# haoheliu/AudioLDM2

Measured on AMD Instinct MI355X. Metric: audio_seconds_per_second, higher is better.
Workload: dtype f32 storage/accumulate; each product = 6 bf16 MFMA partial products of exact 3-part operand splits (fp32-grade); 1 GPU; audioldm2-full: batch 8 prompts/GPU x 1 GPU, 10.24 s @16 kHz, 200 DDIM steps, CFG 3.5, eta 1.0, n_candidates 1; one step = sample_log + VAE decode + HiFi-GAN + D2H of the waveform; synthetic conditioning, random-init weights, host-CPU RNG noise; global_batch=8, parallelism=prompt-sharded replicas x1, weight_broadcast_bytes=0

## Files before the change

audioldm2_amd/csrc/api.hip:

```cpp
#include "common.h"
#include <string.h>

namespace aldm {
static thread_local char g_err[512] = "";
void set_error(const char* fmt, ...) {
    va_list ap;
    va_start(ap, fmt);
    vsnprintf(g_err, sizeof(g_err), fmt, ap);
    va_end(ap);
}
}

extern "C" int aldm_version(void) { return 13; }
extern "C" const char* aldm_last_error(void) { return aldm::g_err; }
```

audioldm2_amd/csrc/igemm.hip:

```cpp
#include "igemm_kernel.h"
#include <algorithm>
#include <atomic>
#include <stdlib.h>

namespace aldm {

int igemm_launch_pre0(int BM, int BN, int kgroups, bool uni, bool w8, dim3 grid, hipStream_t st, const IgemmK& p);
int igemm_launch_pre1(int BM, int BN, int kgroups, bool uni, bool w8, dim3 grid, hipStream_t st, const IgemmK& p);
int igemm_launch_pre2(int BM, int BN, int kgroups, bool uni, bool w8, dim3 grid, hipStream_t st, const IgemmK& p);
int igemm_launch_pre3(int BM, int BN, int kgroups, bool uni, bool w8, dim3 grid, hipStream_t st, const IgemmK& p);
int igemm_launch_pre4(int BM, int BN, int kgroups, bool uni, bool w8, dim3 grid, hipStream_t st, const IgemmK& p);
int igemm_launch_bx_pre0(int BM, int BN, int kgroups, bool uni, bool w8, dim3 grid, hipStream_t st, const IgemmK& p);
int igemm_launch_bx_pre1(int BM, int BN, int kgroups, bool uni, bool w8, dim3 grid, hipStream_t st, const IgemmK& p);
int igemm_launch_bx_pre2(int BM, int BN, int kgroups, bool uni, bool w8, dim3 grid, hipStream_t st, const IgemmK& p);
int igemm_launch_bx_pre3(int BM, int BN, int kgroups, bool uni, bool w8, dim3 grid, hipStream_t st, const IgemmK& p);

int igemm_launch_dma(int BM, int BN, int nst, int parts, bool f16, dim3 grid, hipStream_t st, const IgemmK& p);
bool igemm_dma_config_ok(int BM, int BN, int nst, int parts);
#ifdef ALDM_TEST_HOOKS
extern std::atomic<int> g_debug_drop_product;
#endif
int igemm_launch_dma_ws(int BM, int BN, int nst, int parts, int blocks, hipStream_t st, const IgemmK& p);
bool igemm_dma_ws_config_ok(int BM, int BN, int nst, int parts);
int igemm_dma_ws_blocks_per_cu(int BM, int BN, int nst, int parts);
// ... 112 lines not shown
}

template <int NP>
__global__ void pack_split_kernel(const float* __restrict__ src, uint4* __restrict__ dst, int Kg, int Npad,
                                  int Ko) {
    const int64_t total = (int64_t)Ko * Npad;
    for (int64_t i = blockIdx.x * (int64_t)blockDim.x + threadIdx.x; i < total;
         i += (int64_t)gridDim.x * blockDim.x) {
        const int n = (int)(i % Npad);
        const int ko = (int)(i / Npad);
        u32x2 part[2][3];
#pragma unroll
        for (int h = 0; h < 2; ++h) {
            const int kg = 2 * ko + h;
            f32x4 f = {0.f, 0.f, 0.f, 0.f};
            if (kg < Kg) f = *reinterpret_cast<const f32x4*>(src + ((int64_t)kg * Npad + n) * 4);
            split4_parts(f, part[h], NP);
        }
#pragma unroll
        for (int q = 0; q < NP; ++q) {
            uint4 o;
            o.x = part[0][q][0];
            o.y = part[0][q][1];
            o.z = part[1][q][0];
            o.w = part[1][q][1];
            dst[((int64_t)ko * NP + q) * Npad + n] = o;
        }
    }
}

__global__ void pack_split_f16_kernel(const float* __restrict__ src, uint4* __restrict__ dst, int Kg, int Npad, int Ko, float scale) {
    const int64_t total = (int64_t)Ko * Npad;
    for (int64_t i = blockIdx.x * (int64_t)blockDim.x + threadIdx.x; i < total; i += (int64_t)gridDim.x * blockDim.x) {
        const int n = (int)(i % Npad);
        const int ko = (int)(i / Npad);
        u32x2 part[2][3];
#pragma unroll
        for (int h = 0; h < 2; ++h) {
            const int kg = 2 * ko + h;
            f32x4 f = {0.f, 0.f, 0.f, 0.f};
            if (kg < Kg) f = *reinterpret_cast<const f32x4*>(src + ((int64_t)kg * Npad + n) * 4);
            split4_f16(f, scale, part[h]);
        }
#pragma unroll
        for (int q = 0; q < 2; ++q) {
            uint4 o;
            o.x = part[0][q][0];
            o.y = part[0][q][1];
            o.z = part[1][q][0];
            o.w = part[1][q][1];
            dst[((int64_t)ko * 2 + q) * Npad + n] = o;
        }
    }
}

static int log2_exact(int v) {
    int s = 0;
    while ((1 << s) < v) ++s;
    return (1 << s) == v ? s : -1;
}

}

using namespace aldm;

static thread_local int g_force_bm = 0, g_force_bn = 0, g_force_splits = 0, g_force_kgroups = 0, g_force_stages = 0;

extern "C" void aldm_igemm_force(int bm, int bn, int splits, int kgroups) {
    g_force_bm = bm;
    g_force_bn = bn;
    g_force_splits = splits;
    g_force_kgroups = kgroups;
    g_force_stages = 0;
}
extern "C" void aldm_igemm_force_stages(int stages) { g_force_stages = stages; }

static int default_wave8_mask() {
    static const int m = [] {
        const char* e = getenv("ALDM_IGEMM_W8");
        return e ? atoi(e) : 1;
    }();
    return m;
}
static thread_local int g_wave8_mask = -1;

extern "C" int aldm_igemm_wave8_mask(int mask) {
    g_wave8_mask = mask;
    return mask < 0 ? default_wave8_mask() : mask;
}

static thread_local int g_force_mma = 0;
extern "C" int aldm_igemm_mma(int mode) {
    const int prev = g_force_mma;
    if (mode >= 0 && mode <= 2) g_force_mma = mode;
    return prev;
}

static int pre_mode_of(const aldm_igemm_desc& d) {
    if (d.pre_scale == nullptr && d.pre_act == ALDM_ACT_NONE) return PRE_NONE;
    if (d.pre_scale != nullptr && d.pre_act == ALDM_ACT_NONE) return PRE_AFFINE;
    if (d.pre_scale != nullptr && d.pre_act == ALDM_ACT_SILU) return PRE_AFFINE_SILU;
    if (d.pre_scale == nullptr && d.pre_act == ALDM_ACT_LRELU) return PRE_LRELU;
    return PRE_GENERIC;
}

static int device_cus() {
    static const int n = [] {
        int dev = 0, cus = 0;
        if (hipGetDevice(&dev) != hipSuccess ||
            hipDeviceGetAttribute(&cus, hipDeviceAttributeMultiprocessorCount, dev) != hipSuccess || cus <= 0)
            return 256;
        return cus;
    }();
    return n;
}

static bool dma_ws_eligible(const IgemmK& p, int BM, int BN) {
    const aldm_igemm_desc& d = p.d;
    const bool geglu = d.epi_mode == ALDM_EPI_GEGLU;
    auto al16 = [](const void* q) { return (reinterpret_cast<uintptr_t>(q) & 15) == 0; };
    if (d.out_mul > 0 || d.accumulate || d.batch != 1 || d.act != ALDM_ACT_NONE || d.out_split_act != ALDM_ACT_NONE ||
        d.epi_mode == ALDM_EPI_QKV)
        return false;
    if (p.M % BM != 0 || d.N % BN != 0 || (d.N & 3) != 0 || (d.ldo & 3) != 0) return false;
    if (!al16(d.out) || !al16(d.res) || !al16(d.bias) || !al16(d.rowbias) || !al16(d.out_split)) return false;
    if (d.rowbias && (p.OHW % BM != 0 || (p.rb_ld & 3) != 0)) return false;
    if (geglu && (BN != 128 || d.res || d.rowbias)) return false;
    return true;
}

static bool dma_os_eligible(const IgemmK& p) {
    const aldm_igemm_desc& d = p.d;
    if (d.KH != 1 || d.KW != 1 || d.SH != 1 || d.SW != 1 || d.PH != 0 || d.PW != 0 || d.up_h != 1 || d.up_w != 1) return false;
    if (d.OH != d.H || d.OW != d.W || d.K != p.Cin || d.K % 32 != 0 || d.out_mul > 0 || d.batch > 1) return false;
    if (d.epi_mode == ALDM_EPI_QKV && d.qkv_c % 128 != 0) return false;
    if (d.rowbias || d.accumulate || d.act != ALDM_ACT_NONE) return false;
    auto al16 = [](const void* q) { return (reinterpret_cast<uintptr_t>(q) & 15) == 0; };
    if ((d.N & 3) != 0 || (d.ldo & 3) != 0 || !al16(d.out) || !al16(d.res)) return false;
    return true;
}

static int dma_halo_chunks(const IgemmK& p, int BM) {
    const aldm_igemm_desc& d = p.d;
    if (d.KH != 3 || d.KW != 3 || d.SH != 1 || d.SW != 1 || d.PH != 1 || d.PW != 1 || d.DH != 1 || d.DW != 1) return 0;
    if (d.up_h != 1 || d.up_w != 1 || d.OH != d.H || d.OW != d.W || d.out_mul > 0 || d.batch > 1) return 0;
    if (d.W <= 0 || (d.W & (d.W - 1)) != 0 || BM % d.W != 0 || p.OHW % BM != 0) return 0;
    return ((BM / d.W + 2) * d.W + 15) / 16;
}

static bool tile_supported(int BM, int BN) {
    return (BM == 128 && (BN == 128 || BN == 64 || BN == 32)) || (BM == 64 && (BN == 128 || BN == 64));
}

static int igemm_prepare(const aldm_igemm_desc* dd, IgemmK& p, int& BM, int& BN) {
    ALDM_CHECK(dd != nullptr, "aldm_igemm: null descriptor");
    p.d = *dd;
    aldm_igemm_desc& d = p.d;
    ALDM_CHECK((d.x1 || d.a_split) && d.w && (d.out || d.out_split), "aldm_igemm: null x1/w/out");
    if (!d.x1) d.x1 = reinterpret_cast<const float*>(d.a_split);
    if (d.split_parts == 0) d.split_parts = 3;
    ALDM_CHECK(d.split_parts == 2 || d.split_parts == 3, "aldm_igemm: split_parts must be 0 / 3 or 2");
    if (d.out_split_parts == 0) d.out_split_parts = d.split_parts;
    ALDM_CHECK(d.out_split_parts == 2 || d.out_split_parts == 3, "aldm_igemm: out_split_parts must be 0, 2 or 3");
    ALDM_CHECK(d.a_fmt == ALDM_FMT_BF16 || (d.a_fmt == ALDM_FMT_F16 && d.a_split != nullptr && d.split_parts == 2 && d.acc_scale > 0.0f),
               "aldm_igemm: a_fmt = ALDM_FMT_F16 needs a pre-split operand (a_split), 2-part images and acc_scale > 0");
    if (d.a_fmt == ALDM_FMT_BF16) d.acc_scale = 1.0f;
    ALDM_CHECK(d.out_split_fmt == ALDM_FMT_BF16 ||
                   (d.out_split_fmt == ALDM_FMT_F16 && d.out_split_scale > 0.0f &&
                    (d.epi_mode == ALDM_EPI_QKV ? (d.k_split != nullptr && d.vt_split != nullptr && d.vt_scale > 0.0f) : d.out_split != nullptr)),
               "aldm_igemm: out_split_fmt = ALDM_FMT_F16 needs out_split (QKV: k_split, vt_split and vt_scale) and out_split_scale > 0");
    if (d.out_split_fmt == ALDM_FMT_F16) d.out_split_parts = 2;
    if (!d.x2) d.C2 = 0;
    if (d.pix1 == 0) d.pix1 = d.C1;
    if (d.pix2 == 0) d.pix2 = d.C2;
    if (d.up_h == 0) d.up_h = 1;
    if (d.up_w == 0) d.up_w = 1;
    if (d.batch == 0) d.batch = 1;
    p.Cin = d.C1 + d.C2;
    ALDM_CHECK(d.C1 > 0 && d.C1 % 4 == 0 && d.C2 % 4 == 0,
               "aldm_igemm: C1=%d/C2=%d must be multiples of 4", d.C1, d.C2);
    ALDM_CHECK(d.pix1 % 4 == 0 && d.pix2 % 4 == 0, "aldm_igemm: pixel pitch must be a multiple of 4");
    ALDM_CHECK(d.K == d.KH * d.KW * p.Cin, "aldm_igemm: K=%d != KH*KW*Cin=%d", d.K,
               d.KH * d.KW * p.Cin);
    ALDM_CHECK(d.N > 0 && (d.ldo >= d.N || d.epi_mode == ALDM_EPI_GEGLU || d.epi_mode == ALDM_EPI_QKV),
               "aldm_igemm: bad N=%d ldo=%d", d.N, d.ldo);
    ALDM_CHECK(d.B > 0 && d.H > 0 && d.W > 0 && d.OH > 0 && d.OW > 0, "aldm_igemm: bad extents");
    ALDM_CHECK(d.SH > 0 && d.SW > 0 && d.DH > 0 && d.DW > 0, "aldm_igemm: bad stride/dilation");
    p.shh = log2_exact(d.up_h);
    p.shw = log2_exact(d.up_w);
    ALDM_CHECK(p.shh >= 0 && p.shw >= 0, "aldm_igemm: upsample factors must be powers of two");
    ALDM_CHECK((reinterpret_cast<uintptr_t>(d.x1) & 15) == 0 &&
                   (reinterpret_cast<uintptr_t>(d.w) & 15) == 0 &&
                   (d.x2 == nullptr || (reinterpret_cast<uintptr_t>(d.x2) & 15) == 0),
               "aldm_igemm: operands must be 16-byte aligned");
    if (d.b_mode == ALDM_B_NT) {
        ALDM_CHECK(d.ldb % 4 == 0 && d.ldb >= d.K, "aldm_igemm: NT ldb=%d invalid", d.ldb);
        p.Npad = d.N;
    } else {
        p.Npad = (d.N + 31) / 32 * 32;
        ALDM_CHECK(d.ldb == 0 || d.ldb == p.Npad, "aldm_igemm: packed ldb must equal Npad");
    }
    if (d.out_mul > 0) ALDM_CHECK(d.OH == 1, "aldm_igemm: row remap requires OH == 1");
    ALDM_CHECK((d.pre_scale == nullptr) == (d.pre_shift == nullptr),
               "aldm_igemm: pre_scale/pre_shift must come together");
    ALDM_CHECK(d.pre_scale == nullptr ||
                   ((reinterpret_cast<uintptr_t>(d.pre_scale) | reinterpret_cast<uintptr_t>(d.pre_shift)) & 15) == 0,
               "aldm_igemm: pre_scale/pre_shift must be 16-byte aligned");
    const bool geglu = d.epi_mode == ALDM_EPI_GEGLU;
    const bool qkv = d.epi_mode == ALDM_EPI_QKV;
    ALDM_CHECK(d.epi_mode == ALDM_EPI_PLAIN || geglu || qkv, "aldm_igemm: unknown epi_mode %d", d.epi_mode);
    if (qkv) {
        auto al16 = [](const void* q) { return (reinterpret_cast<uintptr_t>(q) & 15) == 0; };
        ALDM_CHECK(d.a_split && d.qkv_c > 0 && d.qkv_c % 64 == 0 && d.N == 3 * d.qkv_c && d.qkv_rows > 0 && d.qkv_rows % 32 == 0 &&
                       (((int64_t)d.B * d.OH * d.OW) % d.qkv_rows == 0 ||
                        d.qkv_rows == (((int64_t)d.B * d.OH * d.OW + 31) & ~(int64_t)31)) && d.out && d.k_split && d.vt_split && al16(d.out) &&
                       al16(d.k_split) && al16(d.vt_split) && d.ldo >= d.qkv_c && (d.ldo & 3) == 0 && !d.bias && !d.rowbias &&
                       !d.res && !d.out_split && !d.accumulate && d.out_mul == 0 && d.act == ALDM_ACT_NONE && d.alpha == 1.0f &&
                       d.batch <= 1,
                   "aldm_igemm: ALDM_EPI_QKV needs a pre-split operand, N = 3*qkv_c (qkv_c %% 64 == 0), qkv_rows %% 32 == 0 dividing M "
                   "(or M rounded up to 32), "
                   "aligned out / k_split / vt_split and a plain epilogue");
    }
    if (geglu) {
        ALDM_CHECK(d.N % 64 == 0 && d.ldo >= d.N / 2 && d.ldo % 4 == 0 && d.b_mode == ALDM_B_PACKED &&
                       d.out_mul == 0 && !d.res && !d.rowbias && !d.accumulate &&
                       (d.act == ALDM_ACT_NONE || d.act == ALDM_ACT_GELU_TANH) &&
                       (reinterpret_cast<uintptr_t>(d.out) & 15) == 0 && d.stride_o % 4 == 0 &&
                       (d.bias == nullptr || (reinterpret_cast<uintptr_t>(d.bias) & 15) == 0),
                   "aldm_igemm: GEGLU epilogue needs N %% 64 == 0, ldo >= N/2, packed weights, a plain epilogue");
    }
    p.OHW = d.OH * d.OW;
    const int64_t M64 = (int64_t)d.B * p.OHW;
    ALDM_CHECK(M64 < (1ll << 31) - 256, "aldm_igemm: M too large");
    p.M = (int)M64;
    p.HV = d.H * d.up_h;
    p.WV = d.W * d.up_w;
    ALDM_CHECK((int64_t)d.B * d.H * d.W < (1ll << 31), "aldm_igemm: input has too many pixels");
    p.Kg = (d.K + 3) / 4;
    p.rb_ld = d.rowbias_ld > 0 ? d.rowbias_ld : d.N;

    const int nk = (d.K + BK - 1) / BK;
    const int64_t Mz = p.M;
    const int pre = pre_mode_of(d);
    p.dma = 0;
    p.nst = 0;
    p.ws = 0;
    p.ws_blocks = 0;
    p.os_rows = 0;
    ALDM_CHECK(d.out_split_act == ALDM_ACT_NONE || (d.out_split_act == ALDM_ACT_LRELU && d.out_split != nullptr &&
                                                   d.epi_mode == ALDM_EPI_PLAIN),
               "aldm_igemm: out_split_act must be ALDM_ACT_NONE or ALDM_ACT_LRELU with a split-image output of the plain epilogue");
    if (d.out_split) {
        ALDM_CHECK(d.out_split_c > 0 && d.out_split_c % 32 == 0 && d.out_split_c >= (geglu ? d.N / 2 : d.N) &&
                       d.N % 4 == 0 && d.batch == 1 && (reinterpret_cast<uintptr_t>(d.out_split) & 15) == 0 &&
                       ((reinterpret_cast<uintptr_t>(d.out) | reinterpret_cast<uintptr_t>(d.res)) & 15) == 0 &&
                       (d.out == nullptr || (d.ldo & 3) == 0),
                   "aldm_igemm: out_split needs out_split_c %% 32 == 0 and >= N, N %% 4 == 0, batch 1, aligned out/res");
        ALDM_CHECK(d.out != nullptr || !d.accumulate, "aldm_igemm: accumulate needs an fp32 output");
    }
    if (d.a_split) {
        ALDM_CHECK(d.w_split != nullptr && d.b_mode == ALDM_B_PACKED && d.stride_w == 0 && d.batch == 1,
                   "aldm_igemm: a_split needs packed, split weights and batch 1");
        ALDM_CHECK(d.C2 == 0 && d.C1 % 32 == 0 && pre == PRE_NONE,
                   "aldm_igemm: a_split needs one source with C1 %% 32 == 0 and no prologue (C1=%d C2=%d)", d.C1, d.C2);
        ALDM_CHECK(((reinterpret_cast<uintptr_t>(d.a_split) | reinterpret_cast<uintptr_t>(d.w_split)) & 15) == 0,
                   "aldm_igemm: split images must be 16-byte aligned");
        ALDM_CHECK((int64_t)d.B * d.H * d.W * p.Cin * 2 * d.split_parts < (1ll << 40), "aldm_igemm: split image too large");
        const bool can_split = d.N % 4 == 0 && nk >= 8 && !geglu && !qkv;
        const bool have_ws = d.ws != nullptr && (reinterpret_cast<uintptr_t>(d.ws) & 15) == 0;
        auto dma_cost = [&](int bm, int bn, int nst, int sp, int* sp_eff) -> double {
            const int kt = cdiv(nk, sp);
            sp = cdiv(nk, kt);
            *sp_eff = sp;
            const double blocks = (double)cdiv64(Mz, bm) * cdiv(d.N, bn) * sp;
            const int lds = nst * (bm + bn) * 64 * d.split_parts;
            const int o = std::min(2, (160 * 1024) / lds);
            const double tile_c = (bm / 64) * (bn / 64) * 64.0 * (d.split_parts == 3 ? 6 : 3);
            const double dma_c = (bm + bn) * 64.0 * d.split_parts / 56.0;
            const double L = kt * std::max(tile_c, dma_c);
            const double one = kt * std::max(tile_c + 200.0, dma_c) + 6000.0;
            const int64_t nb = (int64_t)((blocks + 255.0) / 256.0);
            const int64_t full = nb / o, last = nb - full * o;
            double T = full * std::max(one, o * L);
            if (last) T += std::max(one, last * L);
            if (sp > 1) T += 10000.0 + (double)(sp + 1) * Mz * d.N * 4.0 / 2000.0;
            return T;
        };
        int splits = 1, nst = 0;
        const bool hint_fits = d.hint_bm > 0 && (!qkv || (d.hint_bn > 0 && d.qkv_c % d.hint_bn == 0)) && (!geglu || d.hint_bn == 128);
        const int f_bm = g_force_bm ? g_force_bm : (hint_fits ? d.hint_bm : 0), f_bn = g_force_bm ? g_force_bn : d.hint_bn;
        const int f_sp = g_force_bm ? g_force_splits : d.hint_splits;
        int f_st = g_force_bm ? g_force_stages : (hint_fits ? d.hint_stages : 0);
        int ws_nst = 0;
        int lw_nst = 0;
        if (f_st >= 300 && f_st < 400) {
            const int KT = d.K / 32;
            int os_nst = f_st - 300;
            if (os_nst == 0) os_nst = igemm_dma_os_default_stages(KT, d.split_parts);
            if (dma_os_eligible(p) && igemm_dma_os_config_ok(KT, os_nst, d.split_parts)) {
                static const int env_rows = [] {
                    const char* e = getenv("ALDM_OS_ROWS");
                    return e ? atoi(e) : 0;
                }();
                const int tn = cdiv(d.N, 128);
                const int stages = cdiv(p.M, 32);
                const int chunks = std::max(1, device_cus() / tn);
                int rows = cdiv(stages, chunks) * 32;
// ... 77 lines not shown
                if (geglu ? bn != 128 : (bn > 64 && d.N <= 64)) continue;
                if (qkv && d.qkv_c % bn != 0) continue;
                if (bm == 256 && Mz < 4096) continue;
                for (int si = 0; si < 8; ++si) {
                    const int sp = sps[si];
                    if (sp > 1 && (!can_split || !have_ws || nk / sp < 3)) break;
                    int spe;
                    const double t = dma_cost(bm, bn, cand[c][2], sp, &spe);
                    if (spe > 1 && (int64_t)spe * Mz * d.N > d.ws_floats) continue;
                    if (t < best) {
                        best = t;
                        BM = bm;
                        BN = bn;
                        nst = cand[c][2];
                        splits = spe;
                    }
                }
            }
        }
        ALDM_CHECK(!geglu || BN == 128, "aldm_igemm: the GEGLU epilogue needs a 128-column tile");
        ALDM_CHECK(!qkv || d.qkv_c % BN == 0, "aldm_igemm: the QKV epilogue needs a tile width dividing qkv_c");
        if (qkv) splits = 1;
        p.tiles_m = cdiv(p.M, BM);
        p.tiles_n = cdiv(d.N, BN);
        p.kt_per_split = cdiv(nk, splits);
        splits = cdiv(nk, p.kt_per_split);
        if (splits > 1 && (!have_ws || d.ws_floats < (int64_t)splits * p.M * d.N)) {
            splits = 1;
            p.kt_per_split = nk;
        }
        p.splits = splits;
        p.kgroups = 1;
        p.bx = 1;
        p.pre = pre;
        p.dma = 1;
        p.nst = nst;
        p.ws = 0;
        p.ws_blocks = 0;
        if (lw_nst > 0) {
            ALDM_CHECK(igemm_dma_lw_config_ok(BM, BN, lw_nst, d.split_parts), "aldm_igemm: no loader-wave DMA kernel for tile %dx%d, %d stages", BM, BN, lw_nst);
            p.ws = 2;
            p.nst = lw_nst;
        }
        if (ws_nst > 0) {
            if (splits == 1 && d.a_fmt == ALDM_FMT_BF16 && d.out_split_parts == d.split_parts && d.out_split_fmt == ALDM_FMT_BF16 &&
                igemm_dma_ws_config_ok(BM, BN, ws_nst, d.split_parts) && dma_ws_eligible(p, BM, BN)) {
                const int ntiles = p.tiles_m * p.tiles_n;
                const int per = cdiv(ntiles, device_cus() * igemm_dma_ws_blocks_per_cu(BM, BN, ws_nst, d.split_parts));
                p.ws = 1;
                p.nst = ws_nst;
                p.ws_blocks = cdiv(ntiles, per);
            } else {
                ALDM_CHECK(!g_force_bm, "aldm_igemm: the persistent DMA kernel cannot run this launch (tile %dx%d, %d stages)", BM,
                           BN, ws_nst);
            }
        }
        return 0;
    }
    const bool bx_ok = d.w_split != nullptr && d.split_parts == 3 && d.b_mode == ALDM_B_PACKED && d.stride_w == 0 && d.batch == 1 &&
                       pre != PRE_GENERIC && (reinterpret_cast<uintptr_t>(d.w_split) & 15) == 0 &&
                       (g_force_mma == 2 || (g_force_mma == 0 && d.hint_mma != 1));
    auto occ_of = [&](int bm, int bn) {
        if (bx_ok && bn != 32) return bm * bn >= 128 * 128 ? 1 : (bm * bn >= 64 * 128 ? 2 : 3);
        return bm * bn >= 128 * 128 ? 2 : ((bm * bn >= 64 * 128 || bn == 32) ? 3 : 4);
    };
    const double pre_w = (d.pre_scale != nullptr || d.pre_act != ALDM_ACT_NONE) ? 1.5 : 1.0;
    auto cost_of = [&](int bm, int bn, int sp, int kg, int* sp_eff) -> double {
        const bool bx = bx_ok && bn != 32;
        const double mf = bx ? 0.375 : 1.0;
        const int kt = cdiv(nk, sp);
        sp = cdiv(nk, kt);
        *sp_eff = sp;
        const double blocks = (double)cdiv64(Mz, bm) * cdiv(d.N, bn) * d.batch * sp;
        const double L = (double)kt * bm * bn / 4.0 * mf;
        const int o = kg == 2 ? (bx ? 1 : 2) : occ_of(bm, bn);
        const double S = (300.0 * (bm / 32) * pre_w + 200.0 * (bn / 32)) *
                         (bx ? (bm * bn >= 128 * 128 && !geglu ? 0.45 : 1.3) : 1.0);
        const double F = 4000.0 + (kg == 2 ? 600.0 : 0.0);
        const int64_t nb = (int64_t)((blocks + 255.0) / 256.0);
        const int64_t full = nb / o, last = nb - full * o;
        const double one = (double)cdiv(kt, kg) * ((double)bm * bn / 4.0 * mf + S) + F;
        double T = full * std::max(one, o * L);
        if (last) T += std::max(one, last * L);
        if (sp > 1) T += 10000.0 + (double)(sp + 1) * Mz * d.N * d.batch * 4.0 / 2000.0;
        return T;
    };
    const bool can_split = d.N % 4 == 0 && nk >= 8 && !geglu;
    const bool have_ws = d.ws != nullptr && (reinterpret_cast<uintptr_t>(d.ws) & 15) == 0;
    int splits = 1, kgroups = 1;
    const int f_bm = g_force_bm ? g_force_bm : d.hint_bm, f_bn = g_force_bm ? g_force_bn : d.hint_bn;
    const int f_sp = g_force_bm ? g_force_splits : d.hint_splits;
    const int f_kg = g_force_bm ? g_force_kgroups : d.hint_kgroups;
    if (f_bm) {
        BM = f_bm;
        BN = f_bn;
        ALDM_CHECK(tile_supported(BM, BN), "aldm_igemm: unsupported forced/hinted tile %dx%d", BM, BN);
        ALDM_CHECK(!geglu || BN == 128, "aldm_igemm: the GEGLU epilogue needs a 128-column tile");
        if (f_sp > 0 && can_split && nk / f_sp >= 1) splits = f_sp;
        if (f_kg == 2) {
            ALDM_CHECK(BM == 64 && BN == 64, "aldm_igemm: two wave groups exist for the 64x64 tile only");
            kgroups = 2;
        }
    } else if (d.N <= 32 && !geglu) {
        BM = 128;
        BN = 32;
    } else {
        static const int cand[4][2] = {{128, 128}, {64, 128}, {128, 64}, {64, 64}};
        static const int sps[8] = {1, 2, 3, 4, 6, 8, 12, 16};
        double best = 1e300;
        BM = 64;
        BN = 64;
        for (int c = 0; c < 4; ++c) {
            const int bm = cand[c][0], bn = cand[c][1];
            if (geglu ? bn != 128 : (bn > 64 && d.N <= 64)) continue;
            for (int si = 0; si < 8; ++si) {
                const int sp = sps[si];
                if (sp > 1 && (!can_split || !have_ws || nk / sp < 3)) break;
                for (int kg = 1; kg <= ((bm == 64 && bn == 64) ? 2 : 1); ++kg) {
                    int spe;
                    const double t = cost_of(bm, bn, sp, kg, &spe);
                    if (spe > 1 && (int64_t)d.batch * spe * Mz * d.N > d.ws_floats) continue;
                    if (kg == 2 && cdiv(nk, spe) < 4) continue;
                    if (t < best) {
                        best = t;
                        BM = bm;
                        BN = bn;
                        splits = spe;
                        kgroups = kg;
                    }
                }
            }
        }
    }
    ALDM_CHECK(!geglu || BN == 128, "aldm_igemm: internal: GEGLU epilogue without a 128-column tile");
    p.tiles_m = cdiv(p.M, BM);
    p.tiles_n = cdiv(d.N, BN);
    if (splits < 1) splits = 1;
    p.kt_per_split = cdiv(nk, splits);
    splits = cdiv(nk, p.kt_per_split);
    if (splits > 1) {
        const int64_t need = (int64_t)d.batch * splits * p.M * d.N;
        if (!have_ws || d.ws_floats < need) {
            splits = 1;
            p.kt_per_split = nk;
        }
    }
    p.splits = splits;
    p.kgroups = kgroups;
    p.bx = bx_ok && BN != 32 ? 1 : 0;
    p.pre = pre;
    return 0;
}

extern "C" int aldm_igemm_plan(const aldm_igemm_desc* dd, int* bm, int* bn, int64_t* flops, int* splits,
                               int* kgroups, int* mma) {
    IgemmK p;
    int BM, BN;
    const int rc = igemm_prepare(dd, p, BM, BN);
    if (rc) return rc;
    if (bm) *bm = BM;
    if (bn) *bn = BN;
    if (flops) *flops = 2ll * p.M * p.d.N * p.d.K * p.d.batch;
    if (splits) *splits = p.splits;
    if (kgroups) *kgroups = p.kgroups;
    if (mma) *mma = p.bx ? ALDM_MMA_BF16X6 : ALDM_MMA_F32;
    return 0;
}

extern "C" int aldm_igemm_plan_stages(const aldm_igemm_desc* dd) {
    IgemmK p;
    int BM, BN;
    if (igemm_prepare(dd, p, BM, BN)) return -1;
    if (p.dma && p.ws == 4) return 400 + (BM == 128 && p.ws_blocks == 4 ? 10 : 0) + p.nst;
    return p.dma ? p.nst + 100 * p.ws : 0;
}

extern "C" int64_t aldm_igemm_ws_floats(const aldm_igemm_desc* dd) {
    if (!dd) return 0;
    aldm_igemm_desc t = *dd;
    t.ws = reinterpret_cast<float*>(uintptr_t(16));
    t.ws_floats = INT64_MAX;
    IgemmK p;
    int BM, BN;
    if (igemm_prepare(&t, p, BM, BN)) return 0;
    return p.splits > 1 ? (int64_t)p.d.batch * p.splits * p.M * p.d.N : 0;
}

extern "C" int aldm_igemm(const aldm_igemm_desc* dd, void* stream) {
    IgemmK p;
    int BM, BN;
    int rc = igemm_prepare(dd, p, BM, BN);
    if (rc) return rc;
    const aldm_igemm_desc& d = p.d;
    dim3 grid((unsigned)(p.tiles_m * p.tiles_n), (unsigned)p.splits, (unsigned)d.batch);
    hipStream_t st = (hipStream_t)stream;
    const int pre = p.pre;
    const bool uni = p.OHW % BM == 0;
    const int env_w8 = g_wave8_mask < 0 ? default_wave8_mask() : g_wave8_mask;
    const bool gn_pre = pre == PRE_AFFINE || pre == PRE_AFFINE_SILU;
    const int tile_bit = (BM == 128 && BN == 128) ? 1 : (BM == 64 && BN == 128) ? 2 : (BM == 128 && BN == 64) ? 4 : 0;
    const bool w8 = p.kgroups == 1 && d.epi_mode != ALDM_EPI_GEGLU && (env_w8 & tile_bit) != 0 &&
                    (p.bx ? tile_bit == 1 : (gn_pre || (tile_bit == 1 && (env_w8 & 8) != 0)));
#ifdef ALDM_TEST_HOOKS
    if (g_debug_drop_product.load(std::memory_order_relaxed))
        ALDM_CHECK(p.dma && p.ws == 0 && BM == 64 && BN == 128 && p.nst == 2 && d.split_parts == 3,
                   "aldm_igemm: aldm_debug_drop_product is set: force the classic DMA-fed 64x128 tile with 2 stages and 3-part images "
                   "(got dma=%d form=%d tile %dx%d, %d stages, %d parts) or clear the switch", p.dma, p.ws, BM, BN, p.nst, d.split_parts);
#endif
    if (p.dma && p.ws == 4) {
        rc = igemm_launch_dma_halo(BM, BN, p.nst, p.ws_blocks, d.split_parts, d.a_fmt == ALDM_FMT_F16, p.os_rows, grid, st, p);
    } else if (p.dma && p.ws == 3) {
        rc = igemm_launch_dma_os(d.K / 32, p.nst, d.split_parts, d.a_fmt == ALDM_FMT_F16, grid, st, p);
    } else if (p.dma && p.ws == 2) {
        rc = igemm_launch_dma_lw(BM, BN, p.nst, d.split_parts, d.a_fmt == ALDM_FMT_F16, grid, st, p);
    } else if (p.dma && p.ws) {
        rc = igemm_launch_dma_ws(BM, BN, p.nst, d.split_parts, p.ws_blocks, st, p);
    } else if (p.dma) {
        rc = igemm_launch_dma(BM, BN, p.nst, d.split_parts, d.a_fmt == ALDM_FMT_F16, grid, st, p);
    } else if (p.bx) {
        switch (pre) {
            case PRE_NONE: rc = igemm_launch_bx_pre0(BM, BN, p.kgroups, uni, w8, grid, st, p); break;
            case PRE_AFFINE: rc = igemm_launch_bx_pre1(BM, BN, p.kgroups, uni, w8, grid, st, p); break;
            case PRE_AFFINE_SILU: rc = igemm_launch_bx_pre2(BM, BN, p.kgroups, uni, w8, grid, st, p); break;
            default: rc = igemm_launch_bx_pre3(BM, BN, p.kgroups, uni, w8, grid, st, p); break;
        }
    } else
    switch (pre) {
        case PRE_NONE: rc = igemm_launch_pre0(BM, BN, p.kgroups, uni, w8, grid, st, p); break;
        case PRE_AFFINE: rc = igemm_launch_pre1(BM, BN, p.kgroups, uni, w8, grid, st, p); break;
        case PRE_AFFINE_SILU: rc = igemm_launch_pre2(BM, BN, p.kgroups, uni, w8, grid, st, p); break;
        case PRE_LRELU: rc = igemm_launch_pre3(BM, BN, p.kgroups, uni, w8, grid, st, p); break;
        default: rc = igemm_launch_pre4(BM, BN, p.kgroups, uni, w8, grid, st, p); break;
    }
    if (rc) {
        set_error("aldm_igemm: no kernel for tile %dx%d", BM, BN);
        return -1;
    }
    if (p.splits > 1) {
        const int64_t total = (int64_t)p.M * (d.N >> 2);
        hipLaunchKernelGGL(igemm_reduce_kernel, dim3((unsigned)cdiv64(total, 256), 1, (unsigned)d.batch),
                           dim3(256), 0, st, p);
    }
    ALDM_LAUNCH_CHECK("aldm_igemm");
    return 0;
}

extern "C" int64_t aldm_split_bytes_parts(int K, int N, int parts) {
    if (K <= 0 || N <= 0 || (parts != 2 && parts != 3)) return 0;
    const int Npad = (N + 31) / 32 * 32;
    const int64_t Ko = 4ll * ((K + 31) / 32);
    return Ko * parts * Npad * 16;
}
extern "C" int64_t aldm_split_bytes(int K, int N) { return aldm_split_bytes_parts(K, N, 3); }

extern "C" int aldm_pack_split_f16(const float* packed, void* dst, int K, int N, float scale, void* stream) {
    ALDM_CHECK(packed && dst && K > 0 && N > 0 && scale > 0.0f, "aldm_pack_split_f16: bad args");
    ALDM_CHECK(((reinterpret_cast<uintptr_t>(packed) | reinterpret_cast<uintptr_t>(dst)) & 15) == 0,
               "aldm_pack_split_f16: operands must be 16-byte aligned");
    const int Npad = (N + 31) / 32 * 32;
    const int Kg = (K + 3) / 4;
    const int Ko = 4 * ((K + 31) / 32);
    const int64_t total = (int64_t)Ko * Npad;
    hipLaunchKernelGGL(pack_split_f16_kernel, dim3((unsigned)std::min<int64_t>(cdiv64(total, 256), 4096)), dim3(256), 0,
                       (hipStream_t)stream, packed, reinterpret_cast<uint4*>(dst), Kg, Npad, Ko, scale);
    ALDM_LAUNCH_CHECK("aldm_pack_split_f16");
    return 0;
}

extern "C" int aldm_pack_split_bf16_parts(const float* packed, void* dst, int K, int N, int parts, void* stream) {
    ALDM_CHECK(packed && dst && K > 0 && N > 0 && (parts == 2 || parts == 3), "aldm_pack_split_bf16: bad args");
    ALDM_CHECK(((reinterpret_cast<uintptr_t>(packed) | reinterpret_cast<uintptr_t>(dst)) & 15) == 0,
               "aldm_pack_split_bf16: operands must be 16-byte aligned");
    const int Npad = (N + 31) / 32 * 32;
    const int Kg = (K + 3) / 4;
    const int Ko = 4 * ((K + 31) / 32);
    const int64_t total = (int64_t)Ko * Npad;
    const int blocks = (int)std::min<int64_t>((total + 255) / 256, 65535);
    if (parts == 3)
        hipLaunchKernelGGL(pack_split_kernel<3>, dim3(blocks), dim3(256), 0, (hipStream_t)stream, packed,
                           reinterpret_cast<uint4*>(dst), Kg, Npad, Ko);
    else
        hipLaunchKernelGGL(pack_split_kernel<2>, dim3(blocks), dim3(256), 0, (hipStream_t)stream, packed,
                           reinterpret_cast<uint4*>(dst), Kg, Npad, Ko);
    ALDM_LAUNCH_CHECK("aldm_pack_split_bf16");
    return 0;
}
extern "C" int aldm_pack_split_bf16(const float* packed, void* dst, int K, int N, void* stream) {
    return aldm_pack_split_bf16_parts(packed, dst, K, N, 3, stream);
}

extern "C" int aldm_pack_weight(const float* src, float* dst, int N, int Cin, int KH, int KW,
                                int transposed, int phase, int stride, void* stream) {
    ALDM_CHECK(src && dst && N > 0 && Cin > 0 && KH > 0 && KW > 0, "aldm_pack_weight: bad args");
    const int Npad = (N + 31) / 32 * 32;
    hipStream_t st = (hipStream_t)stream;
    if (!transposed) {
        const int K = KH * KW * Cin;
        const int Kg = (K + 3) / 4;
        const int64_t total = (int64_t)Kg * Npad * 4;
        const int blocks = (int)std::min<int64_t>(cdiv64(total, 256), 4096);
        hipLaunchKernelGGL(pack_weight_kernel, dim3(blocks), dim3(256), 0, st, src, dst, N, Cin, KH,
                           KW, Kg, Npad);
    } else {
        ALDM_CHECK(KH == 1 && stride > 0 && phase >= 0 && phase < stride,
                   "aldm_pack_weight: bad transposed args");
        const int T = (KW + stride - 1) / stride;
// ... 24 lines not shown
```

audioldm2_amd/csrc/igemm_epilogue.h:

```cpp
#pragma once
#include "common.h"

#ifndef ALDM_DMA_ABLATE
#define ALDM_DMA_ABLATE 0
#endif

namespace aldm {

struct IgemmK {
    aldm_igemm_desc d;
    int Cin, M, OHW, HV, WV, shh, shw, Kg, Npad, tiles_m, tiles_n;
    int splits, kt_per_split;
    int kgroups;
    int rb_ld;
    int bx;
    int pre;
    int dma;
    int nst;
    int ws;
    int ws_blocks;
    int os_rows;
};

enum { PRE_NONE = 0, PRE_AFFINE = 1, PRE_AFFINE_SILU = 2, PRE_LRELU = 3, PRE_GENERIC = 4 };
// ... 24 lines not shown
__device__ __forceinline__ void acc_total(f32x16 (&acc)[MT][NT], const f32x16 (&sum)[MT][NT]) {
#pragma unroll
    for (int i = 0; i < MT; ++i)
#pragma unroll
        for (int j = 0; j < NT; ++j)
#pragma unroll
            for (int e = 0; e < 16; ++e) acc[i][j][e] += sum[i][j][e];
}

using bf16x8 = __bf16 __attribute__((ext_vector_type(8)));
using u32x2 = unsigned __attribute__((ext_vector_type(2)));
using u32x4 = unsigned __attribute__((ext_vector_type(4)));
__device__ __forceinline__ unsigned hi16_pair(unsigned a, unsigned b) { return __builtin_amdgcn_perm(b, a, 0x07060302u); }

constexpr int SPLIT_BLOCK_BYTES = 192;

__device__ __forceinline__ unsigned bf16_rn_bits(float x) {
    const unsigned u = __builtin_bit_cast(unsigned, x);
    return (u + 0x7FFFu + ((u >> 16) & 1u)) & 0xFFFF0000u;
}

__device__ __forceinline__ void split4(const f32x4 v, u32x2 (&part)[3]) {
    unsigned u0[4], u1[4], u2[4];
#pragma unroll
    for (int c = 0; c < 4; ++c) {
        const float x = v[c];
        u0[c] = __builtin_bit_cast(unsigned, x);
        const float r1 = x - __builtin_bit_cast(float, u0[c] & 0xFFFF0000u);
        u1[c] = __builtin_bit_cast(unsigned, r1);
        const float r2 = r1 - __builtin_bit_cast(float, u1[c] & 0xFFFF0000u);
        u2[c] = __builtin_bit_cast(unsigned, r2);
    }
    part[0] = u32x2{hi16_pair(u0[0], u0[1]), hi16_pair(u0[2], u0[3])};
    part[1] = u32x2{hi16_pair(u1[0], u1[1]), hi16_pair(u1[2], u1[3])};
    part[2] = u32x2{hi16_pair(u2[0], u2[1]), hi16_pair(u2[2], u2[3])};
}

using bf16x4 = __bf16 __attribute__((ext_vector_type(4)));
__device__ __forceinline__ void split4_rn2(const f32x4 v, u32x2 (&part)[3]) {
    const bf16x4 h = __builtin_convertvector(v, bf16x4);
    const bf16x4 m = __builtin_convertvector(v - __builtin_convertvector(h, f32x4), bf16x4);
    part[0] = __builtin_bit_cast(u32x2, h);
    part[1] = __builtin_bit_cast(u32x2, m);
    part[2] = u32x2{0u, 0u};
}

__device__ __forceinline__ void split4_parts(const f32x4 v, u32x2 (&part)[3], int parts) {
    if (parts == 2) split4_rn2(v, part);
    else split4(v, part);
}

using f16x4 = _Float16 __attribute__((ext_vector_type(4)));
using f16x8 = _Float16 __attribute__((ext_vector_type(8)));
__device__ __forceinline__ void split4_f16(const f32x4 v, float s, u32x2 (&part)[3]) {
    f32x4 x;
#pragma unroll
    for (int e = 0; e < 4; ++e) {
        const float t = v[e] * s;
        x[e] = t != t ? t : __builtin_fminf(__builtin_fmaxf(t, -65504.0f), 65504.0f);
    }
    const f16x4 h = __builtin_convertvector(x, f16x4);
    const f16x4 l = __builtin_convertvector(x - __builtin_convertvector(h, f32x4), f16x4);
    part[0] = __builtin_bit_cast(u32x2, h);
    part[1] = __builtin_bit_cast(u32x2, l);
    part[2] = u32x2{0u, 0u};
}
__device__ __forceinline__ void split4_fmt(const f32x4 v, u32x2 (&part)[3], int parts, float f16_scale) {
    if (f16_scale != 0.f) split4_f16(v, f16_scale, part);
    else split4_parts(v, part, parts);
}

__device__ __forceinline__ void split_store4(void* img, int64_t row, int Cs, int c, const f32x4 v, int parts = 3) {
    u32x2 part[3];
    split4_parts(v, part, parts);
    char* base = reinterpret_cast<char*>(img) + (row * (Cs >> 5) + (c >> 5)) * (64 * parts) + (c & 31) * 2;
#pragma unroll
    for (int q = 0; q < 3; ++q)
        if (q < parts) *reinterpret_cast<u32x2*>(base + q * 64) = part[q];
}

__device__ __forceinline__ void split_store4_f16(void* img, int64_t row, int Cs, int c, const f32x4 v, float scale) {
    u32x2 part[3];
    split4_f16(v, scale, part);
    char* base = reinterpret_cast<char*>(img) + (row * (Cs >> 5) + (c >> 5)) * 128 + (c & 31) * 2;
    *reinterpret_cast<u32x2*>(base) = part[0];
    *reinterpret_cast<u32x2*>(base + 64) = part[1];
}
__device__ __forceinline__ void split_store4_out(const aldm_igemm_desc& d, void* img, int64_t row, int Cs, int c, const f32x4 v) {
    if (d.out_split_fmt == ALDM_FMT_F16) split_store4_f16(img, row, Cs, c, v, d.out_split_scale);
    else split_store4(img, row, Cs, c, v, d.out_split_parts);
}

template <int P>
__device__ __forceinline__ void split_store4_t(void* img, int64_t row, int Cs, int c, const f32x4 v) {
    static_assert(P == 2 || P == 3, "2 or 3 parts");
    u32x2 part[3];
    if constexpr (P == 2) split4_rn2(v, part);
    else split4(v, part);
    char* base = reinterpret_cast<char*>(img) + (row * (Cs >> 5) + (c >> 5)) * (64 * P) + (c & 31) * 2;
#pragma unroll
    for (int q = 0; q < P; ++q) *reinterpret_cast<u32x2*>(base + q * 64) = part[q];
}

__device__ __forceinline__ float epi_value(const aldm_igemm_desc& d, int rb_ld, const float* __restrict__ outp,
                                           const float* __restrict__ resp, int b, int64_t o, int n, float v) {
    if (d.bias) v += d.bias[n];
    if (d.rowbias) v += d.rowbias[(int64_t)b * rb_ld + n];
    v = act_apply(v, d.act, d.act_slope);
    if (resp) v += resp[o];
    v *= d.alpha;
    if (d.accumulate) v += outp[o];
    return v;
}

__device__ __forceinline__ float silu_fast(float v) {
    return v * __frcp_rn(1.0f + __expf(-v));
}

__device__ __forceinline__ void split8_to_parts(const float (&x)[8], u32x4 (&part)[3], int parts) {
    f32x4 a = {x[0], x[1], x[2], x[3]}, b = {x[4], x[5], x[6], x[7]};
    u32x2 pa[3], pb[3];
    split4_parts(a, pa, parts);
    split4_parts(b, pb, parts);
#pragma unroll
    for (int q = 0; q < 3; ++q) part[q] = u32x4{pa[q][0], pa[q][1], pb[q][0], pb[q][1]};
}

template <int MT, int NT, int PAD = 4>
__device__ __forceinline__ void igemm_epilogue(const IgemmK& p, f32x16 (&acc)[MT][NT], float* lds, int m0, int n0,
                                               int wave, int wm, int wn, int lane, int z, int split) {
    const aldm_igemm_desc& d = p.d;
    const bool epi_st = (ALDM_DMA_ABLATE & 64) ? p.M == -12345 : true;
    constexpr int SP = NT * 32 + PAD;
    constexpr int C4 = NT * 8;
    constexpr int RPI = 64 / C4;
    constexpr int IT = 32 / RPI;
    constexpr int ITC = IT < 4 ? IT : 4;
    const int l31 = lane & 31;
    const int lh = lane >> 5;
    float* stg = lds + wave * (32 * SP);
    const int sr = lane / C4;
    const int sc = (lane % C4) * 4;
    const int ncol = n0 + wn * NT * 32 + sc;
    const bool split_out = p.splits > 1;
    const bool vec = split_out || ((d.ldo & 3) == 0 && (d.N & 3) == 0 &&
                                   ((reinterpret_cast<uintptr_t>(d.out) | reinterpret_cast<uintptr_t>(d.res)) & 15) == 0 &&
                                   ((d.stride_o & 3) == 0));
    float* outp = split_out ? d.ws + ((int64_t)z * p.splits + split) * (int64_t)p.M * d.N
                            : (d.out ? d.out + (int64_t)z * d.stride_o : nullptr);
    const float* resp = (!split_out && d.res) ? d.res + (int64_t)z * d.stride_o : nullptr;
    const bool need_b = !split_out && (d.rowbias != nullptr || d.out_mul > 0);
    const int ld_out = split_out ? d.N : d.ldo;
    void* simg = split_out ? nullptr : d.out_split;
    int col_shift = 0;
    int simg_c = d.out_split_c;
    if (d.epi_mode == ALDM_EPI_QKV) {
        const int seg = n0 / d.qkv_c;
        if (seg == 2) {
            char* vt = reinterpret_cast<char*>(d.vt_split);
            const int heads = d.qkv_c >> 5, parts = d.out_split_parts;
            const int tiles = d.qkv_rows >> 5;
#pragma unroll
            for (int i = 0; i < MT; ++i) {
                const int mb = m0 + (wm * MT + i) * 32;
                if (mb >= p.M) continue;
                const int b = mb / d.qkv_rows, t = (mb - b * d.qkv_rows) >> 5;
#pragma unroll
                for (int j = 0; j < NT; ++j) {
                    const int h = (n0 - 2 * d.qkv_c + (wn * NT + j) * 32) >> 5;
                    char* base = vt + ((((int64_t)b * heads + h) * tiles + t) * parts) * 2048 + l31 * 64 + lh * 16;
#pragma unroll
                    for (int s = 0; s < 2; ++s) {
                        float x8[8];
#pragma unroll
                        for (int e = 0; e < 8; ++e) x8[e] = acc[i][j][8 * s + e];
                        u32x4 part[3];
                        if (d.out_split_fmt == ALDM_FMT_F16) {
                            f32x4 a = {x8[0], x8[1], x8[2], x8[3]}, bq = {x8[4], x8[5], x8[6], x8[7]};
                            u32x2 pa[3], pb[3];
                            split4_f16(a, d.vt_scale, pa);
                            split4_f16(bq, d.vt_scale, pb);
#pragma unroll
                            for (int q = 0; q < 3; ++q) part[q] = u32x4{pa[q][0], pa[q][1], pb[q][0], pb[q][1]};
                        } else {
                            split8_to_parts(x8, part, parts);
                        }
#pragma unroll
                        for (int q = 0; q < 3; ++q)
                            if (q < parts && epi_st) *reinterpret_cast<u32x4*>(base + q * 2048 + s * 32) = part[q];
                    }
                }
            }
            return;
        }
        if (seg == 1) {
            outp = nullptr;
            simg = d.k_split;
            simg_c = d.qkv_c;
            col_shift = d.qkv_c;
        } else {
            simg = nullptr;
        }
    }
    if constexpr (NT == 2) {
        if (d.epi_mode == ALDM_EPI_GEGLU) {
            const int gr = lane >> 3, gc = (lane & 7) * 4;
            const int ncol_p = n0 + wn * 64 + gc;
            const int ncol_o = ((n0 + wn * 64) >> 1) + gc;
            const bool cok = ncol_p < d.N;
            f32x4 bv = {0.f, 0.f, 0.f, 0.f}, bg = {0.f, 0.f, 0.f, 0.f};
            if (d.bias && cok) {
                bv = *reinterpret_cast<const f32x4*>(d.bias + ncol_p);
                bg = *reinterpret_cast<const f32x4*>(d.bias + ncol_p + 32);
            }
            float* go = d.out ? d.out + (int64_t)z * d.stride_o : nullptr;
            const int gate_act = d.act == ALDM_ACT_GELU_TANH ? ALDM_ACT_GELU_TANH : ALDM_ACT_GELU;
#pragma unroll
            for (int i = 0; i < MT; ++i) {
#pragma unroll
                for (int j = 0; j < NT; ++j)
#pragma unroll
                    for (int e = 0; e < 16; ++e)
                        stg[((e & 3) + 8 * (e >> 2) + 4 * lh) * SP + j * 32 + l31] = acc[i][j][e];
#pragma unroll
                for (int it = 0; it < 4; ++it) {
                    const int r = it * 8 + gr;
                    f32x4 xv = *reinterpret_cast<const f32x4*>(&stg[r * SP + gc]) + bv;
                    const f32x4 xg = *reinterpret_cast<const f32x4*>(&stg[r * SP + 32 + gc]) + bg;
#pragma unroll
                    for (int c = 0; c < 4; ++c) xv[c] *= act_apply(xg[c], gate_act, 0.f);
                    const int m = m0 + (wm * MT + i) * 32 + r;
                    if (m < p.M && cok && epi_st) {
                        if (go) *reinterpret_cast<f32x4*>(go + (int64_t)m * d.ldo + ncol_o) = xv;
                        if (simg) split_store4_out(d, simg, m, d.out_split_c, ncol_o, xv);
                    }
                }
            }
            return;
        }
    }
    f32x4 bias4 = {0.f, 0.f, 0.f, 0.f};
    if (!split_out && d.bias) {
#pragma unroll
        for (int c = 0; c < 4; ++c) bias4[c] = d.bias[min(ncol + c, d.N - 1)];
    }
#pragma unroll
    for (int i = 0; i < MT; ++i) {
#pragma unroll
        for (int j = 0; j < NT; ++j)
#pragma unroll
            for (int e = 0; e < 16; ++e)
                stg[((e & 3) + 8 * (e >> 2) + 4 * lh) * SP + j * 32 + l31] = acc[i][j][e];
#pragma unroll
        for (int itc = 0; itc < IT; itc += ITC) {
        f32x4 v[ITC];
        int64_t rowoff[ITC];
        int64_t srow[ITC];
        int rboff[ITC];
        unsigned okmask = 0;
#pragma unroll
        for (int it = 0; it < ITC; ++it) {
            const int r = (itc + it) * RPI + sr;
            v[it] = *reinterpret_cast<const f32x4*>(&stg[r * SP + sc]);
            const int m = m0 + (wm * MT + i) * 32 + r;
            bool ok = m < p.M && ncol < d.N;
            int b = 0;
            int64_t orow = m;
            if (need_b) {
                b = m / p.OHW;
                if (d.out_mul > 0) {
                    const int qq = m - b * p.OHW;
                    const int t = qq * d.out_mul + d.out_off;
                    ok = ok && (unsigned)t < (unsigned)d.out_len;
                    orow = (int64_t)b * d.out_len + t;
                }
            }
            rowoff[it] = ok ? orow * ld_out + (ncol - col_shift) : 0;
            srow[it] = orow;
            rboff[it] = ok ? b * p.rb_ld + ncol : 0;
            okmask |= ((ok && epi_st) ? 1u : 0u) << it;
        }
        if (split_out) {
#pragma unroll
            for (int it = 0; it < ITC; ++it)
                if ((okmask >> it) & 1u) *reinterpret_cast<f32x4*>(outp + rowoff[it]) = v[it];
            continue;
        }
#pragma unroll
        for (int it = 0; it < ITC; ++it) v[it] += bias4;
        if (d.rowbias) {
#pragma unroll
            for (int it = 0; it < ITC; ++it)
#pragma unroll
                for (int c = 0; c < 4; ++c) v[it][c] += d.rowbias[rboff[it] + (ncol + c < d.N ? c : 0)];
        }
        switch (d.act) {
            case ALDM_ACT_NONE: break;
            case ALDM_ACT_SILU:
#pragma unroll
                for (int it = 0; it < ITC; ++it)
#pragma unroll
                    for (int c = 0; c < 4; ++c) v[it][c] = act_apply(v[it][c], ALDM_ACT_SILU, 0.f);
                break;
            case ALDM_ACT_GELU:
#pragma unroll
                for (int it = 0; it < ITC; ++it)
#pragma unroll
                    for (int c = 0; c < 4; ++c) v[it][c] = act_apply(v[it][c], ALDM_ACT_GELU, 0.f);
                break;
            default:
#pragma unroll
                for (int it = 0; it < ITC; ++it)
#pragma unroll
                    for (int c = 0; c < 4; ++c) v[it][c] = act_apply(v[it][c], d.act, d.act_slope);
                break;
        }
        if (vec) {
            if (resp) {
#pragma unroll
                for (int it = 0; it < ITC; ++it) v[it] += *reinterpret_cast<const f32x4*>(resp + rowoff[it]);
            }
#pragma unroll
            for (int it = 0; it < ITC; ++it) v[it] *= d.alpha;
            if (d.accumulate) {
#pragma unroll
                for (int it = 0; it < ITC; ++it) v[it] += *reinterpret_cast<const f32x4*>(outp + rowoff[it]);
            }
            if (outp) {
#pragma unroll
                for (int it = 0; it < ITC; ++it)
                    if ((okmask >> it) & 1u) *reinterpret_cast<f32x4*>(outp + rowoff[it]) = v[it];
            }
            if (simg) {
                if (d.out_split_act == ALDM_ACT_LRELU) {
#pragma unroll
                    for (int it = 0; it < ITC; ++it)
#pragma unroll
                        for (int c = 0; c < 4; ++c) v[it][c] = v[it][c] > 0.0f ? v[it][c] : v[it][c] * d.out_split_slope;
                }
#pragma unroll
                for (int it = 0; it < ITC; ++it)
                    if ((okmask >> it) & 1u) {
                        split_store4_out(d, simg, srow[it], simg_c, ncol - col_shift, v[it]);
                    }
            }
        } else {
#pragma unroll
            for (int it = 0; it < ITC; ++it)
#pragma unroll
                for (int c = 0; c < 4; ++c) {
                    if (!((okmask >> it) & 1u) || ncol + c >= d.N) continue;
                    float x = v[it][c];
                    if (resp) x += resp[rowoff[it] + c];
                    x *= d.alpha;
                    if (d.accumulate) x += outp[rowoff[it] + c];
                    outp[rowoff[it] + c] = x;
                }
        }
        }
    }
}

}
```

audioldm2_amd/csrc/norm.hip:

```cpp
#include <stdlib.h>
#include "igemm_epilogue.h"

namespace aldm {

constexpr int GN_ITERS = 16;
constexpr int GN_UNROLL = 8;

struct GnPart {
    float n, mean, m2;
};

__device__ __forceinline__ void gn_merge(double& n, double& mean, double& m2, double nb, double mb, double m2b) {
    if (nb <= 0.0) return;
    const double nt = n + nb;
    const double dlt = mb - mean;
    mean += dlt * (nb / nt);
    m2 += m2b + dlt * dlt * (n * nb / nt);
    n = nt;
}

template <bool FUSED>
__global__ __launch_bounds__(256) void gn_partial_kernel(const float* __restrict__ x1,
                                                         const float* __restrict__ x2, int P,
                                                         int C1, int C2, int G, int cols, int rows,
// ... 79 lines not shown
                    wred[tid >> 6][1] = mean;
                    wred[tid >> 6][2] = m2;
                }
                __syncthreads();
                if (tid == 0) {
                    double an = gacc[gl][0], am = gacc[gl][1], a2 = gacc[gl][2];
                    for (int w = 0; w < 4; ++w) gn_merge(an, am, a2, wred[w][0], wred[w][1], wred[w][2]);
                    gacc[gl][0] = an;
                    gacc[gl][1] = am;
                    gacc[gl][2] = a2;
                }
                __syncthreads();
            }
            continue;
        }
        ps[tid] = part;
        __syncthreads();
        if (tid < gpb) {
            const int g = g_lo + tid;
            const int base = c4_lo + cp * cols;
            const int lo = max(g * Cg4, base), hi = min((g + 1) * Cg4, min(C4, base + cols));
            if (lo < hi) {
                double n = gacc[tid][0], mean = gacc[tid][1], m2 = gacc[tid][2];
                for (int yy = 0; yy < rows; ++yy)
                    for (int cc = lo; cc < hi; ++cc) {
                        const GnPart& t = ps[yy * cols + (cc - base)];
                        gn_merge(n, mean, m2, (double)t.n, (double)t.mean, (double)t.m2);
                    }
                gacc[tid][0] = n;
                gacc[tid][1] = mean;
                gacc[tid][2] = m2;
            }
        }
        __syncthreads();
    }
    if (FUSED) {
        const int Cg = C / G;
        __shared__ float fin[64][2];
        if (tid < gpb) {
            const double n = gacc[tid][0];
            double var = n > 0.0 ? gacc[tid][2] / n : 0.0;
            if (var < 0.0) var = 0.0;
            fin[tid][0] = (float)gacc[tid][1];
            fin[tid][1] = (float)(1.0 / sqrt(var + (double)eps));
        }
        __syncthreads();
        __shared__ float lsc[256], lsh[256];
        for (int c = g_lo * Cg + tid; c < (g_lo + gpb) * Cg; c += 256) {
            const int g = c / Cg - g_lo;
            const float sc = fin[g][1] * (gamma ? gamma[c] : 1.f);
            const float sh = (beta ? beta[c] : 0.f) - fin[g][0] * sc;
            scale[(int64_t)b * C + c] = sc;
            shift[(int64_t)b * C + c] = sh;
            if (dst) {
                lsc[c - g_lo * Cg] = sc;
                lsh[c - g_lo * Cg] = sh;
            }
        }
        if (dst) {
            __syncthreads();
            const int c_lo = g_lo * Cg, sw = (gpb * Cg) >> 3;
            for (int i = tid; i < P * sw; i += 256) {
                const int p = i / sw;
                const int cl = (i - p * sw) << 3;
                const int c = c_lo + cl;
                const int64_t row = (int64_t)b * P + p;
                const float* src = c < C1 ? x1 + row * C1 + c : x2 + row * C2 + (c - C1);
                f32x4 v0 = *reinterpret_cast<const f32x4*>(src);
                f32x4 v1 = *reinterpret_cast<const f32x4*>(src + 4);
                const int64_t off = (row * (C >> 5) + (c >> 5)) * (64 * parts) + (c & 31) * 2;
                u32x2 p0[3], p1[3];
                if (dst_raw) {
                    const int64_t roff = (row * (C >> 5) + (c >> 5)) * (64 * raw_parts) + (c & 31) * 2;
                    split4_parts(v0, p0, raw_parts);
                    split4_parts(v1, p1, raw_parts);
#pragma unroll
                    for (int q = 0; q < 3; ++q)
                        if (q < raw_parts)
                            *reinterpret_cast<u32x4*>(dst_raw + roff + q * 64) = u32x4{p0[q][0], p0[q][1], p1[q][0], p1[q][1]};
                }
#pragma unroll
                for (int e = 0; e < 4; ++e) {
                    v0[e] = __builtin_fmaf(v0[e], lsc[cl + e], lsh[cl + e]);
                    v1[e] = __builtin_fmaf(v1[e], lsc[cl + 4 + e], lsh[cl + 4 + e]);
                }
                if (act == ALDM_ACT_SILU) {
#pragma unroll
                    for (int e = 0; e < 4; ++e) {
                        v0[e] = silu_fast(v0[e]);
                        v1[e] = silu_fast(v1[e]);
                    }
                }
                split4_fmt(v0, p0, parts, f16_scale);
                split4_fmt(v1, p1, parts, f16_scale);
#pragma unroll
                for (int q = 0; q < 3; ++q)
                    if (q < parts) *reinterpret_cast<u32x4*>(dst + off + q * 64) = u32x4{p0[q][0], p0[q][1], p1[q][0], p1[q][1]};
            }
        }
    } else if (tid < G) {
        double* w = reinterpret_cast<double*>(ws) + ((int64_t)(b * gridDim.x + chunk) * G + tid) * 3;
        w[0] = gacc[tid][0];
        w[1] = gacc[tid][1];
        w[2] = gacc[tid][2];
    }
}

__global__ __launch_bounds__(256) void gn_finalize_kernel(const float* __restrict__ ws, int chunks,
                                                          int P, int C, int G, float eps,
                                                          const float* __restrict__ gamma,
                                                          const float* __restrict__ beta,
                                                          float* __restrict__ scale,
                                                          float* __restrict__ shift) {
    const int b = blockIdx.x;
    __shared__ float s_mean[64], s_rstd[64];
    __shared__ double s_part[256][3];
    const int Cg = C / G;
    const double* wsd = reinterpret_cast<const double*>(ws);
    const int LPG = 256 / G >= 1 ? 256 / G : 1;
    {
        const int g = threadIdx.x / LPG, l = threadIdx.x % LPG;
        double n = 0.0, mean = 0.0, m2 = 0.0;
        if (g < G) {
            for (int ch = l; ch < chunks; ch += LPG) {
                const double* w = wsd + ((int64_t)(b * chunks + ch) * G + g) * 3;
                gn_merge(n, mean, m2, w[0], w[1], w[2]);
            }
        }
        s_part[threadIdx.x][0] = n;
        s_part[threadIdx.x][1] = mean;
        s_part[threadIdx.x][2] = m2;
    }
    __syncthreads();
    if (threadIdx.x < G) {
        const int g = threadIdx.x;
        double n = 0.0, mean = 0.0, m2 = 0.0;
        for (int l = 0; l < LPG; ++l) gn_merge(n, mean, m2, s_part[g * LPG + l][0], s_part[g * LPG + l][1], s_part[g * LPG + l][2]);
        double var = n > 0.0 ? m2 / n : 0.0;
        if (var < 0.0) var = 0.0;
        s_mean[g] = (float)mean;
        s_rstd[g] = (float)(1.0 / sqrt(var + (double)eps));
    }
    __syncthreads();
    for (int c = threadIdx.x; c < C; c += blockDim.x) {
        const int g = c / Cg;
        const float ga = gamma ? gamma[c] : 1.f;
        const float be = beta ? beta[c] : 0.f;
        const float sc = s_rstd[g] * ga;
        scale[(int64_t)b * C + c] = sc;
        shift[(int64_t)b * C + c] = be - s_mean[g] * sc;
    }
}

constexpr int LN_MAXV = 8;

template <int MAXV, int R, bool RMS = false>
__global__ __launch_bounds__(256) void layernorm_kernel(const float* __restrict__ x,
                                                        float* __restrict__ y, int M, int C,
                                                        const float* __restrict__ gamma,
                                                        const float* __restrict__ beta, float eps,
                                                        void* __restrict__ y_split, int parts, float f16_scale) {
    const int lane = threadIdx.x & 63;
    const int row0 = (blockIdx.x * 4 + (threadIdx.x >> 6)) * R;
    if (row0 >= M) return;
    const int C4 = C >> 2;
    f32x4 v[R][MAXV];
#pragma unroll
    for (int r = 0; r < R; ++r) {
        const float* xr = x + (int64_t)min(row0 + r, M - 1) * C;
#pragma unroll
        for (int i = 0; i < MAXV; ++i) {
            const int c4 = lane + 64 * i;
            v[r][i] = c4 < C4 ? *reinterpret_cast<const f32x4*>(xr + 4 * c4) : f32x4{0.f, 0.f, 0.f, 0.f};
        }
    }
    f32x4 ga[MAXV], be[MAXV];
#pragma unroll
    for (int i = 0; i < MAXV; ++i) {
        const int c4 = min(lane + 64 * i, C4 - 1);
        ga[i] = *reinterpret_cast<const f32x4*>(gamma + 4 * c4);
        be[i] = RMS ? f32x4{0.f, 0.f, 0.f, 0.f} : *reinterpret_cast<const f32x4*>(beta + 4 * c4);
    }
    float mean[R], rstd[R];
#pragma unroll
    for (int r = 0; r < R; ++r) {
        float s = 0.f;
#pragma unroll
        for (int i = 0; i < MAXV; ++i) s += (v[r][i][0] + v[r][i][1]) + (v[r][i][2] + v[r][i][3]);
#pragma unroll
        for (int o = 32; o > 0; o >>= 1) s += __shfl_xor(s, o);
        mean[r] = RMS ? 0.f : s / (float)C;
    }
#pragma unroll
    for (int r = 0; r < R; ++r) {
        float q = 0.f;
#pragma unroll
        for (int i = 0; i < MAXV; ++i) {
            if (lane + 64 * i < C4) {
                const f32x4 dlt = v[r][i] - mean[r];
                q += (dlt[0] * dlt[0] + dlt[1] * dlt[1]) + (dlt[2] * dlt[2] + dlt[3] * dlt[3]);
            }
        }
#pragma unroll
        for (int o = 32; o > 0; o >>= 1) q += __shfl_xor(q, o);
        rstd[r] = 1.0f / sqrtf(q / (float)C + eps);
    }
#pragma unroll
    for (int r = 0; r < R; ++r) {
        if (row0 + r >= M) break;
        float* yr = y ? y + (int64_t)(row0 + r) * C : nullptr;
#pragma unroll
        for (int i = 0; i < MAXV; ++i) {
            const int c4 = lane + 64 * i;
            if (c4 < C4) {
                const f32x4 o = (v[r][i] - mean[r]) * rstd[r] * ga[i] + be[i];
                if (yr) *reinterpret_cast<f32x4*>(yr + 4 * c4) = o;
                if (y_split) {
                    if (f16_scale != 0.f) {
                        u32x2 part[3];
                        split4_f16(o, f16_scale, part);
                        char* base = reinterpret_cast<char*>(y_split) + ((int64_t)(row0 + r) * (C >> 5) + (c4 >> 3)) * 128 + (c4 & 7) * 8;
                        *reinterpret_cast<u32x2*>(base) = part[0];
                        *reinterpret_cast<u32x2*>(base + 64) = part[1];
                    } else {
                        split_store4(y_split, row0 + r, C, 4 * c4, o, parts);
                    }
                }
            }
        }
    }
}

template <bool MASKED, bool BIASED = false>
__global__ __launch_bounds__(256) void softmax_rows_kernel(const float* __restrict__ x,
                                                           float* __restrict__ y, int N,
                                                           float scale, const float* __restrict__ keymask,
                                                           int rows_per_batch, int q_rows, int q_pos0,
                                                           const float* __restrict__ bias = nullptr) {
    extern __shared__ __attribute__((aligned(16))) float srow[];
    __shared__ float red[4];
    const int64_t row = blockIdx.x;
    const float* xr = x + row * N;
    float* yr = y + row * N;
    const int tid = threadIdx.x;
    float mx = -INFINITY;
    const float* km = nullptr;
    int jmax = N;
    const float* br = nullptr;
    if (MASKED) {
        km = keymask + (row / rows_per_batch) * N;
        jmax = BIASED ? N : q_pos0 + (int)(row % q_rows) + 1;
    }
    if (BIASED) br = bias + (row % rows_per_batch) * N;
    for (int i = tid; i < N; i += 256) {
        float v = xr[i] * scale;
        if (BIASED) v += br[i];
        if (MASKED && (i >= jmax || km[i] == 0.0f)) v = -INFINITY;
        srow[i] = v;
        mx = fmaxf(mx, v);
    }
#pragma unroll
    for (int o = 32; o > 0; o >>= 1) mx = fmaxf(mx, __shfl_xor(mx, o));
    if ((tid & 63) == 0) red[tid >> 6] = mx;
    __syncthreads();
    mx = fmaxf(fmaxf(red[0], red[1]), fmaxf(red[2], red[3]));
    __syncthreads();
    float s = 0.f;
    for (int i = tid; i < N; i += 256) {
        const float e = (MASKED && srow[i] == -INFINITY) ? 0.0f : expf(srow[i] - mx);
        srow[i] = e;
        s += e;
    }
#pragma unroll
    for (int o = 32; o > 0; o >>= 1) s += __shfl_xor(s, o);
    if ((tid & 63) == 0) red[tid >> 6] = s;
    __syncthreads();
    s = (red[0] + red[1]) + (red[2] + red[3]);
    const float inv = 1.0f / s;
    for (int i = tid; i < N; i += 256) yr[i] = srow[i] * inv;
}

static void gn_geometry(int P, int C, int* cols, int* rows, int* chunk_px, int* chunks) {
    const int C4 = C / 4;
    *cols = C4 < 256 ? C4 : 256;
    *rows = 256 / *cols;
    if (*rows < 1) *rows = 1;
    *chunk_px = *rows * GN_ITERS;
    *chunks = (P + *chunk_px - 1) / *chunk_px;
}

}

using namespace aldm;

extern "C" int64_t aldm_gn_ws_floats(int B, int P, int C, int G) {
    int cols, rows, chunk_px, chunks;
    gn_geometry(P, C, &cols, &rows, &chunk_px, &chunks);
    return (int64_t)B * chunks * G * 6 + 2;
}

extern "C" int aldm_split_rows(const float* x1, const float* x2, int C1, int C2, int64_t rows, int P, const float* scale,
                               const float* shift, int act, void* dst, void* dst_raw, int parts, void* stream);
extern "C" int aldm_split_rows_f16(const float* x1, const float* x2, int C1, int C2, int64_t rows, int P, const float* scale,
                                   const float* shift, int act, float slope, void* dst, void* dst_raw, int raw_parts, float f16_scale,
                                   void* stream);

static int groupnorm_launch(const float* x1, const float* x2, int B, int P, int C1, int C2, int G, float eps,
                            const float* gamma, const float* beta, float* scale, float* shift, float* ws, void* dst,
                            void* dst_raw, int parts, int act, void* stream, int raw_parts = 0, float f16_scale = 0.f) {
    if (raw_parts == 0) raw_parts = parts;
    if (!x2) C2 = 0;
    const int C = C1 + C2;
    ALDM_CHECK(x1 && scale && shift && ws, "aldm_groupnorm_stats: null pointer");
    ws = reinterpret_cast<float*>((reinterpret_cast<uintptr_t>(ws) + 7) & ~uintptr_t(7));
    ALDM_CHECK(G > 0 && G <= 64 && C % G == 0 && (C / G) % 4 == 0 && C1 % 4 == 0,
               "aldm_groupnorm_stats: need C%%G==0, (C/G)%%4==0, C1%%4==0 (C1=%d C2=%d G=%d)", C1, C2, G);
    int cols, rows, chunk_px, chunks;
    gn_geometry(P, C, &cols, &rows, &chunk_px, &chunks);
    hipStream_t st = (hipStream_t)stream;
    static const int64_t fused_max = [] {
        const char* e = getenv("ALDM_GN_FUSED_MAX");
        return e ? (int64_t)atoll(e) : (int64_t)1 << 17;
    }();
    int gs = 1;
    while (gs < G && gs * B < 256 && G % (gs * 2) == 0) gs *= 2;
    const int gpb = G / gs;
    if ((int64_t)P * C <= fused_max && P <= 1024 && gpb <= 4) {
        const int c4b = gpb * (C / G) / 4;
        const int fcols = c4b < 256 ? c4b : 256, frows = 256 / fcols;
        const int slab = gpb * (C / G);
        static const bool fuse_split = [] {
            const char* e = getenv("ALDM_GN_SPLIT_FUSED");
            return e == nullptr || e[0] != '0';
        }();
        if (dst && fuse_split && slab % 8 == 0 && slab <= 256 && C1 % 8 == 0) {
            hipLaunchKernelGGL(gn_partial_kernel<true>, dim3(gs, B), dim3(256), 0, st, x1, x2, P, C1, C2, G, fcols, frows, P, ws,
                               eps, gamma, beta, scale, shift, gpb, reinterpret_cast<char*>(dst),
                               reinterpret_cast<char*>(dst_raw), parts, act, raw_parts, f16_scale);
            ALDM_LAUNCH_CHECK("aldm_groupnorm_split");
            return 0;
        }
        hipLaunchKernelGGL(gn_partial_kernel<true>, dim3(gs, B), dim3(256), 0, st, x1, x2, P, C1, C2, G, fcols,
                           frows, P, ws, eps, gamma, beta, scale, shift, gpb, nullptr, nullptr, 3, ALDM_ACT_NONE);
    } else {
        hipLaunchKernelGGL(gn_partial_kernel<false>, dim3(chunks, B), dim3(256), 0, st, x1, x2, P, C1, C2, G,
                           cols, rows, chunk_px, ws, eps, gamma, beta, scale, shift, G);
        hipLaunchKernelGGL(gn_finalize_kernel, dim3(B), dim3(256), 0, st, ws, chunks, P, C, G, eps, gamma,
                           beta, scale, shift);
    }
    ALDM_LAUNCH_CHECK("aldm_groupnorm_stats");
    if (dst) {
        if (f16_scale != 0.f)
            return aldm_split_rows_f16(x1, x2, C1, C2, (int64_t)B * P, P, scale, shift, act, 0.f, dst, dst_raw, raw_parts, f16_scale, stream);
        return aldm_split_rows(x1, x2, C1, C2, (int64_t)B * P, P, scale, shift, act, dst, dst_raw, parts, stream);
    }
    return 0;
}

extern "C" int aldm_groupnorm_stats(const float* x1, const float* x2, int B, int P, int C1, int C2,
                                    int G, float eps, const float* gamma, const float* beta,
                                    float* scale, float* shift, float* ws, void* stream) {
    return groupnorm_launch(x1, x2, B, P, C1, C2, G, eps, gamma, beta, scale, shift, ws, nullptr, nullptr, 3, ALDM_ACT_NONE,
                            stream);
}

extern "C" int aldm_groupnorm_split(const float* x1, const float* x2, int B, int P, int C1, int C2, int G, float eps,
                                    const float* gamma, const float* beta, int act, float* scale, float* shift, float* ws,
                                    void* dst, void* dst_raw, int parts, void* stream) {
    if (!x2) C2 = 0;
    ALDM_CHECK(dst != nullptr && (parts == 2 || parts == 3) && (C1 + C2) % 32 == 0 && C1 % 8 == 0 && C2 % 8 == 0,
               "aldm_groupnorm_split: need dst, parts 2|3, (C1+C2) %% 32 == 0, C1 %% 8 == 0 (C1=%d C2=%d)", C1, C2);
    ALDM_CHECK(act == ALDM_ACT_NONE || act == ALDM_ACT_SILU, "aldm_groupnorm_split: activation %d not supported", act);
    ALDM_CHECK(((reinterpret_cast<uintptr_t>(dst) | reinterpret_cast<uintptr_t>(dst_raw)) & 15) == 0,
               "aldm_groupnorm_split: split images must be 16-byte aligned");
    return groupnorm_launch(x1, x2, B, P, C1, C2, G, eps, gamma, beta, scale, shift, ws, dst, dst_raw, parts, act, stream);
}

extern "C" int aldm_groupnorm_split_f16(const float* x1, const float* x2, int B, int P, int C1, int C2, int G, float eps,
                                        const float* gamma, const float* beta, int act, float* scale, float* shift, float* ws,
                                        void* dst, void* dst_raw, int raw_parts, float f16_scale, void* stream) {
    if (!x2) C2 = 0;
    ALDM_CHECK(dst != nullptr && f16_scale > 0.0f && (raw_parts == 2 || raw_parts == 3) && (C1 + C2) % 32 == 0 && C1 % 8 == 0 && C2 % 8 == 0,
               "aldm_groupnorm_split_f16: need dst, f16_scale > 0, raw_parts 2|3, (C1+C2) %% 32 == 0, C1 %% 8 == 0 (C1=%d C2=%d)", C1, C2);
    ALDM_CHECK(act == ALDM_ACT_NONE || act == ALDM_ACT_SILU, "aldm_groupnorm_split_f16: activation %d not supported", act);
    ALDM_CHECK(((reinterpret_cast<uintptr_t>(dst) | reinterpret_cast<uintptr_t>(dst_raw)) & 15) == 0,
               "aldm_groupnorm_split_f16: split images must be 16-byte aligned");
    return groupnorm_launch(x1, x2, B, P, C1, C2, G, eps, gamma, beta, scale, shift, ws, dst, dst_raw, 2, act, stream, raw_parts, f16_scale);
}

static int layernorm_launch(const float* x, float* y, void* y_split, int parts, int M, int C, const float* gamma,
                            const float* beta, float eps, void* stream, const char* name, bool rms = false, float f16_scale = 0.f) {
    ALDM_CHECK(parts == 2 || parts == 3, "%s: parts must be 2 or 3", name);
    ALDM_CHECK(x && (y || y_split) && gamma && (beta || rms), "%s: null pointer", name);
    ALDM_CHECK(C % 4 == 0 && C <= 256 * LN_MAXV, "%s: C=%d must be a multiple of 4 and <= %d", name, C, 256 * LN_MAXV);
    ALDM_CHECK(y_split == nullptr || (C % 32 == 0 && (reinterpret_cast<uintptr_t>(y_split) & 15) == 0),
               "%s: a split-image output needs C %% 32 == 0 and 16-byte alignment", name);
    hipStream_t st = (hipStream_t)stream;
#define ALDM_LN(V_, R_)                                                                                             \
    do {                                                                                                            \
        if (rms)                                                                                                    \
            hipLaunchKernelGGL((layernorm_kernel<V_, R_, true>), dim3(cdiv(M, 4 * R_)), dim3(256), 0, st, x, y, M, C, \
                               gamma, beta, eps, y_split, parts, f16_scale);                                        \
        else                                                                                                        \
            hipLaunchKernelGGL((layernorm_kernel<V_, R_, false>), dim3(cdiv(M, 4 * R_)), dim3(256), 0, st, x, y, M, \
                               C, gamma, beta, eps, y_split, parts, f16_scale);                                     \
    } while (0)
    const int nv = cdiv(C / 4, 64);
    static const int env_r = [] {
        const char* e = getenv("ALDM_LN_R");
        return e ? atoi(e) : 0;
    }();
    if (nv <= 1) {
        if (env_r == 4) ALDM_LN(1, 4);
        else if (env_r == 2) ALDM_LN(1, 2);
        else ALDM_LN(1, 1);
    } else if (nv <= 2) {
        if (env_r == 4) ALDM_LN(2, 4);
        else if (env_r == 2) ALDM_LN(2, 2);
        else ALDM_LN(2, 1);
    } else if (nv <= 4) ALDM_LN(4, 2);
    else ALDM_LN(8, 1);
#undef ALDM_LN
    ALDM_LAUNCH_CHECK(name);
    return 0;
}

extern "C" int aldm_layernorm(const float* x, float* y, int M, int C, const float* gamma,
                              const float* beta, float eps, void* stream) {
    return layernorm_launch(x, y, nullptr, 3, M, C, gamma, beta, eps, stream, "aldm_layernorm");
}

extern "C" int aldm_layernorm_split(const float* x, float* y, void* y_split, int M, int C, const float* gamma,
                                    const float* beta, float eps, int parts, void* stream) {
    return layernorm_launch(x, y, y_split, parts, M, C, gamma, beta, eps, stream, "aldm_layernorm_split");
}

extern "C" int aldm_layernorm_split_f16(const float* x, float* y, void* y_split, int M, int C, const float* gamma,
                                        const float* beta, float eps, float f16_scale, void* stream) {
    ALDM_CHECK(y_split != nullptr && f16_scale > 0.0f, "aldm_layernorm_split_f16: need y_split and f16_scale > 0");
    return layernorm_launch(x, y, y_split, 2, M, C, gamma, beta, eps, stream, "aldm_layernorm_split_f16", false, f16_scale);
}

extern "C" int aldm_rmsnorm(const float* x, float* y, int M, int C, const float* weight, float eps, void* stream) {
    return layernorm_launch(x, y, nullptr, 3, M, C, weight, nullptr, eps, stream, "aldm_rmsnorm", true);
}

extern "C" int aldm_softmax_rows(const float* x, float* y, int64_t M, int N, float scale,
                                 void* stream) {
    ALDM_CHECK(x && y && M > 0 && N > 0, "aldm_softmax_rows: bad args");
    ALDM_CHECK((int64_t)N * 4 <= 60 * 1024, "aldm_softmax_rows: row of %d floats exceeds the 60 KiB LDS stage", N);
    ALDM_CHECK(M < (1ll << 31), "aldm_softmax_rows: too many rows");
    hipLaunchKernelGGL(softmax_rows_kernel<false>, dim3((unsigned)M), dim3(256), (size_t)N * 4,
                       (hipStream_t)stream, x, y, N, scale, nullptr, 1, 1, 0);
    ALDM_LAUNCH_CHECK("aldm_softmax_rows");
    return 0;
}

extern "C" int aldm_softmax_rows_masked(const float* x, float* y, int B, int heads, int q_rows, int N, float scale,
                                        const float* keymask, int q_pos0, void* stream) {
    ALDM_CHECK(x && y && keymask && B > 0 && heads > 0 && q_rows > 0 && N > 0 && q_pos0 >= 0,
               "aldm_softmax_rows_masked: bad args");
    ALDM_CHECK((int64_t)N * 4 <= 60 * 1024, "aldm_softmax_rows_masked: row of %d floats exceeds the 60 KiB LDS stage", N);
    const int64_t M = (int64_t)B * heads * q_rows;
    ALDM_CHECK(M < (1ll << 31), "aldm_softmax_rows_masked: too many rows");
    hipLaunchKernelGGL(softmax_rows_kernel<true>, dim3((unsigned)M), dim3(256), (size_t)N * 4, (hipStream_t)stream, x, y,
                       N, scale, keymask, heads * q_rows, q_rows, q_pos0);
    ALDM_LAUNCH_CHECK("aldm_softmax_rows_masked");
    return 0;
}

extern "C" int aldm_softmax_rows_bias(const float* x, float* y, int B, int heads, int q_rows, int N, float scale,
                                      const float* bias, const float* keymask, void* stream) {
    ALDM_CHECK(x && y && bias && keymask && B > 0 && heads > 0 && q_rows > 0 && N > 0, "aldm_softmax_rows_bias: bad args");
    ALDM_CHECK((int64_t)N * 4 <= 60 * 1024, "aldm_softmax_rows_bias: row of %d floats exceeds the 60 KiB LDS stage", N);
    const int64_t M = (int64_t)B * heads * q_rows;
    ALDM_CHECK(M < (1ll << 31), "aldm_softmax_rows_bias: too many rows");
    hipLaunchKernelGGL((softmax_rows_kernel<true, true>), dim3((unsigned)M), dim3(256), (size_t)N * 4, (hipStream_t)stream, x,
                       y, N, scale, keymask, heads * q_rows, q_rows, 0, bias);
    ALDM_LAUNCH_CHECK("aldm_softmax_rows_bias");
    return 0;
}
```

audioldm2_amd/lib.py:

```python
from __future__ import annotations

import ctypes as C
import os

_HERE = os.path.dirname(os.path.abspath(__file__))
LIB_PATH = os.environ.get("ALDM_LIB_PATH") or os.path.join(_HERE, "libaldm_hip.so")
ABI_VERSION = 13

ACT_NONE, ACT_SILU, ACT_LRELU, ACT_TANH, ACT_LOGCLAMP, ACT_GELU, ACT_GELU_TANH = range(7)
B_PACKED, B_NT = 0, 1
EPI_PLAIN, EPI_GEGLU, EPI_QKV = 0, 1, 2
FMT_BF16, FMT_F16 = 0, 1


class IgemmDesc(C.Structure):

    _fields_ = [
        ("x1", C.c_void_p), ("x2", C.c_void_p),
        ("C1", C.c_int32), ("C2", C.c_int32),
        ("pix1", C.c_int32), ("pix2", C.c_int32),
        ("B", C.c_int32), ("H", C.c_int32), ("W", C.c_int32),
        ("up_h", C.c_int32), ("up_w", C.c_int32),
        ("KH", C.c_int32), ("KW", C.c_int32), ("SH", C.c_int32), ("SW", C.c_int32),
        ("PH", C.c_int32), ("PW", C.c_int32), ("DH", C.c_int32), ("DW", C.c_int32),
        ("OH", C.c_int32), ("OW", C.c_int32),
        ("pre_scale", C.c_void_p), ("pre_shift", C.c_void_p),
        ("pre_act", C.c_int32), ("pre_slope", C.c_float),
        ("w", C.c_void_p),
        ("b_mode", C.c_int32), ("ldb", C.c_int32),
        ("K", C.c_int32), ("N", C.c_int32),
        ("bias", C.c_void_p), ("rowbias", C.c_void_p), ("res", C.c_void_p), ("out", C.c_void_p),
        ("ldo", C.c_int32), ("act", C.c_int32), ("act_slope", C.c_float), ("alpha", C.c_float),
        ("accumulate", C.c_int32),
        ("out_mul", C.c_int32), ("out_off", C.c_int32), ("out_len", C.c_int32),
        ("batch", C.c_int32),
        ("stride_x", C.c_int64), ("stride_w", C.c_int64), ("stride_o", C.c_int64),
        ("rowbias_ld", C.c_int32), ("epi_mode", C.c_int32),
        ("ws", C.c_void_p), ("ws_floats", C.c_int64),
        ("hint_bm", C.c_int32), ("hint_bn", C.c_int32), ("hint_splits", C.c_int32), ("hint_kgroups", C.c_int32),
        ("w_split", C.c_void_p), ("hint_mma", C.c_int32), ("hint_stages", C.c_int32),
        ("a_split", C.c_void_p), ("out_split", C.c_void_p), ("out_split_c", C.c_int32), ("split_parts", C.c_int32),
        ("out_split_act", C.c_int32), ("out_split_slope", C.c_float),
        ("k_split", C.c_void_p), ("vt_split", C.c_void_p), ("qkv_c", C.c_int32), ("qkv_rows", C.c_int32),
        ("a_fmt", C.c_int32), ("acc_scale", C.c_float), ("out_split_parts", C.c_int32),
        ("out_split_fmt", C.c_int32), ("out_split_scale", C.c_float), ("vt_scale", C.c_float),
    ]


_SIGS = {
    "aldm_version": (C.c_int, []),
    "aldm_last_error": (C.c_char_p, []),
    "aldm_igemm": (C.c_int, [C.POINTER(IgemmDesc), C.c_void_p]),
    "aldm_igemm_plan": (C.c_int, [C.POINTER(IgemmDesc), C.POINTER(C.c_int), C.POINTER(C.c_int),
                                  C.POINTER(C.c_int64), C.POINTER(C.c_int), C.POINTER(C.c_int),
                                  C.POINTER(C.c_int)]),
    "aldm_igemm_ws_floats": (C.c_int64, [C.POINTER(IgemmDesc)]),
    "aldm_igemm_plan_stages": (C.c_int, [C.POINTER(IgemmDesc)]),
    "aldm_igemm_force": (None, [C.c_int, C.c_int, C.c_int, C.c_int]),
    "aldm_igemm_force_stages": (None, [C.c_int]),
    "aldm_igemm_wave8_mask": (C.c_int, [C.c_int]),
    "aldm_split_image_bytes": (C.c_int64, [C.c_int64, C.c_int, C.c_int]),
    "aldm_split_rows": (C.c_int, [C.c_void_p, C.c_void_p, C.c_int, C.c_int, C.c_int64, C.c_int, C.c_void_p, C.c_void_p,
                                  C.c_int, C.c_void_p, C.c_void_p, C.c_int, C.c_void_p]),
    "aldm_split_rows_act": (C.c_int, [C.c_void_p, C.c_void_p, C.c_int, C.c_int, C.c_int64, C.c_int, C.c_void_p, C.c_void_p,
                                      C.c_int, C.c_float, C.c_void_p, C.c_void_p, C.c_int, C.c_void_p]),
    "aldm_layernorm_split": (C.c_int, [C.c_void_p, C.c_void_p, C.c_void_p, C.c_int, C.c_int, C.c_void_p, C.c_void_p,
                                       C.c_float, C.c_int, C.c_void_p]),
    "aldm_attention_d32_split": (C.c_int, [C.c_void_p, C.c_void_p, C.c_void_p, C.c_void_p, C.c_void_p, C.c_int, C.c_int,
                                           C.c_int, C.c_int, C.c_int, C.c_int, C.c_int, C.c_int, C.c_int,
                                           C.c_void_p, C.c_float, C.c_void_p]),
    "aldm_split_bytes_parts": (C.c_int64, [C.c_int, C.c_int, C.c_int]),
    "aldm_pack_split_bf16_parts": (C.c_int, [C.c_void_p, C.c_void_p, C.c_int, C.c_int, C.c_int, C.c_void_p]),
    "aldm_pack_split_f16": (C.c_int, [C.c_void_p, C.c_void_p, C.c_int, C.c_int, C.c_float, C.c_void_p]),
    "aldm_split_rows_f16": (C.c_int, [C.c_void_p, C.c_void_p, C.c_int, C.c_int, C.c_int64, C.c_int, C.c_void_p, C.c_void_p,
                                      C.c_int, C.c_float, C.c_void_p, C.c_void_p, C.c_int, C.c_float, C.c_void_p]),
    "aldm_groupnorm_split_f16": (C.c_int, [C.c_void_p, C.c_void_p, C.c_int, C.c_int, C.c_int, C.c_int, C.c_int, C.c_float,
                                           C.c_void_p, C.c_void_p, C.c_int, C.c_void_p, C.c_void_p, C.c_void_p, C.c_void_p,
                                           C.c_void_p, C.c_int, C.c_float, C.c_void_p]),
    "aldm_layernorm_split_f16": (C.c_int, [C.c_void_p, C.c_void_p, C.c_void_p, C.c_int, C.c_int, C.c_void_p, C.c_void_p,
                                           C.c_float, C.c_float, C.c_void_p]),
    "aldm_igemm_mma": (C.c_int, [C.c_int]),
    "aldm_split_bytes": (C.c_int64, [C.c_int, C.c_int]),
    "aldm_pack_split_bf16": (C.c_int, [C.c_void_p, C.c_void_p, C.c_int, C.c_int, C.c_void_p]),
    "aldm_pack_weight": (C.c_int, [C.c_void_p, C.c_void_p, C.c_int, C.c_int, C.c_int, C.c_int,
                                   C.c_int, C.c_int, C.c_int, C.c_void_p]),
    "aldm_pack_kn": (C.c_int, [C.c_void_p, C.c_void_p, C.c_int, C.c_int, C.c_int, C.c_int,
                               C.c_int64, C.c_int64, C.c_void_p]),
    "aldm_groupnorm_stats": (C.c_int, [C.c_void_p, C.c_void_p, C.c_int, C.c_int, C.c_int, C.c_int,
                                       C.c_int, C.c_float, C.c_void_p, C.c_void_p, C.c_void_p,
                                       C.c_void_p, C.c_void_p, C.c_void_p]),
    "aldm_gn_ws_floats": (C.c_int64, [C.c_int, C.c_int, C.c_int, C.c_int]),
    "aldm_groupnorm_split": (C.c_int, [C.c_void_p, C.c_void_p, C.c_int, C.c_int, C.c_int, C.c_int, C.c_int, C.c_float,
                                       C.c_void_p, C.c_void_p, C.c_int, C.c_void_p, C.c_void_p, C.c_void_p, C.c_void_p,
                                       C.c_void_p, C.c_int, C.c_void_p]),
    "aldm_layernorm": (C.c_int, [C.c_void_p, C.c_void_p, C.c_int, C.c_int, C.c_void_p, C.c_void_p,
                                 C.c_float, C.c_void_p]),
    "aldm_attention_mma": (C.c_int, [C.c_int]),
    "aldm_attention_sched": (C.c_int, [C.c_int]),
    "aldm_attention_query_tiles": (C.c_int, [C.c_int, C.c_int, C.c_int]),
    "aldm_attention_d32_presplit_f16": (C.c_int, [C.c_void_p, C.c_void_p, C.c_void_p, C.c_void_p, C.c_void_p, C.c_int, C.c_float,
                                                  C.c_int, C.c_int, C.c_int, C.c_int, C.c_int, C.c_int, C.c_float, C.c_float,
                                                  C.c_float, C.c_float, C.c_void_p]),
    "aldm_attention_d32_presplit": (C.c_int, [C.c_void_p, C.c_void_p, C.c_void_p, C.c_void_p, C.c_void_p, C.c_int, C.c_int,
                                              C.c_int, C.c_int, C.c_int, C.c_int, C.c_int, C.c_float, C.c_void_p]),
    "aldm_vt_regroup": (C.c_int, [C.c_void_p, C.c_void_p, C.c_int, C.c_int, C.c_int, C.c_int, C.c_void_p]),
    "aldm_attention_d32": (C.c_int, [C.c_void_p, C.c_void_p, C.c_void_p, C.c_void_p, C.c_int,
                                     C.c_int, C.c_int, C.c_int, C.c_int, C.c_int, C.c_int, C.c_int,
                                     C.c_void_p, C.c_float, C.c_void_p]),
    "aldm_rel_attention": (C.c_int, [C.c_void_p, C.c_void_p, C.c_void_p, C.c_void_p, C.c_int, C.c_int, C.c_int, C.c_int,
                                     C.c_int, C.c_int, C.c_int, C.c_int, C.c_void_p, C.c_void_p, C.c_int, C.c_void_p,
                                     C.c_void_p]),
    "aldm_rowscale_add": (C.c_int, [C.c_void_p, C.c_void_p, C.c_void_p, C.c_void_p, C.c_int64, C.c_int, C.c_int, C.c_void_p]),
    "aldm_rmsnorm": (C.c_int, [C.c_void_p, C.c_void_p, C.c_int, C.c_int, C.c_void_p, C.c_float, C.c_void_p]),
    "aldm_softmax_rows_bias": (C.c_int, [C.c_void_p, C.c_void_p, C.c_int, C.c_int, C.c_int, C.c_int, C.c_float, C.c_void_p,
                                         C.c_void_p, C.c_void_p]),
    "aldm_resample_sinc": (C.c_int, [C.c_void_p, C.c_void_p, C.c_void_p, C.c_int, C.c_int, C.c_int, C.c_int, C.c_int, C.c_int,
                                     C.c_int, C.c_void_p]),
    "aldm_power_spec": (C.c_int, [C.c_void_p, C.c_void_p, C.c_int64, C.c_int, C.c_int, C.c_int, C.c_void_p]),
    "aldm_col_affine": (C.c_int, [C.c_void_p, C.c_void_p, C.c_void_p, C.c_void_p, C.c_int64, C.c_int, C.c_void_p]),
    "aldm_bicubic_patchify": (C.c_int, [C.c_void_p, C.c_void_p, C.c_int, C.c_int, C.c_int, C.c_int, C.c_int, C.c_void_p]),
    "aldm_token_mean": (C.c_int, [C.c_void_p, C.c_void_p, C.c_int, C.c_int, C.c_int, C.c_void_p]),
    "aldm_row_cosine": (C.c_int, [C.c_void_p, C.c_void_p, C.c_void_p, C.c_int, C.c_int, C.c_float, C.c_void_p]),
    "aldm_decode_linear": (C.c_int, [C.c_void_p, C.c_int, C.c_int, C.c_int, C.c_void_p, C.c_int, C.c_void_p, C.c_void_p,
                                     C.c_void_p, C.c_float, C.c_int, C.c_void_p, C.c_int, C.c_void_p, C.c_int, C.c_void_p]),
    "aldm_decode_attention": (C.c_int, [C.c_void_p, C.c_int, C.c_void_p, C.c_void_p, C.c_void_p, C.c_void_p, C.c_int, C.c_int,
                                        C.c_int, C.c_float, C.c_void_p, C.c_int, C.c_void_p]),
    "aldm_decode_gemv_slices": (C.c_int, [C.c_int, C.c_int]),
    "aldm_decode_gemv": (C.c_int, [C.c_void_p, C.c_int, C.c_int, C.c_int64, C.c_void_p, C.c_int, C.c_int, C.c_int, C.c_void_p,
                                   C.c_int, C.c_void_p, C.c_void_p]),
    "aldm_decode_reduce_ln": (C.c_int, [C.c_void_p, C.c_int, C.c_int64, C.c_int, C.c_void_p, C.c_void_p, C.c_void_p, C.c_int,
                                        C.c_int, C.c_int, C.c_void_p, C.c_int, C.c_void_p, C.c_void_p, C.c_float, C.c_void_p,
                                        C.c_int, C.c_void_p, C.c_int, C.c_void_p]),
    "aldm_decode_attention_parts": (C.c_int, [C.c_void_p, C.c_int, C.c_int, C.c_int64, C.c_void_p, C.c_void_p, C.c_void_p,
                                              C.c_void_p, C.c_void_p, C.c_int, C.c_int, C.c_int, C.c_float, C.c_void_p, C.c_int,
                                              C.c_void_p]),
    "aldm_softmax_rows_masked": (C.c_int, [C.c_void_p, C.c_void_p, C.c_int, C.c_int, C.c_int, C.c_int, C.c_float,
                                           C.c_void_p, C.c_int, C.c_void_p]),
    "aldm_softmax_rows": (C.c_int, [C.c_void_p, C.c_void_p, C.c_int64, C.c_int, C.c_float,
                                    C.c_void_p]),
    "aldm_geglu": (C.c_int, [C.c_void_p, C.c_void_p, C.c_int64, C.c_int, C.c_void_p]),
    "aldm_timestep_embedding": (C.c_int, [C.c_void_p, C.c_void_p, C.c_int, C.c_int, C.c_float,
                                          C.c_void_p]),
    "aldm_nchw_to_nhwc": (C.c_int, [C.c_void_p, C.c_void_p, C.c_int, C.c_int, C.c_int, C.c_int,
                                    C.c_void_p]),
    "aldm_nhwc_to_nchw": (C.c_int, [C.c_void_p, C.c_void_p, C.c_int, C.c_int, C.c_int, C.c_void_p]),
    "aldm_ddim_step": (C.c_int, [C.c_void_p, C.c_void_p, C.c_void_p, C.c_void_p, C.c_void_p,
                                 C.c_void_p, C.c_int64, C.c_void_p]),
    "aldm_ddim_step_indexed": (C.c_int, [C.c_void_p, C.c_void_p, C.c_void_p, C.c_void_p, C.c_void_p, C.c_void_p, C.c_int64,
                                         C.c_int, C.c_void_p]),
    "aldm_plms_first_step": (C.c_int, [C.c_void_p, C.c_void_p, C.c_void_p, C.c_void_p, C.c_void_p, C.c_void_p, C.c_void_p,
                                       C.c_int64, C.c_void_p]),
    "aldm_plms_step_indexed": (C.c_int, [C.c_void_p, C.c_void_p, C.c_void_p, C.c_void_p, C.c_void_p, C.c_void_p, C.c_int64,
                                         C.c_int, C.c_void_p]),
    "aldm_dpmpp_step_indexed": (C.c_int, [C.c_void_p, C.c_void_p, C.c_void_p, C.c_void_p, C.c_void_p, C.c_int64, C.c_int,
                                          C.c_void_p]),
    "aldm_step_advance": (C.c_int, [C.c_void_p, C.c_void_p, C.c_void_p, C.c_int, C.c_int, C.c_void_p]),
    "aldm_ddpm_step": (C.c_int, [C.c_void_p, C.c_void_p, C.c_void_p, C.c_void_p, C.c_void_p, C.c_int64,
                                 C.c_void_p]),
    "aldm_inpaint_blend": (C.c_int, [C.c_void_p, C.c_void_p, C.c_void_p, C.c_void_p, C.c_void_p,
                                     C.c_int64, C.c_void_p]),
    "aldm_axpby": (C.c_int, [C.c_void_p, C.c_void_p, C.c_void_p, C.c_float, C.c_float, C.c_int64,
                             C.c_void_p]),
    "aldm_reflect_pad_1d": (C.c_int, [C.c_void_p, C.c_void_p, C.c_int, C.c_int, C.c_int, C.c_int,
                                      C.c_void_p]),
    "aldm_mag_phase": (C.c_int, [C.c_void_p, C.c_void_p, C.c_void_p, C.c_int64, C.c_int, C.c_int,
                                 C.c_int, C.c_void_p]),
    "aldm_row_l2norm": (C.c_int, [C.c_void_p, C.c_void_p, C.c_int64, C.c_int, C.c_int, C.c_void_p]),
}

EXPORTED_SYMBOLS = tuple(_SIGS.keys())
TEST_HOOK_SIGS = {"aldm_debug_drop_product": (C.c_int, [C.c_int])}
TESTHOOKS_LIB_PATH = os.path.join(_HERE, "libaldm_hip_testhooks.so")

_lib = None


def source_hash(family: str = "all") -> str:
    import glob
    import hashlib
    h = hashlib.sha256()
    files = sorted(glob.glob(os.path.join(_HERE, "csrc", "*.hip")) + glob.glob(os.path.join(_HERE, "csrc", "*.h")) +
                   glob.glob(os.path.join(os.path.dirname(_HERE), "include", "*.h")))
    if family == "igemm":
        files = [f for f in files if os.path.basename(f).startswith("igemm") or os.path.basename(f) in ("common.h", "aldm_hip.h")]
    elif family != "all":
        raise ValueError(f"source_hash: unknown family {family!r}")
    for f in files:
        h.update(os.path.basename(f).encode())
        with open(f, "rb") as fh:
            h.update(fh.read())
    return h.hexdigest()[:16]


def tuning_hash() -> str:
    import glob
    import hashlib
    h = hashlib.sha256()
    for f in sorted(glob.glob(os.path.join(_HERE, "tuning", "*.json"))):
        h.update(os.path.basename(f).encode())
        with open(f, "rb") as fh:
            h.update(fh.read())
    return h.hexdigest()[:16]


def load():
    global _lib
    if _lib is not None:
        return _lib
    if not os.path.exists(LIB_PATH):
        raise RuntimeError(
            f"{LIB_PATH} is missing: the HIP kernel library has not been built. Run "
            "`python -c 'import __graft_entry__ as g; g.build()'` (or `make -C audioldm2_amd/csrc`). "
            "There is no CPU fallback for the sampling hot path."
        )
    lib = C.CDLL(LIB_PATH)
    for name, (res, args) in _SIGS.items():
        fn = getattr(lib, name)
        fn.restype = res
        fn.argtypes = args
    for name, (res, args) in TEST_HOOK_SIGS.items():
        fn = getattr(lib, name, None)
        if fn is not None:
            fn.restype = res
            fn.argtypes = args
    ver = lib.aldm_version()
    if ver != ABI_VERSION:
        raise RuntimeError(f"libaldm_hip.so ABI version {ver} != expected {ABI_VERSION}; rebuild")
    _lib = lib
    return lib


def check(rc: int, what: str = ""):
    if rc != 0:
        msg = load().aldm_last_error().decode("utf-8", "replace")
        raise RuntimeError(f"libaldm_hip {what} failed ({rc}): {msg}")
```

audioldm2_amd/ops.py:

```python
from __future__ import annotations

import ctypes as C
import json
import os
from dataclasses import dataclass
from typing import List, Optional, Sequence, Tuple

import torch

from . import lib as _l
from .lib import (ACT_GELU, ACT_GELU_TANH, ACT_LOGCLAMP, ACT_LRELU, ACT_NONE, ACT_SILU, ACT_TANH, B_NT, B_PACKED,
                  IgemmDesc)


def _stream() -> int:
    return torch.cuda.current_stream().cuda_stream


def _p(t: Optional[torch.Tensor]):
    return None if t is None else t.data_ptr()


def _chk(t: torch.Tensor, name: str):
    if not (t.is_cuda and t.dtype == torch.float32 and t.is_contiguous()):
# ... 211 lines not shown

    @property
    def device(self):
        return self.data.device

    def data_ptr(self) -> int:
        return self.data.data_ptr()

    def view(self, *shape) -> "SplitT":
        shape = tuple(shape[0]) if len(shape) == 1 and isinstance(shape[0], (tuple, list)) else tuple(shape)
        n = 1
        for s_ in shape:
            n *= abs(s_)
        tot = self.rows * self.C
        shape = tuple(tot // n if s_ == -1 else s_ for s_ in shape)
        assert shape[-1] == self.C, "a split image can only be re-viewed over its row dimensions"
        return SplitT(self.data, shape, self.fmt, self.scale, self.rn, self.rt)

    def float(self) -> torch.Tensor:
        if self.fmt == "f16":
            h = self.data.view(torch.float16).float()
            return ((h[:, :, 0] + h[:, :, 1]) / self.scale).reshape(self.shape)
        parts = (self.data.to(torch.int32) << 16).view(torch.float32)
        acc = parts[:, :, 0] + parts[:, :, 1]
        if self.parts == 3:
            acc = acc + parts[:, :, 2]
        return acc.reshape(self.shape)


DMA_MODE = os.environ.get("ALDM_DMA", "1") != "0"


def set_dma(on: bool) -> bool:
    global DMA_MODE
    prev, DMA_MODE = DMA_MODE, bool(on)
    return prev


def use_dma() -> bool:
    return DMA_MODE and MMA_MODE in ("bf16x6", "bf16x3", "f16x3")


def split_rows(x: torch.Tensor, x2: Optional[torch.Tensor] = None, pre=None, act: int = ACT_NONE,
               want_raw: bool = False, slope: float = 0.0):
    _chk(x, "split_rows.x")
    C1 = x.shape[-1]
    C2 = 0
    if x2 is not None:
        _chk(x2, "split_rows.x2")
        assert x2.shape[:-1] == x.shape[:-1]
        C2 = x2.shape[-1]
    shape = (*x.shape[:-1], C1 + C2)
    rows = x.numel() // C1
    P = rows // x.shape[0]
    dst = SplitT.empty(shape, x.device)
    raw = SplitT.empty(shape, x.device) if want_raw else None
    sc = sh = None
    if pre is not None:
        sc, sh = pre
        assert sc.shape == (x.shape[0], C1 + C2) and sc.is_contiguous() and sh.is_contiguous()
    _l.check(_l.load().aldm_split_rows_act(x.data_ptr(), _p(x2), C1, C2, rows, P, _p(sc), _p(sh), act, slope, dst.data_ptr(),
                                           None if raw is None else raw.data_ptr(), dst.parts, _stream()), "split_rows")
    return (dst, raw) if want_raw else dst


PROFILE = None
ATTN_PROFILE = None


_ws = {}
_ws_retired = []
WS_SLOT = 0


def _workspace(lib, d: IgemmDesc, device) -> None:
    need = lib.aldm_igemm_ws_floats(C.byref(d))
    if need <= 0:
        return
    key = (device.index if device.index is not None else torch.cuda.current_device(), WS_SLOT)
    buf = _ws.get(key)
    if buf is None or buf.numel() < need:
        if torch.cuda.is_current_stream_capturing():
            return
        if buf is not None:
            _ws_retired.append(buf)
        buf = torch.empty(max(need, 8 << 20), device=device, dtype=torch.float32)
        _ws[key] = buf
    d.ws = buf.data_ptr()
    d.ws_floats = buf.numel()


_TUNE_FIELDS = ("B", "H", "W", "C1", "C2", "pix1", "up_h", "up_w", "KH", "KW", "SH", "SW", "PH", "PW", "DH", "DW",
                "OH", "OW", "N", "b_mode", "batch", "epi_mode", "out_mul")
_TUNED = None
TUNE_LOG = None


def tune_key(d: IgemmDesc) -> str:
    return ",".join(str(getattr(d, f)) for f in _TUNE_FIELDS) + f",{_pre_mode(d)}" + \
        (("," + ("dma2" if d.split_parts == 2 else "dma")) if d.a_split else "")


def _tuned_table(bx=False):
    global _TUNED
    if _TUNED is None:
        _TUNED = {False: {}, True: {}, "dma": {}, "dma2": {}}
        if os.environ.get("ALDM_NO_TUNING", "0") != "1":
            for mode, name in ((False, "mi355x_igemm.json"), (True, "mi355x_igemm_bf16x6.json"),
                               ("dma", "mi355x_igemm_dma.json"), ("dma2", "mi355x_igemm_dma_bf16x3.json")):
                path = os.path.join(os.environ.get("ALDM_TUNING_DIR", ""), name)
                if not (os.environ.get("ALDM_TUNING_DIR") and os.path.exists(path)):
                    path = os.path.join(os.path.dirname(os.path.abspath(__file__)), "tuning", name)
                if os.path.exists(path):
                    with open(path) as f:
                        _TUNED[mode] = {k: v[:5] if mode is True else v[:4] for k, v in json.load(f)["entries"].items()}
    return _TUNED[bx]


def _set_split_operand(d: IgemmDesc, x: "SplitT", pw: "Packed", so: Optional["SplitT"] = None) -> None:
    d.a_split = x.data_ptr()
    d.split_parts = x.parts
    if x.fmt == "f16":
        d.a_fmt = _l.FMT_F16
        d.w_split = pw.split16_ptr()
        d.acc_scale = 1.0 / (x.scale * pw.w_scale)
        d.out_split_parts = so.parts if so is not None else 3
    else:
        d.w_split = pw.split_ptr(x.parts)
        if so is not None:
            assert so.parts == x.parts and so.fmt == "bf16"


def _igemm(d: IgemmDesc, what: str, device=None):
    lib = _l.load()
    if d.a_split and d.epi_mode == _l.EPI_QKV:
        d.epi_mode = _l.EPI_PLAIN
        key = tune_key(d)
        d.epi_mode = _l.EPI_QKV
    else:
        key = tune_key(d)
    key_t = key
    if TUNE_LOG is not None:
        TUNE_LOG.append(key)
    if d.a_split:
        hint = _tuned_table("dma2" if d.split_parts == 2 else "dma").get(key_t)
        if hint is not None:
            d.hint_bm, d.hint_bn, d.hint_splits, d.hint_stages = hint[:4]
    else:
        hint = _tuned_table(bool(d.w_split)).get(key)
        if hint is not None:
            d.hint_bm, d.hint_bn, d.hint_splits, d.hint_kgroups = hint[:4]
            d.hint_mma = hint[4] if len(hint) > 4 else 0
    _workspace(lib, d, device if device is not None else torch.device("cuda", torch.cuda.current_device()))
    if PROFILE is None:
        _l.check(lib.aldm_igemm(C.byref(d), _stream()), what)
        return
    bm, bn, fl, sp, kg, mma = C.c_int(), C.c_int(), C.c_int64(), C.c_int(), C.c_int(), C.c_int()
    _l.check(lib.aldm_igemm_plan(C.byref(d), C.byref(bm), C.byref(bn), C.byref(fl), C.byref(sp), C.byref(kg),
                                 C.byref(mma)), what)
    e0 = torch.cuda.Event(enable_timing=True)
    e1 = torch.cuda.Event(enable_timing=True)
    e0.record()
    _l.check(lib.aldm_igemm(C.byref(d), _stream()), what)
    e1.record()
    shape = (d.B * d.OH * d.OW, d.N, d.K, d.KH * d.KW, d.C2, int(bool(d.pre_scale)), d.pre_act, d.batch,
             sp.value * 10 + kg.value, int(bool(d.a_split)), int(bool(d.out)), int(bool(d.out_split)), d.split_parts or 3,
             int(d.epi_mode == _l.EPI_GEGLU), int(bool(d.res)))
    PROFILE.append((what, bm.value, bn.value, fl.value, e0, e1, shape,
                    _kernel_name(d, bm.value, bn.value, kg.value, bool(mma.value))))


def _pre_mode(d: IgemmDesc) -> int:
    if not d.pre_scale and d.pre_act == ACT_NONE:
        return 0
    if d.pre_scale and d.pre_act == ACT_NONE:
        return 1
    if d.pre_scale and d.pre_act == ACT_SILU:
        return 2
    if not d.pre_scale and d.pre_act == ACT_LRELU:
        return 3
    return 4


def _kernel_name(d: IgemmDesc, bm: int, bn: int, kg: int = 1, bx: bool = False) -> str:
    if d.a_split:
        nst = _l.load().aldm_igemm_plan_stages(C.byref(d))
        if nst >= 400:
            w8 = (nst - 400) // 10
            return f"igemm_dma_halo_kernel<{bm}, {bn}, {(nst - 400) % 10}, {4 if (bm == 256 or w8) else 2}, {d.split_parts or 3}>"
        if nst >= 300:
            epi = 1 if d.epi_mode == _l.EPI_GEGLU else (2 if d.epi_mode == _l.EPI_QKV else 0)
            return f"igemm_dma_os_kernel<{d.K // 32}, {nst - 300}, {d.split_parts or 3}, {epi}>"
        if nst >= 200:
            return f"igemm_dma_lw_kernel<{bm}, {bn}, {nst - 200}, {4 if bm == 256 else 2}, {d.split_parts or 3}>"
        if nst >= 100:
            return f"igemm_dma_ws_kernel<{bm}, {bn}, {nst - 100}, {d.split_parts or 3}>"
        return f"igemm_dma_kernel<{bm}, {bn}, {nst}, {4 if bm == 256 else 2}, {d.split_parts or 3}>"
    pre = _pre_mode(d)
    wm, wn = (4, 1) if bn == 32 else (2, 2)
    w8 = _wave8_mask if _wave8_mask >= 0 else int(os.environ.get("ALDM_IGEMM_W8", "1"))
    bit = {(128, 128): 1, (64, 128): 2, (128, 64): 4}.get((bm, bn), 0)
    if kg == 1 and d.epi_mode != _l.EPI_GEGLU and (w8 & bit) and (
            bit == 1 if bx else (pre in (1, 2) or (bit == 1 and (w8 & 8)))):
        wm, wn = (4, 2) if bit == 4 else (2, 4)
    if bx and (bm, bn) == (128, 128) and d.epi_mode == _l.EPI_GEGLU and pre == 0:
        wm, wn = 4, 2
    uni = "true" if pre in (1, 2) and (d.OH * d.OW) % bm == 0 else "false"
    return f"igemm_kernel<{bm}, {bn}, {wm}, {wn}, {pre}, {kg}, {uni}, {'true' if bx else 'false'}>"


def igemm_force(bm: int = 0, bn: int = 0, splits: int = 0, kgroups: int = 0, stages: int = 0) -> None:
    _l.load().aldm_igemm_force(bm, bn, splits, kgroups)
    _l.load().aldm_igemm_force_stages(stages)


def attention_mma(mode: int) -> int:
    return _l.load().aldm_attention_mma(mode)


def attention_sched(sched: int) -> int:
    return _l.load().aldm_attention_sched(sched)


def attention_query_tiles(B: int, heads: int, Lq: int) -> int:
    return _l.load().aldm_attention_query_tiles(B, heads, Lq)


def debug_drop_product(on: bool) -> bool:
    fn = getattr(_l.load(), "aldm_debug_drop_product", None)
    if fn is None:
        raise RuntimeError("aldm_debug_drop_product is a test hook of libaldm_hip_testhooks.so; the release library does not "
                           f"export it (run with ALDM_LIB_PATH={_l.TESTHOOKS_LIB_PATH})")
    return bool(fn(1 if on else 0))


def igemm_mma(mode: int) -> int:
    return _l.load().aldm_igemm_mma(mode)


_wave8_mask = -1


def igemm_wave8(mask: int = -1) -> int:
    global _wave8_mask
    _wave8_mask = mask
    return _l.load().aldm_igemm_wave8_mask(mask)


def _npad(n: int) -> int:
    return (n + 31) // 32 * 32


def pack_conv(weight: torch.Tensor, bias: Optional[torch.Tensor] = None) -> Packed:
    w = weight.detach().to(device="cuda", dtype=torch.float32).contiguous()
    if w.dim() == 2:
        N, Cin, KH, KW = w.shape[0], w.shape[1], 1, 1
    elif w.dim() == 3:
        N, Cin, KH, KW = w.shape[0], w.shape[1], 1, w.shape[2]
    else:
        N, Cin, KH, KW = w.shape
    K = KH * KW * Cin
    dst = torch.empty(((K + 3) // 4) * _npad(N) * 4, device="cuda", dtype=torch.float32)
    lib = _l.load()
    _l.check(lib.aldm_pack_weight(w.data_ptr(), dst.data_ptr(), N, Cin, KH, KW, 0, 0, 1, _stream()),
             "pack_weight")
    b = None if bias is None else bias.detach().to(device="cuda", dtype=torch.float32).contiguous()
    return Packed(dst, N, Cin, KH, KW, b)


def pack_geglu(weight: torch.Tensor, bias: Optional[torch.Tensor]) -> Packed:
    two_inner = weight.shape[0]
    inner = two_inner // 2
    assert weight.dim() == 2 and two_inner % 64 == 0
    g = torch.arange(inner // 32).view(-1, 1, 1)
    j = torch.arange(2).view(1, -1, 1)
    l = torch.arange(32).view(1, 1, -1)
    perm = (j * inner + g * 32 + l).reshape(-1).to(weight.device)
    pw = pack_conv(weight.detach()[perm], None if bias is None else bias.detach()[perm])
    pw.geglu = True
    return pw


def linear_geglu(x, pw: Packed, split_out: Optional[str] = None, gate_act: int = ACT_NONE,
                 out: Optional[torch.Tensor] = None):
    is_split = isinstance(x, SplitT)
    if not is_split:
        _chk(x, "linear_geglu.x")
    shp = x.shape
    M = (x.rows if is_split else x.numel() // shp[-1])
    assert shp[-1] == pw.Cin and pw.KH == 1 and pw.KW == 1 and pw.N % 64 == 0
    oshape = (*shp[:-1], pw.N // 2)
    if split_out == "only":
        assert out is None
    elif out is None:
        out = torch.empty(oshape, device=x.device, dtype=torch.float32)
    else:
        _chk(out, "linear_geglu.out")
        assert out.numel() == M * (pw.N // 2), (out.shape, oshape)
        out = out.view(oshape)
    so = None
    if split_out:
        if is_split and x.fmt == "f16" and x.rn > 0.0 and f16_mode() and F16_FF_OUT:
            if pw.geglu:
                bound, typ = pw.geglu_bound(x.rn, x.rt)
            else:
                bound, typ = pw.out_bound(x.rn) ** 2, 0.0
            if typ <= 0.0 or bound <= typ * 2.0 ** F16_GEGLU_MAX_SLACK_LOG2:
                so = SplitT.empty(oshape, x.device, f16_scale=_pow2_scale(bound))
        if so is None:
            so = SplitT.empty(oshape, x.device)
    d = IgemmDesc()
    if is_split:
        _set_split_operand(d, x, pw, so if (so is None or so.fmt == "bf16") else None)
        if so is not None and so.fmt == "f16":
            d.out_split_fmt = _l.FMT_F16; d.out_split_scale = so.scale
    else:
        d.x1 = x.data_ptr(); d.split_parts = 3
        d.w_split = pw.split_ptr(3)
    if so is not None and not is_split:
        d.split_parts = so.parts
    d.C1 = pw.Cin; d.B = 1; d.H = 1; d.W = M; d.up_h = d.up_w = 1
    d.KH = d.KW = d.SH = d.SW = d.DH = d.DW = 1
    d.OH = 1; d.OW = M
    d.w = pw.data.data_ptr(); d.b_mode = B_PACKED; d.K = pw.K; d.N = pw.N
    d.bias = _p(pw.bias); d.out = _p(out); d.ldo = pw.N // 2; d.alpha = 1.0
    if so is not None:
        d.out_split = so.data_ptr(); d.out_split_c = pw.N // 2
    d.epi_mode = _l.EPI_GEGLU; d.batch = 1
    d.act = gate_act
    _igemm(d, "igemm(geglu)")
    return so if split_out == "only" else ((out, so) if split_out else out)


def linear_qkv(x: "SplitT", pw: Packed, heads: int, rows_per_sample: int):
    assert isinstance(x, SplitT) and pw.KH == 1 and pw.KW == 1 and pw.bias is None
    Cq = heads * 32
    assert pw.N == 3 * Cq and x.shape[-1] == pw.Cin
    M = x.rows
    assert M % rows_per_sample == 0
    Bn = M // rows_per_sample
    ragged = rows_per_sample % 32 != 0
    f16_kv = x.fmt == "f16" and x.rn > 0.0 and f16_mode() and F16_ATTN
    P = 2 if f16_kv else (3 if x.fmt == "f16" else x.parts)
    dev = x.device
    q = torch.empty((*x.shape[:-1], Cq), device=dev, dtype=torch.float32)
    if ragged:
        k_img = torch.empty((M + 31, heads, P, 32), device=dev, dtype=torch.int16)[:M]
        vt_img = torch.empty((Bn, heads, -(-rows_per_sample // 32), P, 32, 32), device=dev, dtype=torch.int16)
        vt_raw = torch.empty((heads, -(-M // 32), P, 32, 32), device=dev, dtype=torch.int16)
    else:
        k_img = torch.empty((M, heads, P, 32), device=dev, dtype=torch.int16)
        vt_img = torch.empty((Bn, heads, rows_per_sample // 32, P, 32, 32), device=dev, dtype=torch.int16)
    d = IgemmDesc()
    _set_split_operand(d, x, pw)
    d.out_split_parts = P
    if f16_kv:
        bound = pw.out_bound(x.rn)
        kv_scale = _pow2_scale(bound)
        q_scale = _pow2_scale(bound * (32 ** -0.5) * 1.4426950408889634)
        d.out_split_fmt = _l.FMT_F16; d.out_split_scale = kv_scale; d.vt_scale = kv_scale
        k_img._aldm_f16 = vt_img._aldm_f16 = (q_scale, kv_scale, kv_scale)
    d.C1 = pw.Cin; d.B = 1; d.H = 1; d.W = M; d.up_h = d.up_w = 1
    d.KH = d.KW = d.SH = d.SW = d.DH = d.DW = 1
    d.OH = 1; d.OW = M
    d.w = pw.data.data_ptr(); d.b_mode = B_PACKED; d.K = pw.K; d.N = pw.N
    d.out = q.data_ptr(); d.ldo = Cq; d.alpha = 1.0
    d.k_split = k_img.data_ptr(); d.vt_split = vt_img.data_ptr(); d.qkv_c = Cq; d.qkv_rows = rows_per_sample
    if ragged:
        d.vt_split = vt_raw.data_ptr(); d.qkv_rows = vt_raw.shape[1] * 32
    d.epi_mode = _l.EPI_QKV; d.batch = 1
    _igemm(d, "igemm(qkv)")
    if ragged:
        _l.check(_l.load().aldm_vt_regroup(vt_raw.data_ptr(), vt_img.data_ptr(), Bn, rows_per_sample, heads, P, _stream()),
                 "vt_regroup")
    return q, k_img, vt_img


def attention_presplit(q: torch.Tensor, k_img: torch.Tensor, vt_img: torch.Tensor, heads: int, *,
                       scale: Optional[float] = None, split_out: Optional[str] = None):
    qp, Lq, ldq = _rowview(q, "attn_pre.q")
    B = q.shape[0]
    Lk = k_img.shape[0] // B
    parts = k_img.shape[2]
    assert q.shape[2] == heads * 32 and k_img.shape[1] == heads and vt_img.shape[0] == B and vt_img.shape[2] == -(-Lk // 32)
    if scale is None:
        scale = 32 ** -0.5
    out = None if split_out == "only" else torch.empty((B, Lq, heads * 32), device=q.device, dtype=torch.float32)
    f16s = getattr(k_img, "_aldm_f16", None) or getattr(vt_img, "_aldm_f16", None)
    if f16s is None and parts == 2 and f16_mode():
        raise RuntimeError("attention_presplit: a 2-part K / V^T image without its fp16 scales in f16x3 mode (the scales are an "
                           "attribute of the tensors linear_qkv returned: pass those, not a view or a clone of them)")
    f16_out = f16s is not None and F16_ATTN_OUT
    so = None
    if split_out:
        so = SplitT.empty((B, Lq, heads * 32), q.device, f16_scale=f16s[2]) if f16_out else \
            SplitT.empty((B, Lq, heads * 32), q.device, 3 if f16s is not None else parts)
    ev = None
    if ATTN_PROFILE is not None:
        ev = (torch.cuda.Event(enable_timing=True), torch.cuda.Event(enable_timing=True))
        ev[0].record()
    if f16s is not None:
        assert abs(scale - 32 ** -0.5) < 1e-12, "the fp16 images' q scale was chosen for the default softmax scale"
        _l.check(_l.load().aldm_attention_d32_presplit_f16(qp, k_img.data_ptr(), vt_img.data_ptr(), _p(out),
                                                           None if so is None else so.data_ptr(),
                                                           3 if so is None else (0 if so.fmt == "f16" else so.parts),
                                                           0.0 if so is None or so.fmt != "f16" else so.scale, B, heads,
                                                           Lq, Lk, ldq, heads * 32, scale, f16s[0], f16s[1], f16s[2], _stream()),
                 "attention_d32_presplit_f16")
    else:
        _l.check(_l.load().aldm_attention_d32_presplit(qp, k_img.data_ptr(), vt_img.data_ptr(), _p(out),
                                                       None if so is None else so.data_ptr(), parts, B, heads, Lq, Lk, ldq,
                                                       heads * 32, scale, _stream()), "attention_d32_presplit")
    if ev is not None:
        ev[1].record()
        ATTN_PROFILE.append((B, heads, Lq, Lk, False, 4.0 * B * heads * Lq * Lk * 32, ev[0], ev[1]))
    if not split_out:
        return out
    return so if split_out == "only" else (out, so)


def pack_convtr1d(weight: torch.Tensor, bias: Optional[torch.Tensor], stride: int) -> List[Packed]:
    w = weight.detach().to(device="cuda", dtype=torch.float32).contiguous()
    Cin, N, KW = w.shape
    T = (KW + stride - 1) // stride
    lib = _l.load()
    b = None if bias is None else bias.detach().to(device="cuda", dtype=torch.float32).contiguous()
    out = []
    for ph in range(stride):
        dst = torch.empty(((T * Cin + 3) // 4) * _npad(N) * 4, device="cuda", dtype=torch.float32)
        _l.check(lib.aldm_pack_weight(w.data_ptr(), dst.data_ptr(), N, Cin, 1, KW, 1, ph, stride,
                                      _stream()), "pack_weight(tr)")
        out.append(Packed(dst, N, Cin, 1, T, b))
    return out


def conv(x: torch.Tensor, pw: Packed, *, stride=(1, 1), pad=(0, 0), dil=(1, 1), up=(1, 1),
         x2: Optional[torch.Tensor] = None, out_hw: Optional[Tuple[int, int]] = None,
         pre: Optional[Tuple[torch.Tensor, torch.Tensor]] = None, pre_act: int = ACT_NONE,
         pre_slope: float = 0.0, bias: Optional[torch.Tensor] = None,
         rowbias: Optional[torch.Tensor] = None, res: Optional[torch.Tensor] = None,
         act: int = ACT_NONE, act_slope: float = 0.0, alpha: float = 1.0,
         out: Optional[torch.Tensor] = None, accumulate: bool = False,
         remap: Optional[Tuple[int, int, int]] = None,
         use_pw_bias: bool = True, split_out: Optional[str] = None, split_act: int = ACT_NONE, split_slope: float = 0.0):
    is_split = isinstance(x, SplitT)
    if is_split:
        assert x2 is None and pre is None and pre_act == ACT_NONE, "a pre-split operand takes no prologue"
    else:
        _chk(x, "conv.x")
    B, H, W, C1 = x.shape
    C2 = 0
    if x2 is not None:
        _chk(x2, "conv.x2")
        assert x2.shape[:3] == x.shape[:3]
        C2 = x2.shape[3]
    assert C1 + C2 == pw.Cin, f"channels {C1}+{C2} != packed Cin {pw.Cin}"
    VH, VW = H * up[0], W * up[1]
    if out_hw is None:
        OH = (VH + 2 * pad[0] - dil[0] * (pw.KH - 1) - 1) // stride[0] + 1
        OW = (VW + 2 * pad[1] - dil[1] * (pw.KW - 1) - 1) // stride[1] + 1
    else:
        OH, OW = out_hw
    N = pw.N
    if remap is not None:
        out_mul, out_off, out_len = remap
        oshape = (B, 1, out_len, N)
    else:
        out_mul = out_off = out_len = 0
        oshape = (B, OH, OW, N)
    if split_out == "only":
        assert out is None and not accumulate
    elif out is None:
        assert not accumulate
        out = torch.empty(oshape, device=x.device, dtype=torch.float32)
    else:
        _chk(out, "conv.out")
        assert out.numel() == oshape[0] * oshape[1] * oshape[2] * oshape[3], (out.shape, oshape)
    so = SplitT.empty(oshape, x.device) if split_out else None
    if bias is None and use_pw_bias:
        bias = pw.bias
    d = IgemmDesc()
    if is_split:
        _set_split_operand(d, x, pw, so)
    else:
        d.x1 = x.data_ptr(); d.split_parts = so.parts if so is not None else 3
    d.x2 = _p(x2)
    d.C1 = C1; d.C2 = C2; d.pix1 = 0; d.pix2 = 0
    d.B = B; d.H = H; d.W = W; d.up_h = up[0]; d.up_w = up[1]
    d.KH = pw.KH; d.KW = pw.KW; d.SH = stride[0]; d.SW = stride[1]
    d.PH = pad[0]; d.PW = pad[1]; d.DH = dil[0]; d.DW = dil[1]
    d.OH = OH; d.OW = OW
    if pre is not None:
        d.pre_scale = pre[0].data_ptr(); d.pre_shift = pre[1].data_ptr()
    d.pre_act = pre_act; d.pre_slope = pre_slope
    d.w = pw.data.data_ptr(); d.b_mode = B_PACKED; d.ldb = 0
    if not is_split:
        d.w_split = pw.split_ptr(3)
    d.K = pw.K; d.N = N
    d.bias = _p(bias); d.rowbias = _p(rowbias); d.res = _p(res); d.out = _p(out)
    if so is not None:
        d.out_split = so.data_ptr(); d.out_split_c = N
        d.out_split_act = split_act; d.out_split_slope = split_slope
    if rowbias is not None:
        if not (rowbias.dim() == 2 and rowbias.stride(1) == 1 and rowbias.shape == (B, N)):
            raise RuntimeError("conv.rowbias: need a [B, N] fp32 view with unit inner stride")
        d.rowbias_ld = rowbias.stride(0)
    d.ldo = N; d.act = act; d.act_slope = act_slope; d.alpha = alpha
    d.accumulate = 1 if accumulate else 0
    d.out_mul = out_mul; d.out_off = out_off; d.out_len = out_len
    d.batch = 1
    _igemm(d, "igemm(conv)")
    if split_out == "only":
        return so
    return (out.view(oshape), so) if split_out else out.view(oshape)


def linear(x, pw: Packed, **kw):
    shp = x.shape
    if isinstance(x, SplitT):
        M = x.rows
        y = conv(x.view(1, 1, M, shp[-1]), pw, **kw)
    else:
        M = x.numel() // shp[-1]
        y = conv(x.reshape(1, 1, M, shp[-1]), pw, **kw)
    oshape = (*shp[:-1], pw.N)
    if isinstance(y, tuple):
        return y[0].view(oshape), y[1].view(oshape)
    return y.view(oshape)


def _view3(t: torch.Tensor, name: str):
    if not (t.is_cuda and t.dtype == torch.float32 and t.dim() == 3 and t.stride(2) == 1):
        raise RuntimeError(f"{name}: need a [Z, R, D] fp32 CUDA view with unit inner stride")
    return t.data_ptr(), t.stride(0), t.stride(1)


def gemm_nt(a: torch.Tensor, bmat: torch.Tensor, *, alpha: float = 1.0,
            out: Optional[torch.Tensor] = None) -> torch.Tensor:
    ap, sa, lda = _view3(a, "gemm_nt.a")
    bp, sb, ldb = _view3(bmat, "gemm_nt.b")
    Z, M, K = a.shape
    Zb, N, Kb = bmat.shape
    assert Z == Zb and K == Kb and K % 4 == 0
    if out is None:
        out = torch.empty((Z, M, N), device=a.device, dtype=torch.float32)
    d = IgemmDesc()
    d.x1 = ap; d.C1 = K; d.pix1 = lda; d.B = 1; d.H = 1; d.W = M; d.up_h = d.up_w = 1
    d.KH = d.KW = d.SH = d.SW = d.DH = d.DW = 1
    d.OH = 1; d.OW = M
    d.w = bp; d.b_mode = B_NT; d.ldb = ldb; d.K = K; d.N = N
    d.out = out.data_ptr(); d.ldo = N; d.alpha = alpha
    d.batch = Z; d.stride_x = sa; d.stride_w = sb; d.stride_o = M * N
    _igemm(d, "igemm(nt)")
    return out


def pack_kn(src: torch.Tensor) -> torch.Tensor:
    sp, ss, lds = _view3(src, "pack_kn.src")
    Z, K, N = src.shape
    per = ((K + 3) // 4) * _npad(N) * 4
    dst = torch.empty((Z, per), device=src.device, dtype=torch.float32)
    _l.check(_l.load().aldm_pack_kn(sp, dst.data_ptr(), K, N, lds, Z, ss, per, _stream()), "pack_kn")
    return dst


def gemm_packed_batched(a: torch.Tensor, bp: torch.Tensor, K: int, N: int, *,
                        out: Optional[torch.Tensor] = None) -> torch.Tensor:
    _chk(a, "gemm_packed.a")
    Z, M, Ka = a.shape
    assert Ka == K and K % 4 == 0
    if out is None:
        out = torch.empty((Z, M, N), device=a.device, dtype=torch.float32)
    d = IgemmDesc()
    d.x1 = a.data_ptr(); d.C1 = K; d.B = 1; d.H = 1; d.W = M; d.up_h = d.up_w = 1
    d.KH = d.KW = d.SH = d.SW = d.DH = d.DW = 1
    d.OH = 1; d.OW = M
    d.w = bp.data_ptr(); d.b_mode = B_PACKED; d.ldb = 0; d.K = K; d.N = N
    d.out = out.data_ptr(); d.ldo = N; d.alpha = 1.0
    d.batch = Z; d.stride_x = M * K; d.stride_w = bp.shape[1]; d.stride_o = M * N
    _igemm(d, "igemm(packed batched)")
    return out


_gn_ws = {}


def gn_stats(x: torch.Tensor, gamma: torch.Tensor, beta: torch.Tensor, *, groups: int = 32,
             eps: float = 1e-5, x2: Optional[torch.Tensor] = None):
    _chk(x, "gn.x")
    B = x.shape[0]
    C1 = x.shape[-1]
    P = x.numel() // (B * C1)
    C2 = 0
    if x2 is not None:
        _chk(x2, "gn.x2")
        C2 = x2.shape[-1]
    Cc = C1 + C2
    lib = _l.load()
    nws = lib.aldm_gn_ws_floats(B, P, Cc, groups)
    ws = torch.empty(nws, device=x.device, dtype=torch.float32)
    ss = torch.empty((2, B, Cc), device=x.device, dtype=torch.float32)
    _l.check(lib.aldm_groupnorm_stats(x.data_ptr(), _p(x2), B, P, C1, C2, groups, eps,
                                      gamma.data_ptr(), beta.data_ptr(), ss[0].data_ptr(),
                                      ss[1].data_ptr(), ws.data_ptr(), _stream()), "groupnorm_stats")
    return ss[0], ss[1]


def gn_split(x: torch.Tensor, gamma: torch.Tensor, beta: torch.Tensor, *, groups: int = 32, eps: float = 1e-5,
             x2: Optional[torch.Tensor] = None, act: int = ACT_NONE, want_raw: bool = False):
    _chk(x, "gn_split.x")
    B = x.shape[0]
    C1 = x.shape[-1]
    P = x.numel() // (B * C1)
    C2 = 0
    if x2 is not None:
        _chk(x2, "gn_split.x2")
        assert x2.shape[:-1] == x.shape[:-1]
        C2 = x2.shape[-1]
    Cc = C1 + C2
    lib = _l.load()
    ws = torch.empty(lib.aldm_gn_ws_floats(B, P, Cc, groups), device=x.device, dtype=torch.float32)
    ss = torch.empty((2, B, Cc), device=x.device, dtype=torch.float32)
    shape = (*x.shape[:-1], Cc)
    raw = SplitT.empty(shape, x.device) if want_raw else None
    if f16_mode():
        dst = SplitT.empty(shape, x.device, f16_scale=_norm_f16_scale(gamma, beta, (Cc // groups) * P))
        _l.check(lib.aldm_groupnorm_split_f16(x.data_ptr(), _p(x2), B, P, C1, C2, groups, eps, gamma.data_ptr(), beta.data_ptr(), act,
                                              ss[0].data_ptr(), ss[1].data_ptr(), ws.data_ptr(), dst.data_ptr(),
                                              None if raw is None else raw.data_ptr(), 3, dst.scale, _stream()), "groupnorm_split_f16")
        return (dst, raw) if want_raw else dst
    dst = SplitT.empty(shape, x.device)
    _l.check(lib.aldm_groupnorm_split(x.data_ptr(), _p(x2), B, P, C1, C2, groups, eps, gamma.data_ptr(), beta.data_ptr(), act,
                                      ss[0].data_ptr(), ss[1].data_ptr(), ws.data_ptr(), dst.data_ptr(),
                                      None if raw is None else raw.data_ptr(), dst.parts, _stream()), "groupnorm_split")
    return (dst, raw) if want_raw else dst


def layernorm(x: torch.Tensor, gamma: torch.Tensor, beta: torch.Tensor, eps: float = 1e-5,
              split_out: Optional[str] = None):
    _chk(x, "ln.x")
    Cc = x.shape[-1]
    M = x.numel() // Cc
    y = None if split_out == "only" else torch.empty_like(x)
    if not split_out:
        _l.check(_l.load().aldm_layernorm(x.data_ptr(), y.data_ptr(), M, Cc, gamma.data_ptr(),
                                          beta.data_ptr(), eps, _stream()), "layernorm")
        return y
    if f16_mode():
        so = SplitT.empty(x.shape, x.device, f16_scale=_norm_f16_scale(gamma, beta, Cc))
        so.rn = _row_norm_bound(gamma, beta, Cc)
        so.rt = _row_norm_typical(gamma, beta)
        _l.check(_l.load().aldm_layernorm_split_f16(x.data_ptr(), _p(y), so.data_ptr(), M, Cc, gamma.data_ptr(), beta.data_ptr(), eps,
                                                    so.scale, _stream()), "layernorm_split_f16")
        return so if split_out == "only" else (y, so)
    so = SplitT.empty(x.shape, x.device)
    _l.check(_l.load().aldm_layernorm_split(x.data_ptr(), _p(y), so.data_ptr(), M, Cc, gamma.data_ptr(),
                                            beta.data_ptr(), eps, so.parts, _stream()), "layernorm_split")
    return so if split_out == "only" else (y, so)


def _rowview(t: torch.Tensor, name: str):
    if not (t.is_cuda and t.dtype == torch.float32 and t.dim() == 3 and t.stride(2) == 1
            and t.stride(0) == t.shape[1] * t.stride(1)):
        raise RuntimeError(f"{name}: need [B, L, D] fp32 CUDA view with unit inner stride")
    return t.data_ptr(), t.shape[1], t.stride(1)


def attention(q: torch.Tensor, k: torch.Tensor, v: torch.Tensor, heads: int, *,
              mask: Optional[torch.Tensor] = None, scale: Optional[float] = None,
              split_out: Optional[str] = None):
    qp, Lq, ldq = _rowview(q, "attn.q")
    kp, Lk, ldk = _rowview(k, "attn.k")
    vp, Lv, ldv = _rowview(v, "attn.v")
    assert Lk == Lv and q.shape[2] == heads * 32
    B = q.shape[0]
    if scale is None:
        scale = 32 ** -0.5
    out = None if split_out == "only" else torch.empty((B, Lq, heads * 32), device=q.device, dtype=torch.float32)
    if mask is not None:
        mask = mask.to(torch.float32).reshape(B, Lk).contiguous()
    ev = None
    if ATTN_PROFILE is not None:
        ev = (torch.cuda.Event(enable_timing=True), torch.cuda.Event(enable_timing=True))
        ev[0].record()
    if not split_out:
        _l.check(_l.load().aldm_attention_d32(qp, kp, vp, out.data_ptr(), B, heads, Lq, Lk, ldq, ldk, ldv,
                                              heads * 32, _p(mask), scale, _stream()), "attention_d32")
        res = out
    else:
        so = SplitT.empty((B, Lq, heads * 32), q.device)
        _l.check(_l.load().aldm_attention_d32_split(qp, kp, vp, _p(out), so.data_ptr(), so.parts, B, heads, Lq, Lk, ldq,
                                                    ldk, ldv, heads * 32, _p(mask), scale, _stream()), "attention_d32_split")
        res = so if split_out == "only" else (out, so)
    if ev is not None:
        ev[1].record()
        ATTN_PROFILE.append((B, heads, Lq, Lk, mask is not None, 4.0 * B * heads * Lq * Lk * 32, ev[0], ev[1]))
    return res


def rmsnorm(x: torch.Tensor, weight: torch.Tensor, eps: float = 1e-6) -> torch.Tensor:
    _chk(x, "rmsnorm.x")
    Cc = x.shape[-1]
    y = torch.empty_like(x)
    _l.check(_l.load().aldm_rmsnorm(x.data_ptr(), y.data_ptr(), x.numel() // Cc, Cc, weight.data_ptr(), eps, _stream()),
             "rmsnorm")
    return y


def softmax_rows_bias(x: torch.Tensor, bias: torch.Tensor, keymask: torch.Tensor, scale: float = 1.0) -> torch.Tensor:
    _chk(x, "softmax_bias.x"); _chk(bias, "softmax_bias.bias"); _chk(keymask, "softmax_bias.keymask")
    B, heads, q_rows, N = x.shape
    assert bias.shape == (heads, q_rows, N) and keymask.shape == (B, N)
    y = torch.empty_like(x)
    _l.check(_l.load().aldm_softmax_rows_bias(x.data_ptr(), y.data_ptr(), B, heads, q_rows, N, scale, bias.data_ptr(),
                                              keymask.data_ptr(), _stream()), "softmax_rows_bias")
    return y


def rel_attention(q: torch.Tensor, k: torch.Tensor, v: torch.Tensor, heads: int, emb_k: torch.Tensor, emb_v: torch.Tensor,
                  mask: torch.Tensor) -> torch.Tensor:
    qp, T, ldq = _rowview(q, "rel_attn.q")
    kp, Tk, ldk = _rowview(k, "rel_attn.k")
    vp, Tv, ldv = _rowview(v, "rel_attn.v")
    B = q.shape[0]
    d = q.shape[2] // heads
    assert T == Tk == Tv and emb_k.shape == emb_v.shape and emb_k.shape[1] == d and emb_k.shape[0] % 2 == 1
    _chk(emb_k, "rel_attn.emb_k"); _chk(emb_v, "rel_attn.emb_v"); _chk(mask, "rel_attn.mask")
    assert mask.shape == (B, T)
    out = torch.empty((B, T, heads * d), device=q.device, dtype=torch.float32)
    _l.check(_l.load().aldm_rel_attention(qp, kp, vp, out.data_ptr(), B, heads, T, d, ldq, ldk, ldv, heads * d,
                                          emb_k.data_ptr(), emb_v.data_ptr(), emb_k.shape[0] // 2, mask.data_ptr(),
                                          _stream()), "rel_attention")
    return out


def rowscale_add(x: torch.Tensor, s: torch.Tensor, res: Optional[torch.Tensor] = None, divide: bool = False) -> torch.Tensor:
    _chk(x, "rowscale.x"); _chk(s, "rowscale.s")
    Cc = x.shape[-1]
    rows = x.numel() // Cc
    assert s.numel() == rows
    if res is not None:
        _chk(res, "rowscale.res")
        assert res.shape == x.shape
    y = torch.empty_like(x)
    _l.check(_l.load().aldm_rowscale_add(x.data_ptr(), s.data_ptr(), _p(res), y.data_ptr(), rows, Cc, 1 if divide else 0,
                                         _stream()), "rowscale_add")
    return y


def resample_sinc(x: torch.Tensor, kernel: torch.Tensor, down: int, up: int, width: int, out_len: int) -> torch.Tensor:
    _chk(x, "resample.x"); _chk(kernel, "resample.kernel")
    B, T = x.shape
    assert kernel.shape[0] == up
    y = torch.empty((B, out_len), device=x.device, dtype=torch.float32)
    _l.check(_l.load().aldm_resample_sinc(x.data_ptr(), kernel.data_ptr(), y.data_ptr(), B, T, out_len, down, up,
                                          kernel.shape[1], width, _stream()), "resample_sinc")
    return y


def power_spec(spec: torch.Tensor, F: int, ld_out: int) -> torch.Tensor:
    _chk(spec, "power_spec.spec")
    M = spec.numel() // spec.shape[-1]
    out = torch.empty((M, ld_out), device=spec.device, dtype=torch.float32)
    _l.check(_l.load().aldm_power_spec(spec.data_ptr(), out.data_ptr(), M, F, spec.shape[-1], ld_out, _stream()),
             "power_spec")
    return out


def col_affine(x: torch.Tensor, scale: torch.Tensor, shift: torch.Tensor) -> torch.Tensor:
    _chk(x, "col_affine.x"); _chk(scale, "col_affine.scale"); _chk(shift, "col_affine.shift")
    Cc = x.shape[-1]
    assert scale.numel() == Cc and shift.numel() == Cc
    y = torch.empty_like(x)
    _l.check(_l.load().aldm_col_affine(x.data_ptr(), scale.data_ptr(), shift.data_ptr(), y.data_ptr(), x.numel() // Cc, Cc,
                                       _stream()), "col_affine")
    return y


def bicubic_patchify(x: torch.Tensor, S: int, p: int) -> torch.Tensor:
    _chk(x, "bicubic_patchify.x")
    B, T, Fm = x.shape
    out = torch.empty((B, (S // p) ** 2, p * p), device=x.device, dtype=torch.float32)
    _l.check(_l.load().aldm_bicubic_patchify(x.data_ptr(), out.data_ptr(), B, T, Fm, S, p, _stream()), "bicubic_patchify")
    return out
# ... 348 lines not shown
```

audioldm2_amd/unet.py:

```python
from __future__ import annotations

from typing import List, Optional

import torch
import torch.nn as nn

import os

from . import ops
from .ops import ACT_NONE, ACT_SILU

PRESPLIT_ATTENTION = os.environ.get("ALDM_ATTN_PRESPLIT", "1") != "0" and "ALDM_ATTN_MMA" not in os.environ


class ResBlock(nn.Module):

    def __init__(self, channels, emb_channels, dropout, out_channels=None):
        super().__init__()
        self.channels = channels
        self.out_channels = out_channels or channels
        self.in_layers = nn.Sequential(nn.GroupNorm(32, channels), nn.SiLU(),
                                       nn.Conv2d(channels, self.out_channels, 3, padding=1))
        self.emb_layers = nn.Sequential(nn.SiLU(), nn.Linear(emb_channels, self.out_channels))
        self.out_layers = nn.Sequential(nn.GroupNorm(32, self.out_channels), nn.SiLU(), nn.Dropout(p=dropout),
                                        nn.Conv2d(self.out_channels, self.out_channels, 3, padding=1))
        if self.out_channels == channels:
            self.skip_connection = nn.Identity()
        else:
            self.skip_connection = nn.Conv2d(channels, self.out_channels, 1)
        self._pk = None

    def _prepare(self):
        if self._pk is None:
            c1, c2 = self.in_layers[2], self.out_layers[3]
            self._pk = dict(
                gn1=(self.in_layers[0].weight.detach().float().cuda().contiguous(),
                     self.in_layers[0].bias.detach().float().cuda().contiguous()),
                gn2=(self.out_layers[0].weight.detach().float().cuda().contiguous(),
                     self.out_layers[0].bias.detach().float().cuda().contiguous()),
                conv1=ops.pack_conv(c1.weight, c1.bias),
                conv2=ops.pack_conv(c2.weight, c2.bias),
                skip=None if isinstance(self.skip_connection, nn.Identity)
                else ops.pack_conv(self.skip_connection.weight, self.skip_connection.bias),
            )
        return self._pk

    def run(self, x, e, x2=None):
        pk = self._prepare()
        c2 = 0 if x2 is None else x2.shape[-1]
        if ops.use_dma() and self.channels % 32 == 0 and x.shape[-1] % 8 == 0 and c2 % 8 == 0:
            if pk["skip"] is None:
                assert x2 is None
                a1, skip = ops.gn_split(x, *pk["gn1"], groups=32, eps=1e-5, act=ACT_SILU), x
            else:
                a1, araw = ops.gn_split(x, *pk["gn1"], groups=32, eps=1e-5, x2=x2, act=ACT_SILU, want_raw=True)
                skip = ops.conv(araw, pk["skip"])
            h = ops.conv(a1, pk["conv1"], pad=(1, 1), rowbias=e)
            a2 = ops.gn_split(h, *pk["gn2"], groups=32, eps=1e-5, act=ACT_SILU)
            return ops.conv(a2, pk["conv2"], pad=(1, 1), res=skip)
        sc, sh = ops.gn_stats(x, *pk["gn1"], groups=32, eps=1e-5, x2=x2)
        h = ops.conv(x, pk["conv1"], x2=x2, pad=(1, 1), pre=(sc, sh), pre_act=ACT_SILU, rowbias=e)
        sc2, sh2 = ops.gn_stats(h, *pk["gn2"], groups=32, eps=1e-5)
        if pk["skip"] is None:
            assert x2 is None
            skip = x
        else:
            skip = ops.conv(x, pk["skip"], x2=x2)
        return ops.conv(h, pk["conv2"], pad=(1, 1), pre=(sc2, sh2), pre_act=ACT_SILU, res=skip)


class Downsample(nn.Module):

    def __init__(self, channels, use_conv=True, dims=2, out_channels=None, padding=1):
        super().__init__()
        assert use_conv and dims == 2
        self.channels = channels
        self.out_channels = out_channels or channels
        self.op = nn.Conv2d(channels, self.out_channels, 3, stride=2, padding=padding)
        self._pk = None

    def run(self, x):
        if self._pk is None:
            self._pk = ops.pack_conv(self.op.weight, self.op.bias)
        if ops.use_dma() and self.channels % 32 == 0:
            x = ops.split_rows(x)
        return ops.conv(x, self._pk, stride=(2, 2), pad=(1, 1))


class Upsample(nn.Module):

    def __init__(self, channels, use_conv=True, dims=2, out_channels=None, padding=1):
        super().__init__()
        assert use_conv and dims == 2
        self.channels = channels
        self.out_channels = out_channels or channels
        self.conv = nn.Conv2d(channels, self.out_channels, 3, padding=padding)
        self._pk = None

    def run(self, x):
        if self._pk is None:
            self._pk = ops.pack_conv(self.conv.weight, self.conv.bias)
        if ops.use_dma() and self.channels % 32 == 0:
            x = ops.split_rows(x)
        return ops.conv(x, self._pk, pad=(1, 1), up=(2, 2))


class GEGLU(nn.Module):
    def __init__(self, dim_in, dim_out):
        super().__init__()
        self.proj = nn.Linear(dim_in, dim_out * 2)


class FeedForward(nn.Module):

    def __init__(self, dim, mult=4, dropout=0.0):
        super().__init__()
        self.net = nn.Sequential(GEGLU(dim, dim * mult), nn.Dropout(dropout), nn.Linear(dim * mult, dim))


class CrossAttention(nn.Module):

    def __init__(self, query_dim, context_dim=None, heads=8, dim_head=64, dropout=0.0):
        super().__init__()
        inner = dim_head * heads
        self.heads = heads
        self.dim_head = dim_head
        self.scale = dim_head ** -0.5
        context_dim = query_dim if context_dim is None else context_dim
        self.to_q = nn.Linear(query_dim, inner, bias=False)
        self.to_k = nn.Linear(context_dim, inner, bias=False)
        self.to_v = nn.Linear(context_dim, inner, bias=False)
        self.to_out = nn.Sequential(nn.Linear(inner, query_dim), nn.Dropout(dropout))


class BasicTransformerBlock(nn.Module):

    def __init__(self, dim, n_heads, d_head, dropout=0.0, context_dim=None):
        super().__init__()
        assert d_head == 32, "the HIP attention kernel is specialised for head dim 32 (all AudioLDM2 configs)"
        self.attn1 = CrossAttention(dim, heads=n_heads, dim_head=d_head, dropout=dropout)
        self.ff = FeedForward(dim, dropout=dropout)
        self.attn2 = CrossAttention(dim, context_dim=context_dim, heads=n_heads, dim_head=d_head, dropout=dropout)
        self.norm1 = nn.LayerNorm(dim)
        self.norm2 = nn.LayerNorm(dim)
        self.norm3 = nn.LayerNorm(dim)
        self.heads = n_heads
        self.dim = dim
        self._pk = None
        self._kv = None

    def _context_kv(self, context, pk):
        for c in (self._kv or ()):
            if c[0] is context and c[1] == context._version:
                return c[2]
        kv = ops.linear(context, pk["kv2"])
        if not torch.cuda.is_current_stream_capturing():
            self._kv = [(context, context._version, kv)] + list(self._kv or ())[:1]
        return kv

    def _prepare(self):
        if self._pk is None:
            f = lambda t: t.detach().float().cuda().contiguous()
            a1, a2 = self.attn1, self.attn2
            self._pk = dict(
                ln=[(f(n.weight), f(n.bias)) for n in (self.norm1, self.norm2, self.norm3)],
                qkv1=ops.pack_conv(torch.cat([a1.to_q.weight, a1.to_k.weight, a1.to_v.weight], 0)),
                out1=ops.pack_conv(a1.to_out[0].weight, a1.to_out[0].bias),
                qkv2=ops.pack_conv(torch.cat([a2.to_q.weight, a2.to_k.weight, a2.to_v.weight], 0))
                if a2.to_k.weight.shape[1] == self.dim else None,
                q2=ops.pack_conv(a2.to_q.weight),
                kv2=ops.pack_conv(torch.cat([a2.to_k.weight, a2.to_v.weight], 0)),
                out2=ops.pack_conv(a2.to_out[0].weight, a2.to_out[0].bias),
                ff1=ops.pack_geglu(self.ff.net[0].proj.weight, self.ff.net[0].proj.bias),
                ff2=ops.pack_conv(self.ff.net[2].weight, self.ff.net[2].bias),
            )
        return self._pk

    def run(self, h, context=None, mask=None, want_split=False):
        pk = self._prepare()
        C = self.dim
        so = "only" if (ops.use_dma() and C % 32 == 0) else None
        n = ops.layernorm(h, *pk["ln"][0], split_out=so)
        pre = so is not None and PRESPLIT_ATTENTION and C % 64 == 0 and pk["qkv1"].bias is None
        if pre:
            q, kimg, vtimg = ops.linear_qkv(n, pk["qkv1"], self.heads, h.shape[1])
            a = ops.attention_presplit(q, kimg, vtimg, self.heads, split_out=so)
        else:
            qkv = ops.linear(n, pk["qkv1"])
            a = ops.attention(qkv[:, :, :C], qkv[:, :, C:2 * C], qkv[:, :, 2 * C:], self.heads, split_out=so)
        h = ops.linear(a, pk["out1"], res=h)
        n = ops.layernorm(h, *pk["ln"][1], split_out=so)
        if context is None:
            if pk["qkv2"] is None:
                raise RuntimeError("attn2 was built with a context_dim but no context was provided")
            if pre and pk["qkv2"].bias is None:
                q, kimg, vtimg = ops.linear_qkv(n, pk["qkv2"], self.heads, h.shape[1])
                a = ops.attention_presplit(q, kimg, vtimg, self.heads, split_out=so)
            else:
                qkv = ops.linear(n, pk["qkv2"])
                a = ops.attention(qkv[:, :, :C], qkv[:, :, C:2 * C], qkv[:, :, 2 * C:], self.heads, split_out=so)
        else:
            q = ops.linear(n, pk["q2"])
            kv = self._context_kv(context, pk)
            a = ops.attention(q, kv[:, :, :C], kv[:, :, C:], self.heads, mask=mask, split_out=so)
        h = ops.linear(a, pk["out2"], res=h)
        n = ops.layernorm(h, *pk["ln"][2], split_out=so)
        g = ops.linear_geglu(n, pk["ff1"], split_out=so)
        if want_split and so:
            return ops.linear(g, pk["ff2"], res=h, split_out="also")
        return ops.linear(g, pk["ff2"], res=h)


class SpatialTransformer(nn.Module):

    def __init__(self, in_channels, n_heads, d_head, depth=1, dropout=0.0, context_dim=None):
        super().__init__()
        self.in_channels = in_channels
        inner = n_heads * d_head
        self.norm = nn.GroupNorm(32, in_channels, eps=1e-6, affine=True)
        self.proj_in = nn.Conv2d(in_channels, inner, 1)
        self.transformer_blocks = nn.ModuleList(
            [BasicTransformerBlock(inner, n_heads, d_head, dropout=dropout, context_dim=context_dim)
             for _ in range(depth)])
        self.proj_out = nn.Conv2d(inner, in_channels, 1)
        self._pk = None

    def run(self, x, context=None, mask=None):
        if self._pk is None:
            self._pk = dict(gn=(self.norm.weight.detach().float().cuda().contiguous(),
                                self.norm.bias.detach().float().cuda().contiguous()),
                            pin=ops.pack_conv(self.proj_in.weight, self.proj_in.bias),
                            pout=ops.pack_conv(self.proj_out.weight, self.proj_out.bias))
        pk = self._pk
        B, H, W, C = x.shape
        if ops.use_dma() and C % 32 == 0 and self.proj_in.out_channels % 32 == 0:
            h = ops.conv(ops.gn_split(x, *pk["gn"], groups=32, eps=1e-6), pk["pin"]).view(B, H * W, -1)
            hs = None
            for i, blk in enumerate(self.transformer_blocks):
                r = blk.run(h, context, mask, want_split=i == len(self.transformer_blocks) - 1)
                h, hs = r if isinstance(r, tuple) else (r, None)
            return ops.conv((hs if hs is not None else h).view(B, H, W, -1), pk["pout"], res=x)
        sc, sh = ops.gn_stats(x, *pk["gn"], groups=32, eps=1e-6)
        h = ops.conv(x, pk["pin"], pre=(sc, sh)).view(B, H * W, -1)
        for blk in self.transformer_blocks:
            h = blk.run(h, context, mask)
        return ops.conv(h.view(B, H, W, -1), pk["pout"], res=x)


class TimestepEmbedSequential(nn.Sequential):

    def run(self, x, emb, context_list, mask_list, x2=None, lo=0, hi=None):
        ctxs = [None] + list(context_list)
        masks = [None] + list(mask_list)
        layers = list(self)
        st_id = sum(isinstance(l, SpatialTransformer) for l in layers[:lo])
        for layer in layers[lo:hi]:
            if isinstance(layer, ResBlock):
                x = layer.run(x, emb[layer._emb_slice], x2)
                x2 = None
            elif isinstance(layer, SpatialTransformer):
                if st_id >= len(ctxs):
                    c, m = None, None
                else:
                    c, m = ctxs[st_id], masks[st_id]
                x = layer.run(x, c, m)
                st_id += 1
            elif isinstance(layer, (Downsample, Upsample)):
                x = layer.run(x)
            elif isinstance(layer, _ConvIn):
                x = layer.run(x)
            else:
                raise RuntimeError(f"unexpected layer {type(layer)}")
        assert x2 is None, "skip tensor was not consumed by a ResBlock"
        return x


class _EmbSlices:

    def __init__(self, t):
        self.t = t

    def __getitem__(self, sl):
        return self.t[:, sl]


class _ConvIn(nn.Conv2d):

    _pk = None

    def run(self, x):
        if self._pk is None:
            self._pk = ops.pack_conv(self.weight, self.bias)
        return ops.conv(x, self._pk, pad=(1, 1))


class UNetModel(nn.Module):

    def __init__(self, image_size, in_channels, model_channels, out_channels, num_res_blocks,
                 attention_resolutions, dropout=0, channel_mult=(1, 2, 4, 8), conv_resample=True, dims=2,
                 extra_sa_layer=True, num_classes=None, extra_film_condition_dim=None,
                 use_checkpoint=False, use_fp16=False, num_heads=-1, num_head_channels=-1,
                 num_heads_upsample=-1, use_scale_shift_norm=False, resblock_updown=False,
                 use_new_attention_order=False, use_spatial_transformer=True, transformer_depth=1,
                 context_dim=None, n_embed=None, legacy=True):
        super().__init__()
        if dims != 2 or use_scale_shift_norm or resblock_updown or not use_spatial_transformer \
                or n_embed is not None or num_classes is not None or use_fp16 or not conv_resample:
            raise NotImplementedError("UNetModel(HIP): only the option set used by the AudioLDM2 configs "
                                      "(utils.py:329-343) is implemented")
        if num_heads_upsample == -1:
            num_heads_upsample = num_heads
        assert num_heads != -1 or num_head_channels != -1, "Either num_heads or num_head_channels has to be set"
        self.image_size = image_size
        self.in_channels = in_channels
        self.model_channels = model_channels
        self.out_channels = out_channels
        self.num_res_blocks = num_res_blocks
        self.attention_resolutions = attention_resolutions
        self.channel_mult = channel_mult
        self.extra_film_condition_dim = extra_film_condition_dim
        self.use_extra_film_by_concat = extra_film_condition_dim is not None
        self.dtype = torch.float32
        ted = model_channels * 4
        self.time_embed = nn.Sequential(nn.Linear(model_channels, ted), nn.SiLU(), nn.Linear(ted, ted))
        if self.use_extra_film_by_concat:
            self.film_emb = nn.Linear(extra_film_condition_dim, ted)
        if context_dim is not None and not isinstance(context_dim, (list, tuple)):
            context_dim = [context_dim]
        elif context_dim is None:
            context_dim = [None]
        context_dim = list(context_dim)
        emb_ch = ted * 2 if self.use_extra_film_by_concat else ted

        def transformers(ch):
            if num_head_channels == -1:
                heads, dim_head = num_heads, ch // num_heads
            else:
                heads, dim_head = ch // num_head_channels, num_head_channels
            out = []
            if extra_sa_layer:
                out.append(SpatialTransformer(ch, heads, dim_head, depth=transformer_depth, context_dim=None))
            for cd in context_dim:
                out.append(SpatialTransformer(ch, heads, dim_head, depth=transformer_depth, context_dim=cd))
            return out

        self.input_blocks = nn.ModuleList(
            [TimestepEmbedSequential(_ConvIn(in_channels, model_channels, 3, padding=1))])
        chans = [model_channels]
        ch, ds = model_channels, 1
        for level, mult in enumerate(channel_mult):
            for _ in range(num_res_blocks):
                layers = [ResBlock(ch, emb_ch, dropout, out_channels=mult * model_channels)]
                ch = mult * model_channels
                if ds in attention_resolutions:
                    layers += transformers(ch)
                self.input_blocks.append(TimestepEmbedSequential(*layers))
                chans.append(ch)
            if level != len(channel_mult) - 1:
                self.input_blocks.append(TimestepEmbedSequential(Downsample(ch, True, out_channels=ch)))
                chans.append(ch)
                ds *= 2
        self.middle_block = TimestepEmbedSequential(
            ResBlock(ch, emb_ch, dropout), *transformers(ch), ResBlock(ch, emb_ch, dropout))
        self.output_blocks = nn.ModuleList([])
        for level, mult in list(enumerate(channel_mult))[::-1]:
            for i in range(num_res_blocks + 1):
                ich = chans.pop()
                layers = [ResBlock(ch + ich, emb_ch, dropout, out_channels=model_channels * mult)]
                ch = model_channels * mult
                if ds in attention_resolutions:
                    layers += transformers(ch)
                if level and i == num_res_blocks:
                    layers.append(Upsample(ch, True, out_channels=ch))
                    ds //= 2
                self.output_blocks.append(TimestepEmbedSequential(*layers))
        self.out = nn.Sequential(nn.GroupNorm(32, ch), nn.SiLU(),
                                 nn.Conv2d(model_channels, out_channels, 3, padding=1))
        self._pk = None
        self._graph_cache = {}
        self.register_load_state_dict_post_hook(lambda module, incompatible: module.invalidate_packed())

    def invalidate_packed(self):
        from .ddim import drop_graph_entries
        drop_graph_entries(self._graph_cache)
        for m in self.modules():
            if hasattr(m, "_pk"):
                m._pk = None
            if hasattr(m, "_kv"):
                m._kv = None

    def drop_step_caches(self):
        from .ddim import drop_graph_entries
        drop_graph_entries(self._graph_cache)
        for m in self.modules():
            if hasattr(m, "_kv"):
                m._kv = None

    def collect_context_kv(self, contexts):
        out = []
        for m in self.modules():
            if isinstance(m, BasicTransformerBlock) and m._kv:
                for ctx, _ver, kv in m._kv:
                    if any(ctx is c for c in contexts):
                        out.append((m, ctx, kv))
        return out

    def refresh_context_kv(self, entries):
        n = 0
        for m, ctx, kv in entries:
            pk = m._prepare()
            ops.linear(ctx, pk["kv2"], out=kv)
            m._kv = [(ctx, ctx._version, kv)] + [c for c in (m._kv or ()) if c[2] is not kv][:1]
            n += 1
        return n

    def _prepare(self):
        if self._pk is None:
            f = lambda t: t.detach().float().cuda().contiguous()
            rbs = [m for m in self.modules() if isinstance(m, ResBlock)]
            off = 0
            for m in rbs:
                m._emb_slice = slice(off, off + m.out_channels)
                off += m.out_channels
            self._pk = dict(
                emb_all=ops.pack_conv(torch.cat([m.emb_layers[1].weight for m in rbs], 0),
                                      torch.cat([m.emb_layers[1].bias for m in rbs], 0)),
                te0=ops.pack_conv(self.time_embed[0].weight, self.time_embed[0].bias),
                te2=ops.pack_conv(self.time_embed[2].weight, self.time_embed[2].bias),
                film=ops.pack_conv(self.film_emb.weight, self.film_emb.bias)
                if self.use_extra_film_by_concat else None,
                gn=(f(self.out[0].weight), f(self.out[0].bias)),
                out=ops.pack_conv(self.out[2].weight, self.out[2].bias),
            )
        return self._pk

    def _shared_prefix_end(self, context_list):
        if self.use_extra_film_by_concat:
            return None
        for bi, blk in enumerate(self.input_blocks):
            st = 0
            for li, layer in enumerate(blk):
                if isinstance(layer, SpatialTransformer):
                    if st >= 1 and st - 1 < len(context_list) and context_list[st - 1] is not None:
                        return bi, li
                    st += 1
        return None

    @torch.no_grad()
    def forward(self, x, timesteps=None, y=None, context_list=None, context_attn_mask_list=None, cfg_shared=False, **kwargs):
        assert (y is not None) == self.use_extra_film_by_concat, \
            "must specify y if and only if the model is class-conditional or film embedding conditional"
        if not x.is_cuda:
            raise RuntimeError("UNetModel(HIP) runs on the MI355X only; there is no CPU path")
        pk = self._prepare()
        context_list = [c.float().contiguous() if c is not None else None for c in (context_list or [])]
        mask_list = list(context_attn_mask_list or [])
        div = self._shared_prefix_end(context_list) if cfg_shared else None
        B = x.shape[0]
        if cfg_shared:
            assert timesteps.shape[0] in (B, 2 * B) and all(c is None or c.shape[0] == 2 * B for c in context_list), \
                "cfg_shared: x [B, ...] once, contexts for the 2B rows [uncond ; cond]"
            timesteps = timesteps[:B]
            if div is None:
                x = x.repeat(2, 1, 1, 1)
                timesteps = timesteps.repeat(2)
        t_emb = ops.timestep_embedding(timesteps, self.model_channels)
        emb = ops.linear(ops.linear(t_emb, pk["te0"], act=ACT_SILU), pk["te2"])
        if self.use_extra_film_by_concat:
            emb = torch.cat([emb, ops.linear(y.float().contiguous(), pk["film"])], dim=-1).contiguous()
        emb_rows = ops.linear(emb, pk["emb_all"], pre_act=ACT_SILU)
        emb = _EmbSlices(emb_rows)
        h = ops.nchw_to_nhwc(x.float().contiguous())
        hs = []
        if div is None:
            for module in self.input_blocks:
                h = module.run(h, emb, context_list, mask_list)
                hs.append(h)
        else:
            dup = lambda t: t.repeat(2, *([1] * (t.dim() - 1)))
            emb_half, emb = emb, _EmbSlices(dup(emb_rows))
            for bi, module in enumerate(self.input_blocks):
                if bi < div[0]:
                    h = module.run(h, emb_half, context_list, mask_list)
                elif bi == div[0]:
                    h = module.run(h, emb_half, context_list, mask_list, hi=div[1])
                    h = module.run(dup(h), emb, context_list, mask_list, lo=div[1])
                else:
                    h = module.run(h, emb, context_list, mask_list)
                hs.append(h)
        h = self.middle_block.run(h, emb, context_list, mask_list)
        for module in self.output_blocks:
            skip = hs.pop()
            if skip.shape[0] != h.shape[0]:
                skip = dup(skip)
            h = module.run(h, emb, context_list, mask_list, x2=skip)
        sc, sh = ops.gn_stats(h, *pk["gn"], groups=32, eps=1e-5)
        out = ops.conv(h, pk["out"], pad=(1, 1), pre=(sc, sh), pre_act=ACT_SILU)
        return ops.nhwc_to_nchw(out)
```

include/aldm_hip.h:

```cpp
#ifndef ALDM_HIP_H
#define ALDM_HIP_H

#include <stdint.h>

#ifdef __cplusplus
extern "C" {
#endif

int aldm_version(void);
const char* aldm_last_error(void);

enum {
    ALDM_ACT_NONE = 0,
    ALDM_ACT_SILU = 1,
    ALDM_ACT_LRELU = 2,
    ALDM_ACT_TANH = 3,
    ALDM_ACT_LOGCLAMP = 4,
    ALDM_ACT_GELU = 5,
    ALDM_ACT_GELU_TANH = 6
};

enum { ALDM_EPI_PLAIN = 0, ALDM_EPI_GEGLU = 1, ALDM_EPI_QKV = 2 };

enum {
    ALDM_B_PACKED = 0,
    ALDM_B_NT = 1
};

enum { ALDM_MMA_F32 = 0, ALDM_MMA_BF16X6 = 1 };

typedef struct aldm_igemm_desc {
    const float* x1;
    const float* x2;
    int32_t C1, C2;
    int32_t pix1, pix2;
    int32_t B, H, W;
    int32_t up_h, up_w;
    int32_t KH, KW, SH, SW, PH, PW, DH, DW;
    int32_t OH, OW;
    const float* pre_scale;
    const float* pre_shift;
    int32_t pre_act;
    float pre_slope;
    const float* w;
    int32_t b_mode;
    int32_t ldb;
    int32_t K, N;
    const float* bias;
    const float* rowbias;
    const float* res;
    float* out;
    int32_t ldo;
    int32_t act;
    float act_slope;
    float alpha;
    int32_t accumulate;
    int32_t out_mul, out_off, out_len;
    int32_t batch;
    int64_t stride_x, stride_w, stride_o;
    int32_t rowbias_ld;
    int32_t epi_mode;
    float* ws;
    int64_t ws_floats;
    int32_t hint_bm, hint_bn, hint_splits;
    int32_t hint_kgroups;
    const void* w_split;
    int32_t hint_mma;
    int32_t hint_stages;
    const void* a_split;
    void* out_split;
    int32_t out_split_c;
    int32_t split_parts;
    int32_t out_split_act;
    float out_split_slope;
    void* k_split;
    void* vt_split;
    int32_t qkv_c;
    int32_t qkv_rows;
    int32_t a_fmt;
    float acc_scale;
    int32_t out_split_parts;
    int32_t out_split_fmt;
    float out_split_scale;
    float vt_scale;
} aldm_igemm_desc;

int aldm_igemm(const aldm_igemm_desc* d, void* stream);
int64_t aldm_igemm_ws_floats(const aldm_igemm_desc* d);
enum { ALDM_FMT_BF16 = 0, ALDM_FMT_F16 = 1 };
int aldm_igemm_plan(const aldm_igemm_desc* d, int* bm, int* bn, int64_t* flops, int* splits, int* kgroups,
                    int* mma);
int aldm_igemm_plan_stages(const aldm_igemm_desc* d);
void aldm_igemm_force(int bm, int bn, int splits, int kgroups);
void aldm_igemm_force_stages(int stages);
int aldm_igemm_wave8_mask(int mask);
int aldm_igemm_mma(int mode);
#ifdef ALDM_TEST_HOOKS
int aldm_debug_drop_product(int on);
#endif
int64_t aldm_split_bytes(int K, int N);
int aldm_pack_split_bf16(const float* packed, void* dst, int K, int N, void* stream);
int64_t aldm_split_bytes_parts(int K, int N, int parts);
int aldm_pack_split_bf16_parts(const float* packed, void* dst, int K, int N, int parts, void* stream);
int aldm_pack_split_f16(const float* packed, void* dst, int K, int N, float scale, void* stream);

int64_t aldm_split_image_bytes(int64_t rows, int C, int parts);
int aldm_split_rows(const float* x1, const float* x2, int C1, int C2, int64_t rows, int P, const float* scale,
                    const float* shift, int act, void* dst, void* dst_raw, int parts, void* stream);
int aldm_split_rows_act(const float* x1, const float* x2, int C1, int C2, int64_t rows, int P, const float* scale,
                        const float* shift, int act, float slope, void* dst, void* dst_raw, int parts, void* stream);
int aldm_split_rows_f16(const float* x1, const float* x2, int C1, int C2, int64_t rows, int P, const float* scale,
                        const float* shift, int act, float slope, void* dst, void* dst_raw, int raw_parts, float f16_scale,
                        void* stream);

int aldm_pack_weight(const float* src, float* dst, int N, int Cin, int KH, int KW,
                     int transposed, int phase, int stride, void* stream);
int aldm_pack_kn(const float* src, float* dst, int K, int N, int lds, int batch,
                 int64_t stride_src, int64_t stride_dst, void* stream);

int aldm_groupnorm_stats(const float* x1, const float* x2, int B, int P, int C1, int C2,
                         int G, float eps, const float* gamma, const float* beta,
                         float* scale, float* shift, float* ws, void* stream);
int64_t aldm_gn_ws_floats(int B, int P, int C, int G);
int aldm_groupnorm_split(const float* x1, const float* x2, int B, int P, int C1, int C2, int G, float eps,
                         const float* gamma, const float* beta, int act, float* scale, float* shift, float* ws,
                         void* dst, void* dst_raw, int parts, void* stream);
int aldm_groupnorm_split_f16(const float* x1, const float* x2, int B, int P, int C1, int C2, int G, float eps,
                             const float* gamma, const float* beta, int act, float* scale, float* shift, float* ws,
                             void* dst, void* dst_raw, int raw_parts, float f16_scale, void* stream);
int aldm_layernorm(const float* x, float* y, int M, int C, const float* gamma,
                   const float* beta, float eps, void* stream);
int aldm_layernorm_split(const float* x, float* y, void* y_split, int M, int C, const float* gamma,
                         const float* beta, float eps, int parts, void* stream);
int aldm_layernorm_split_f16(const float* x, float* y, void* y_split, int M, int C, const float* gamma,
                             const float* beta, float eps, float f16_scale, void* stream);

int aldm_attention_d32(const float* q, const float* k, const float* v, float* out,
                       int B, int heads, int Lq, int Lk, int ldq, int ldk, int ldv, int ldo,
                       const float* mask, float scale, void* stream);
int aldm_attention_d32_split(const float* q, const float* k, const float* v, float* out, void* out_split,
                             int parts, int B, int heads, int Lq, int Lk, int ldq, int ldk, int ldv, int ldo,
                             const float* mask, float scale, void* stream);
int aldm_attention_d32_presplit(const float* q, const void* k_split, const void* vt_split, float* out, void* out_split,
                                int parts, int B, int heads, int Lq, int Lk, int ldq, int ldo, float scale, void* stream);
int aldm_vt_regroup(const void* src, void* dst, int B, int L, int heads, int parts, void* stream);
int aldm_attention_mma(int mode);
int aldm_attention_sched(int sched);
int aldm_attention_query_tiles(int B, int heads, int Lq);
int aldm_attention_d32_presplit_f16(const float* q, const void* k_split, const void* vt_split, float* out, void* out_split,
                                    int out_parts, float out_scale, int B, int heads, int Lq, int Lk, int ldq, int ldo,
                                    float scale, float q_scale, float k_scale, float v_scale, void* stream);
int aldm_rel_attention(const float* q, const float* k, const float* v, float* out, int B, int heads, int T, int d,
                       int ldq, int ldk, int ldv, int ldo, const float* emb_k, const float* emb_v, int window,
                       const float* mask, void* stream);
int aldm_rowscale_add(const float* x, const float* s, const float* res, float* y, int64_t rows, int C, int divide,
                      void* stream);
int aldm_rmsnorm(const float* x, float* y, int M, int C, const float* weight, float eps, void* stream);
int aldm_softmax_rows_bias(const float* x, float* y, int B, int heads, int q_rows, int N, float scale, const float* bias,
                           const float* keymask, void* stream);
int aldm_softmax_rows(const float* x, float* y, int64_t M, int N, float scale, void* stream);
int aldm_softmax_rows_masked(const float* x, float* y, int B, int heads, int q_rows, int N, float scale,
                             const float* keymask, int q_pos0, void* stream);

int aldm_decode_linear(const float* x, int ldx, int M, int K, const float* w_kn, int N, const float* bias,
                       const float* ln_gamma, const float* ln_beta, float ln_eps, int act, const float* res, int ldr,
                       float* y, int ldy, void* stream);
int aldm_decode_attention(const float* qkv, int ldq, const int64_t* pos, float* k_cache, float* v_cache, const float* keymask,
                          int B, int heads, int n_tot, float scale, float* out, int ldo, void* stream);
int aldm_decode_gemv_slices(int K, int N);
int aldm_decode_gemv(const float* x, int ldx, int xparts, int64_t xstride, const float* xbias, int xact, int M, int K,
                     const float* w_kn, int N, float* ypart, void* stream);
int aldm_decode_reduce_ln(const float* part, int nparts, int64_t pstride, int ldp, const float* bias, const int64_t* bias_row,
                          const float* res, int ldr, int M, int N, float* h_out, int ldh, const float* ln_gamma,
                          const float* ln_beta, float ln_eps, float* xn, int ldn, float* xn2, int ldn2, void* stream);
int aldm_decode_attention_parts(const float* qkv_part, int ldq, int qparts, int64_t qstride, const float* qbias,
                                const int64_t* pos, float* k_cache, float* v_cache, const float* keymask, int B, int heads,
                                int n_tot, float scale, float* out, int ldo, void* stream);

int aldm_geglu(const float* x, float* y, int64_t M, int C, void* stream);
int aldm_timestep_embedding(const float* t, float* out, int B, int dim, float max_period,
                            void* stream);
int aldm_nchw_to_nhwc(const float* x, float* y, int B, int C, int HW, int rep, void* stream);
int aldm_nhwc_to_nchw(const float* x, float* y, int B, int C, int HW, void* stream);
int aldm_ddim_step(const float* x, const float* eps, const float* noise, const float* coef,
                   float* x_prev, float* pred_x0, int64_t n, void* stream);
int aldm_ddim_step_indexed(float* x, const float* eps, const float* noise_tab, const float* coef_tab,
                           const int* step_idx, float* pred_x0, int64_t n, int coef_ld, void* stream);
int aldm_plms_first_step(const float* x, const float* e_t, const float* e_next, const float* coef_row, float* x_out,
                         float* pred_x0, float* hist, int64_t n, void* stream);
int aldm_plms_step_indexed(float* x, const float* eps, float* hist, const float* coef_tab, const int* step_idx,
                           float* pred_x0, int64_t n, int coef_ld, void* stream);
int aldm_dpmpp_step_indexed(float* x, const float* eps, float* x0_buf, const float* coef_tab, const int* step_idx, int64_t n,
                            int coef_ld, void* stream);
int aldm_step_advance(int* step_idx, const float* t_tab, float* t_cur, int nt, int steps, void* stream);
int aldm_ddpm_step(const float* x, const float* eps, const float* noise, const float* coef,
                   float* x_prev, int64_t n, void* stream);
int aldm_inpaint_blend(const float* x0, const float* qnoise, const float* mask, const float* coef,
                       float* x, int64_t n, void* stream);
int aldm_axpby(const float* a, const float* b, float* y, float alpha, float beta, int64_t n,
               void* stream);
int aldm_reflect_pad_1d(const float* x, float* y, int B, int T, int pad, int ld_out,
                        void* stream);
int aldm_mag_phase(const float* spec, float* mag, float* phase, int64_t M, int F, int ld_spec,
                   int ld_mag, void* stream);

int aldm_row_l2norm(const float* x, float* out, int64_t M, int F, int ld, void* stream);

int aldm_resample_sinc(const float* x, const float* kernel, float* y, int B, int T, int Tout, int down, int up, int taps,
                       int width, void* stream);
int aldm_power_spec(const float* spec, float* out, int64_t M, int F, int ld_spec, int ld_out, void* stream);
int aldm_col_affine(const float* x, const float* scale, const float* shift, float* y, int64_t rows, int C, void* stream);
int aldm_bicubic_patchify(const float* x, float* out, int B, int T, int mel, int S, int p, void* stream);
int aldm_token_mean(const float* x, float* y, int B, int L, int C, void* stream);
int aldm_row_cosine(const float* a, const float* b, float* out, int M, int C, float eps, void* stream);

#ifdef __cplusplus
}
#endif
#endif
```

Before: 18.95 audio-s/s.

## Fuse GroupNorm column statistics into conv GEMM epilogue and finalize from records

The implicit-GEMM epilogue now optionally emits per-32-row, per-column mean and M2 records, merged across lanes with shuffles, for the output tensor. A new finalize kernel combines these records into GroupNorm scale and shift, so the following GroupNorm no longer rereads the full activation to compute statistics. The UNet runner decides per layer whether the next norm benefits and requests records. This adds epilogue work and register pressure to the GEMMs and a small record buffer, and the statistics path is restricted to simple plain epilogues.

```diff
diff --git a/audioldm2_amd/csrc/api.hip b/audioldm2_amd/csrc/api.hip
--- a/audioldm2_amd/csrc/api.hip
+++ b/audioldm2_amd/csrc/api.hip
@@ -11,5 +11,5 @@
 }
 }
 
-extern "C" int aldm_version(void) { return 13; }
+extern "C" int aldm_version(void) { return 14; }
 extern "C" const char* aldm_last_error(void) { return aldm::g_err; }
diff --git a/audioldm2_amd/csrc/igemm.hip b/audioldm2_amd/csrc/igemm.hip
--- a/audioldm2_amd/csrc/igemm.hip
+++ b/audioldm2_amd/csrc/igemm.hip
@@ -288,7 +288,7 @@
     return (BM == 128 && (BN == 128 || BN == 64 || BN == 32)) || (BM == 64 && (BN == 128 || BN == 64));
 }
 
-static int igemm_prepare(const aldm_igemm_desc* dd, IgemmK& p, int& BM, int& BN) {
+static int igemm_prepare_plan(const aldm_igemm_desc* dd, IgemmK& p, int& BM, int& BN) {
     ALDM_CHECK(dd != nullptr, "aldm_igemm: null descriptor");
     p.d = *dd;
     aldm_igemm_desc& d = p.d;
@@ -672,6 +672,28 @@
     return 0;
 }
 
+static int igemm_prepare(const aldm_igemm_desc* dd, IgemmK& p, int& BM, int& BN) {
+    const int rc = igemm_prepare_plan(dd, p, BM, BN);
+    if (rc) return rc;
+    aldm_igemm_desc& d = p.d;
+    if (d.col_stats) {
+        const bool shared_epi = !(p.dma && (p.ws == 1 || p.ws == 3));
+        const bool vec = (d.ldo & 3) == 0 && (d.N & 3) == 0 && (d.stride_o & 3) == 0 &&
+                         ((reinterpret_cast<uintptr_t>(d.out) | reinterpret_cast<uintptr_t>(d.res)) & 15) == 0;
+        if (!(shared_epi && vec && d.epi_mode == ALDM_EPI_PLAIN && d.out != nullptr && p.splits == 1 && d.batch == 1 &&
+              d.accumulate == 0 && d.out_mul == 0 && p.OHW % 32 == 0 && (reinterpret_cast<uintptr_t>(d.col_stats) & 7) == 0))
+            d.col_stats = nullptr;
+    }
+    return 0;
+}
+
+extern "C" int aldm_igemm_col_stats(const aldm_igemm_desc* dd) {
+    IgemmK p;
+    int BM, BN;
+    if (igemm_prepare(dd, p, BM, BN)) return -1;
+    return p.d.col_stats != nullptr ? 1 : 0;
+}
+
 extern "C" int aldm_igemm_plan(const aldm_igemm_desc* dd, int* bm, int* bn, int64_t* flops, int* splits,
                                int* kgroups, int* mma) {
     IgemmK p;
diff --git a/audioldm2_amd/csrc/igemm_epilogue.h b/audioldm2_amd/csrc/igemm_epilogue.h
--- a/audioldm2_amd/csrc/igemm_epilogue.h
+++ b/audioldm2_amd/csrc/igemm_epilogue.h
@@ -200,6 +200,7 @@
     const bool need_b = !split_out && (d.rowbias != nullptr || d.out_mul > 0);
     const int ld_out = split_out ? d.N : d.ldo;
     void* simg = split_out ? nullptr : d.out_split;
+    float* cst = d.col_stats;
     int col_shift = 0;
     int simg_c = d.out_split_c;
     if (d.epi_mode == ALDM_EPI_QKV) {
@@ -299,6 +300,7 @@
 #pragma unroll
             for (int e = 0; e < 16; ++e)
                 stg[((e & 3) + 8 * (e >> 2) + 4 * lh) * SP + j * 32 + l31] = acc[i][j][e];
+        f32x4 cs_p = {0.f, 0.f, 0.f, 0.f}, cs_s = {0.f, 0.f, 0.f, 0.f}, cs_q = {0.f, 0.f, 0.f, 0.f};
 #pragma unroll
         for (int itc = 0; itc < IT; itc += ITC) {
         f32x4 v[ITC];
@@ -374,6 +376,16 @@
 #pragma unroll
                 for (int it = 0; it < ITC; ++it) v[it] += *reinterpret_cast<const f32x4*>(outp + rowoff[it]);
             }
+            if (cst) {
+                if (itc == 0) cs_p = v[0];
+#pragma unroll
+                for (int it = 0; it < ITC; ++it) {
+                    const f32x4 dv = v[it] - cs_p;
+                    cs_s += dv;
+#pragma unroll
+                    for (int c = 0; c < 4; ++c) cs_q[c] = __builtin_fmaf(dv[c], dv[c], cs_q[c]);
+                }
+            }
             if (outp) {
 #pragma unroll
                 for (int it = 0; it < ITC; ++it)
@@ -406,7 +418,56 @@
                 }
         }
         }
-    }
-}
-
-}
+        if (cst) {
+            static_assert(RPI == 2 || RPI == 4 || RPI == 8, "column statistics: 2, 4 or 8 lanes per column quad");
+            constexpr float inv_n = 1.0f / IT;
+            float mu[4], m2[4];
+#pragma unroll
+            for (int c = 0; c < 4; ++c) {
+                const float md = cs_s[c] * inv_n;
+                mu[c] = cs_p[c] + md;
+                m2[c] = fmaxf(__builtin_fmaf(-cs_s[c], md, cs_q[c]), 0.f);
+            }
+            constexpr int SA = C4 * (RPI / 2);
+            const bool ba = (lane & SA) != 0;
+            float km[2], k2[2];
+#pragma unroll
+            for (int k = 0; k < 2; ++k) {
+                const float om = __shfl_xor(ba ? mu[k] : mu[2 + k], SA), o2 = __shfl_xor(ba ? m2[k] : m2[2 + k], SA);
+                const float am = ba ? mu[2 + k] : mu[k], a2 = ba ? m2[2 + k] : m2[k];
+                const float dl = om - am;
+                km[k] = 0.5f * (am + om);
+                k2[k] = (a2 + o2) + (dl * dl) * (0.5f * IT);
+            }
+            const int mb = m0 + (wm * MT + i) * 32;
+            const bool st_ok = epi_st && mb < p.M && ncol < d.N;
+            float* rec = cst + ((int64_t)(mb >> 5) * d.N + ncol + (ba ? 2 : 0)) * 2;
+            if constexpr (RPI == 2) {
+                if (st_ok) *reinterpret_cast<f32x4*>(rec) = f32x4{km[0], k2[0], km[1], k2[1]};
+            } else {
+                constexpr int SB = C4 * (RPI / 4);
+                const bool bb = (lane & SB) != 0;
+                const float om = __shfl_xor(bb ? km[0] : km[1], SB), o2 = __shfl_xor(bb ? k2[0] : k2[1], SB);
+                const float am = bb ? km[1] : km[0], a2 = bb ? k2[1] : k2[0];
+                float dl = om - am;
+                float rm = 0.5f * (am + om);
+                float r2 = (a2 + o2) + (dl * dl) * (1.0f * IT);
+                bool mine = true;
+                if constexpr (RPI == 8) {
+                    const float pm = __shfl_xor(rm, C4), p2 = __shfl_xor(r2, C4);
+                    dl = pm - rm;
+                    rm = 0.5f * (rm + pm);
+                    r2 = (r2 + p2) + (dl * dl) * (2.0f * IT);
+                    mine = (lane & C4) == 0;
+                }
+                if (st_ok && mine) {
+                    float* r1 = rec + (bb ? 2 : 0);
+                    r1[0] = rm;
+                    r1[1] = r2;
+                }
+            }
+        }
+    }
+}
+
+}
diff --git a/audioldm2_amd/csrc/norm.hip b/audioldm2_amd/csrc/norm.hip
--- a/audioldm2_amd/csrc/norm.hip
+++ b/audioldm2_amd/csrc/norm.hip
@@ -255,6 +255,64 @@
     }
 }
 
+__global__ __launch_bounds__(256) void gn_finalize_records_kernel(const float* __restrict__ rec1, const float* __restrict__ rec2,
+                                                                  int S, int C1, int C2, int G, float eps,
+                                                                  const float* __restrict__ gamma, const float* __restrict__ beta,
+                                                                  float* __restrict__ scale, float* __restrict__ shift,
+                                                                  int rb1, int rb2) {
+    const int g = blockIdx.x, b = blockIdx.y, tid = threadIdx.x;
+    const int C = C1 + C2, Cg = C / G, c_lo = g * Cg;
+    const int64_t s1 = (int64_t)(b % rb1) * S, s2 = (int64_t)(b % rb2) * S;
+    const int total = S * Cg;
+    auto rec_of = [&](int i) {
+        const int sl = i / Cg, c = c_lo + (i - sl * Cg);
+        const float* r = c < C1 ? rec1 + ((s1 + sl) * C1 + c) * 2 : rec2 + ((s2 + sl) * C2 + (c - C1)) * 2;
+        return *reinterpret_cast<const float2*>(r);
+    };
+    double n = 0.0, mean = 0.0, m2 = 0.0;
+    constexpr int GN_REC_UNROLL = 8;
+    float2 v[GN_REC_UNROLL];
+#pragma unroll
+    for (int u = 0; u < GN_REC_UNROLL; ++u) {
+        const int i = tid + u * 256;
+        v[u] = i < total ? rec_of(i) : float2{0.f, 0.f};
+    }
+#pragma unroll
+    for (int u = 0; u < GN_REC_UNROLL; ++u)
+        if (tid + u * 256 < total) gn_merge(n, mean, m2, 32.0, (double)v[u].x, (double)v[u].y);
+    for (int i = tid + GN_REC_UNROLL * 256; i < total; i += 256) {
+        const float2 w = rec_of(i);
+        gn_merge(n, mean, m2, 32.0, (double)w.x, (double)w.y);
+    }
+#pragma unroll
+    for (int o = 32; o > 0; o >>= 1) {
+        const double nb = __shfl_xor(n, o), mb = __shfl_xor(mean, o), m2b = __shfl_xor(m2, o);
+        gn_merge(n, mean, m2, nb, mb, m2b);
+    }
+    __shared__ double wred[4][3];
+    __shared__ float fin[2];
+    if ((tid & 63) == 0) {
+        wred[tid >> 6][0] = n;
+        wred[tid >> 6][1] = mean;
+        wred[tid >> 6][2] = m2;
+    }
+    __syncthreads();
+    if (tid == 0) {
+        double an = 0.0, am = 0.0, a2 = 0.0;
+        for (int w = 0; w < 4; ++w) gn_merge(an, am, a2, wred[w][0], wred[w][1], wred[w][2]);
+        double var = an > 0.0 ? a2 / an : 0.0;
+        if (var < 0.0) var = 0.0;
+        fin[0] = (float)am;
+        fin[1] = (float)(1.0 / sqrt(var + (double)eps));
+    }
+    __syncthreads();
+    for (int c = c_lo + tid; c < c_lo + Cg; c += 256) {
+        const float sc = fin[1] * (gamma ? gamma[c] : 1.f);
+        scale[(int64_t)b * C + c] = sc;
+        shift[(int64_t)b * C + c] = (beta ? beta[c] : 0.f) - fin[0] * sc;
+    }
+}
+
 constexpr int LN_MAXV = 8;
 
 template <int MAXV, int R, bool RMS = false>
@@ -410,7 +468,8 @@
 
 static int groupnorm_launch(const float* x1, const float* x2, int B, int P, int C1, int C2, int G, float eps,
                             const float* gamma, const float* beta, float* scale, float* shift, float* ws, void* dst,
-                            void* dst_raw, int parts, int act, void* stream, int raw_parts = 0, float f16_scale = 0.f) {
+                            void* dst_raw, int parts, int act, void* stream, int raw_parts = 0, float f16_scale = 0.f,
+                            const float* rec1 = nullptr, const float* rec2 = nullptr, int rb1 = 0, int rb2 = 0) {
     if (raw_parts == 0) raw_parts = parts;
     if (!x2) C2 = 0;
     const int C = C1 + C2;
@@ -421,10 +480,8 @@
     int cols, rows, chunk_px, chunks;
     gn_geometry(P, C, &cols, &rows, &chunk_px, &chunks);
     hipStream_t st = (hipStream_t)stream;
-    static const int64_t fused_max = [] {
-        const char* e = getenv("ALDM_GN_FUSED_MAX");
-        return e ? (int64_t)atoll(e) : (int64_t)1 << 17;
-    }();
+    const char* fm_env = getenv("ALDM_GN_FUSED_MAX");
+    const int64_t fused_max = fm_env ? (int64_t)atoll(fm_env) : (int64_t)1 << 17;
     int gs = 1;
     while (gs < G && gs * B < 256 && G % (gs * 2) == 0) gs *= 2;
     const int gpb = G / gs;
@@ -445,6 +502,10 @@
         }
         hipLaunchKernelGGL(gn_partial_kernel<true>, dim3(gs, B), dim3(256), 0, st, x1, x2, P, C1, C2, G, fcols,
                            frows, P, ws, eps, gamma, beta, scale, shift, gpb, nullptr, nullptr, 3, ALDM_ACT_NONE);
+    } else if (rec1 && (!x2 || rec2) && P % 32 == 0 && rb1 >= 0 && rb2 >= 0 && B % (rb1 > 0 ? rb1 : B) == 0 && B % (rb2 > 0 ? rb2 : B) == 0 &&
+               ((reinterpret_cast<uintptr_t>(rec1) | reinterpret_cast<uintptr_t>(rec2)) & 7) == 0) {
+        hipLaunchKernelGGL(gn_finalize_records_kernel, dim3(G, B), dim3(256), 0, st, rec1, x2 ? rec2 : nullptr, P / 32, C1, C2, G,
+                           eps, gamma, beta, scale, shift, rb1 > 0 ? rb1 : B, rb2 > 0 ? rb2 : B);
     } else {
         hipLaunchKernelGGL(gn_partial_kernel<false>, dim3(chunks, B), dim3(256), 0, st, x1, x2, P, C1, C2, G,
                            cols, rows, chunk_px, ws, eps, gamma, beta, scale, shift, G);
@@ -489,6 +550,41 @@
     ALDM_CHECK(((reinterpret_cast<uintptr_t>(dst) | reinterpret_cast<uintptr_t>(dst_raw)) & 15) == 0,
                "aldm_groupnorm_split_f16: split images must be 16-byte aligned");
     return groupnorm_launch(x1, x2, B, P, C1, C2, G, eps, gamma, beta, scale, shift, ws, dst, dst_raw, 2, act, stream, raw_parts, f16_scale);
+}
+
+extern "C" int aldm_groupnorm_stats_rec(const float* x1, const float* x2, int B, int P, int C1, int C2, int G, float eps,
+                                        const float* gamma, const float* beta, float* scale, float* shift, float* ws,
+                                        const float* rec1, const float* rec2, int rb1, int rb2, void* stream) {
+    return groupnorm_launch(x1, x2, B, P, C1, C2, G, eps, gamma, beta, scale, shift, ws, nullptr, nullptr, 3, ALDM_ACT_NONE,
+                            stream, 0, 0.f, rec1, rec2, rb1, rb2);
+}
+
+extern "C" int aldm_groupnorm_split_rec(const float* x1, const float* x2, int B, int P, int C1, int C2, int G, float eps,
+                                        const float* gamma, const float* beta, int act, float* scale, float* shift, float* ws,
+                                        void* dst, void* dst_raw, int parts, const float* rec1, const float* rec2, int rb1, int rb2,
+                                        void* stream) {
+    if (!x2) C2 = 0;
+    ALDM_CHECK(dst != nullptr && (parts == 2 || parts == 3) && (C1 + C2) % 32 == 0 && C1 % 8 == 0 && C2 % 8 == 0,
+               "aldm_groupnorm_split: need dst, parts 2|3, (C1+C2) %% 32 == 0, C1 %% 8 == 0 (C1=%d C2=%d)", C1, C2);
+    ALDM_CHECK(act == ALDM_ACT_NONE || act == ALDM_ACT_SILU, "aldm_groupnorm_split: activation %d not supported", act);
+    ALDM_CHECK(((reinterpret_cast<uintptr_t>(dst) | reinterpret_cast<uintptr_t>(dst_raw)) & 15) == 0,
+               "aldm_groupnorm_split: split images must be 16-byte aligned");
+    return groupnorm_launch(x1, x2, B, P, C1, C2, G, eps, gamma, beta, scale, shift, ws, dst, dst_raw, parts, act, stream, 0, 0.f,
+                            rec1, rec2, rb1, rb2);
+}
+
+extern "C" int aldm_groupnorm_split_f16_rec(const float* x1, const float* x2, int B, int P, int C1, int C2, int G, float eps,
+                                            const float* gamma, const float* beta, int act, float* scale, float* shift, float* ws,
+                                            void* dst, void* dst_raw, int raw_parts, float f16_scale, const float* rec1,
+                                            const float* rec2, int rb1, int rb2, void* stream) {
+    if (!x2) C2 = 0;
+    ALDM_CHECK(dst != nullptr && f16_scale > 0.0f && (raw_parts == 2 || raw_parts == 3) && (C1 + C2) % 32 == 0 && C1 % 8 == 0 && C2 % 8 == 0,
+               "aldm_groupnorm_split_f16: need dst, f16_scale > 0, raw_parts 2|3, (C1+C2) %% 32 == 0, C1 %% 8 == 0 (C1=%d C2=%d)", C1, C2);
+    ALDM_CHECK(act == ALDM_ACT_NONE || act == ALDM_ACT_SILU, "aldm_groupnorm_split_f16: activation %d not supported", act);
+    ALDM_CHECK(((reinterpret_cast<uintptr_t>(dst) | reinterpret_cast<uintptr_t>(dst_raw)) & 15) == 0,
+               "aldm_groupnorm_split_f16: split images must be 16-byte aligned");
+    return groupnorm_launch(x1, x2, B, P, C1, C2, G, eps, gamma, beta, scale, shift, ws, dst, dst_raw, 2, act, stream, raw_parts,
+                            f16_scale, rec1, rec2, rb1, rb2);
 }
 
 static int layernorm_launch(const float* x, float* y, void* y_split, int parts, int M, int C, const float* gamma,
diff --git a/audioldm2_amd/lib.py b/audioldm2_amd/lib.py
--- a/audioldm2_amd/lib.py
+++ b/audioldm2_amd/lib.py
@@ -5,7 +5,7 @@
 
 _HERE = os.path.dirname(os.path.abspath(__file__))
 LIB_PATH = os.environ.get("ALDM_LIB_PATH") or os.path.join(_HERE, "libaldm_hip.so")
-ABI_VERSION = 13
+ABI_VERSION = 14
 
 ACT_NONE, ACT_SILU, ACT_LRELU, ACT_TANH, ACT_LOGCLAMP, ACT_GELU, ACT_GELU_TANH = range(7)
 B_PACKED, B_NT = 0, 1
@@ -44,6 +44,7 @@
         ("k_split", C.c_void_p), ("vt_split", C.c_void_p), ("qkv_c", C.c_int32), ("qkv_rows", C.c_int32),
         ("a_fmt", C.c_int32), ("acc_scale", C.c_float), ("out_split_parts", C.c_int32),
         ("out_split_fmt", C.c_int32), ("out_split_scale", C.c_float), ("vt_scale", C.c_float),
+        ("col_stats", C.c_void_p),
     ]
 
 
@@ -56,6 +57,7 @@
                                   C.POINTER(C.c_int)]),
     "aldm_igemm_ws_floats": (C.c_int64, [C.POINTER(IgemmDesc)]),
     "aldm_igemm_plan_stages": (C.c_int, [C.POINTER(IgemmDesc)]),
+    "aldm_igemm_col_stats": (C.c_int, [C.POINTER(IgemmDesc)]),
     "aldm_igemm_force": (None, [C.c_int, C.c_int, C.c_int, C.c_int]),
     "aldm_igemm_force_stages": (None, [C.c_int]),
     "aldm_igemm_wave8_mask": (C.c_int, [C.c_int]),
@@ -93,6 +95,16 @@
     "aldm_groupnorm_split": (C.c_int, [C.c_void_p, C.c_void_p, C.c_int, C.c_int, C.c_int, C.c_int, C.c_int, C.c_float,
                                        C.c_void_p, C.c_void_p, C.c_int, C.c_void_p, C.c_void_p, C.c_void_p, C.c_void_p,
                                        C.c_void_p, C.c_int, C.c_void_p]),
+    "aldm_groupnorm_stats_rec": (C.c_int, [C.c_void_p, C.c_void_p, C.c_int, C.c_int, C.c_int, C.c_int,
+                                           C.c_int, C.c_float, C.c_void_p, C.c_void_p, C.c_void_p,
+                                           C.c_void_p, C.c_void_p, C.c_void_p, C.c_void_p, C.c_int, C.c_int, C.c_void_p]),
+    "aldm_groupnorm_split_rec": (C.c_int, [C.c_void_p, C.c_void_p, C.c_int, C.c_int, C.c_int, C.c_int, C.c_int, C.c_float,
+                                           C.c_void_p, C.c_void_p, C.c_int, C.c_void_p, C.c_void_p, C.c_void_p, C.c_void_p,
+                                           C.c_void_p, C.c_int, C.c_void_p, C.c_void_p, C.c_int, C.c_int, C.c_void_p]),
+    "aldm_groupnorm_split_f16_rec": (C.c_int, [C.c_void_p, C.c_void_p, C.c_int, C.c_int, C.c_int, C.c_int, C.c_int, C.c_float,
+                                               C.c_void_p, C.c_void_p, C.c_int, C.c_void_p, C.c_void_p, C.c_void_p, C.c_void_p,
+                                               C.c_void_p, C.c_int, C.c_float, C.c_void_p, C.c_void_p, C.c_int, C.c_int,
+                                               C.c_void_p]),
     "aldm_layernorm": (C.c_int, [C.c_void_p, C.c_void_p, C.c_int, C.c_int, C.c_void_p, C.c_void_p,
                                  C.c_float, C.c_void_p]),
     "aldm_attention_mma": (C.c_int, [C.c_int]),
diff --git a/audioldm2_amd/ops.py b/audioldm2_amd/ops.py
--- a/audioldm2_amd/ops.py
+++ b/audioldm2_amd/ops.py
@@ -387,9 +387,10 @@
             d.hint_bm, d.hint_bn, d.hint_splits, d.hint_kgroups = hint[:4]
             d.hint_mma = hint[4] if len(hint) > 4 else 0
     _workspace(lib, d, device if device is not None else torch.device("cuda", torch.cuda.current_device()))
+    wrote = bool(d.col_stats) and lib.aldm_igemm_col_stats(C.byref(d)) == 1
     if PROFILE is None:
         _l.check(lib.aldm_igemm(C.byref(d), _stream()), what)
-        return
+        return wrote
     bm, bn, fl, sp, kg, mma = C.c_int(), C.c_int(), C.c_int64(), C.c_int(), C.c_int(), C.c_int()
     _l.check(lib.aldm_igemm_plan(C.byref(d), C.byref(bm), C.byref(bn), C.byref(fl), C.byref(sp), C.byref(kg),
                                  C.byref(mma)), what)
@@ -403,6 +404,7 @@
              int(d.epi_mode == _l.EPI_GEGLU), int(bool(d.res)))
     PROFILE.append((what, bm.value, bn.value, fl.value, e0, e1, shape,
                     _kernel_name(d, bm.value, bn.value, kg.value, bool(mma.value))))
+    return wrote
 
 
 def _pre_mode(d: IgemmDesc) -> int:
@@ -677,7 +679,8 @@
          act: int = ACT_NONE, act_slope: float = 0.0, alpha: float = 1.0,
          out: Optional[torch.Tensor] = None, accumulate: bool = False,
          remap: Optional[Tuple[int, int, int]] = None,
-         use_pw_bias: bool = True, split_out: Optional[str] = None, split_act: int = ACT_NONE, split_slope: float = 0.0):
+         use_pw_bias: bool = True, split_out: Optional[str] = None, split_act: int = ACT_NONE, split_slope: float = 0.0,
+         want_col_stats: bool = False):
     is_split = isinstance(x, SplitT)
     if is_split:
         assert x2 is None and pre is None and pre_act == ACT_NONE, "a pre-split operand takes no prologue"
@@ -744,10 +747,17 @@
     d.accumulate = 1 if accumulate else 0
     d.out_mul = out_mul; d.out_off = out_off; d.out_len = out_len
     d.batch = 1
-    _igemm(d, "igemm(conv)")
+    rec = None
+    if want_col_stats and _GN_EPI_STATS and out is not None and remap is None and (OH * OW) % 32 == 0:
+        rec = torch.empty((B * OH * OW // 32, N, 2), device=x.device, dtype=torch.float32)
+        d.col_stats = rec.data_ptr()
+    wrote = _igemm(d, "igemm(conv)")
     if split_out == "only":
         return so
-    return (out.view(oshape), so) if split_out else out.view(oshape)
+    res_t = out.view(oshape)
+    if rec is not None and wrote:
+        res_t._col_stats = rec
+    return (res_t, so) if split_out else res_t
 
 
 def linear(x, pw: Packed, **kw):
@@ -760,8 +770,8 @@
         y = conv(x.reshape(1, 1, M, shp[-1]), pw, **kw)
     oshape = (*shp[:-1], pw.N)
     if isinstance(y, tuple):
-        return y[0].view(oshape), y[1].view(oshape)
-    return y.view(oshape)
+        return _keep_col_stats(y[0].view(oshape), y[0]), y[1].view(oshape)
+    return _keep_col_stats(y.view(oshape), y)
 
 
 def _view3(t: torch.Tensor, name: str):
@@ -819,6 +829,52 @@
 
 _gn_ws = {}
 
+_GN_EPI_STATS = os.environ.get("ALDM_GN_EPI_STATS", "1") != "0"
+
+
+def set_gn_epi_stats(on: bool) -> bool:
+    global _GN_EPI_STATS
+    prev, _GN_EPI_STATS = _GN_EPI_STATS, bool(on)
+    return prev
+
+
+def gn_wants_records(P: int, C: int) -> bool:
+    fused_max = int(os.environ.get("ALDM_GN_FUSED_MAX", 1 << 17))
+    return _GN_EPI_STATS and P % 32 == 0 and (P * C > fused_max or P > 1024)
+
+
+def col_stats_of(t) -> Optional[torch.Tensor]:
+    return getattr(t, "_col_stats", None) if _GN_EPI_STATS else None
+
+
+def _keep_col_stats(new: torch.Tensor, old: torch.Tensor) -> torch.Tensor:
+    rec = getattr(old, "_col_stats", None)
+    if rec is not None:
+        new._col_stats = rec
+    return new
+
+
+def dup_samples(t: torch.Tensor) -> torch.Tensor:
+    out = t.repeat(2, *([1] * (t.dim() - 1)))
+    rec = getattr(t, "_col_stats", None)
+    if rec is not None:
+        out._col_stats = rec
+    return out
+
+
+def _gn_records(x, x2):
+    r1 = col_stats_of(x)
+    r2 = col_stats_of(x2) if x2 is not None else None
+    if r1 is None or (x2 is not None and r2 is None):
+        return None, None
+    return r1, r2
+
+
+def _rec_samples(x, rec) -> int:
+    if rec is None:
+        return 0
+    return rec.shape[0] * 32 * x.shape[0] // (x.numel() // x.shape[-1])
+
 
 def gn_stats(x: torch.Tensor, gamma: torch.Tensor, beta: torch.Tensor, *, groups: int = 32,
              eps: float = 1e-5, x2: Optional[torch.Tensor] = None):
@@ -835,6 +891,13 @@
     nws = lib.aldm_gn_ws_floats(B, P, Cc, groups)
     ws = torch.empty(nws, device=x.device, dtype=torch.float32)
     ss = torch.empty((2, B, Cc), device=x.device, dtype=torch.float32)
+    r1, r2 = _gn_records(x, x2)
+    if r1 is not None:
+        _l.check(lib.aldm_groupnorm_stats_rec(x.data_ptr(), _p(x2), B, P, C1, C2, groups, eps,
+                                              gamma.data_ptr(), beta.data_ptr(), ss[0].data_ptr(),
+                                              ss[1].data_ptr(), ws.data_ptr(), r1.data_ptr(), _p(r2), _rec_samples(x, r1),
+                                              _rec_samples(x2, r2), _stream()), "groupnorm_stats_rec")
+        return ss[0], ss[1]
     _l.check(lib.aldm_groupnorm_stats(x.data_ptr(), _p(x2), B, P, C1, C2, groups, eps,
                                       gamma.data_ptr(), beta.data_ptr(), ss[0].data_ptr(),
                                       ss[1].data_ptr(), ws.data_ptr(), _stream()), "groupnorm_stats")
@@ -858,13 +921,26 @@
     ss = torch.empty((2, B, Cc), device=x.device, dtype=torch.float32)
     shape = (*x.shape[:-1], Cc)
     raw = SplitT.empty(shape, x.device) if want_raw else None
+    r1, r2 = _gn_records(x, x2)
     if f16_mode():
         dst = SplitT.empty(shape, x.device, f16_scale=_norm_f16_scale(gamma, beta, (Cc // groups) * P))
+        if r1 is not None:
+            _l.check(lib.aldm_groupnorm_split_f16_rec(x.data_ptr(), _p(x2), B, P, C1, C2, groups, eps, gamma.data_ptr(), beta.data_ptr(),
+                                                      act, ss[0].data_ptr(), ss[1].data_ptr(), ws.data_ptr(), dst.data_ptr(),
+                                                      None if raw is None else raw.data_ptr(), 3, dst.scale, r1.data_ptr(), _p(r2),
+                                                      _rec_samples(x, r1), _rec_samples(x2, r2), _stream()), "groupnorm_split_f16_rec")
+            return (dst, raw) if want_raw else dst
         _l.check(lib.aldm_groupnorm_split_f16(x.data_ptr(), _p(x2), B, P, C1, C2, groups, eps, gamma.data_ptr(), beta.data_ptr(), act,
                                               ss[0].data_ptr(), ss[1].data_ptr(), ws.data_ptr(), dst.data_ptr(),
                                               None if raw is None else raw.data_ptr(), 3, dst.scale, _stream()), "groupnorm_split_f16")
         return (dst, raw) if want_raw else dst
     dst = SplitT.empty(shape, x.device)
+    if r1 is not None:
+        _l.check(lib.aldm_groupnorm_split_rec(x.data_ptr(), _p(x2), B, P, C1, C2, groups, eps, gamma.data_ptr(), beta.data_ptr(), act,
+                                              ss[0].data_ptr(), ss[1].data_ptr(), ws.data_ptr(), dst.data_ptr(),
+                                              None if raw is None else raw.data_ptr(), dst.parts, r1.data_ptr(), _p(r2),
+                                              _rec_samples(x, r1), _rec_samples(x2, r2), _stream()), "groupnorm_split_rec")
+        return (dst, raw) if want_raw else dst
     _l.check(lib.aldm_groupnorm_split(x.data_ptr(), _p(x2), B, P, C1, C2, groups, eps, gamma.data_ptr(), beta.data_ptr(), act,
                                       ss[0].data_ptr(), ss[1].data_ptr(), ws.data_ptr(), dst.data_ptr(),
                                       None if raw is None else raw.data_ptr(), dst.parts, _stream()), "groupnorm_split")
diff --git a/audioldm2_amd/unet.py b/audioldm2_amd/unet.py
--- a/audioldm2_amd/unet.py
+++ b/audioldm2_amd/unet.py
@@ -45,9 +45,10 @@
             )
         return self._pk
 
-    def run(self, x, e, x2=None):
+    def run(self, x, e, x2=None, out_stats=False):
         pk = self._prepare()
         c2 = 0 if x2 is None else x2.shape[-1]
+        hst = ops.gn_wants_records(x.shape[1] * x.shape[2], self.out_channels)
         if ops.use_dma() and self.channels % 32 == 0 and x.shape[-1] % 8 == 0 and c2 % 8 == 0:
             if pk["skip"] is None:
                 assert x2 is None
@@ -55,18 +56,18 @@
             else:
                 a1, araw = ops.gn_split(x, *pk["gn1"], groups=32, eps=1e-5, x2=x2, act=ACT_SILU, want_raw=True)
                 skip = ops.conv(araw, pk["skip"])
-            h = ops.conv(a1, pk["conv1"], pad=(1, 1), rowbias=e)
+            h = ops.conv(a1, pk["conv1"], pad=(1, 1), rowbias=e, want_col_stats=hst)
             a2 = ops.gn_split(h, *pk["gn2"], groups=32, eps=1e-5, act=ACT_SILU)
-            return ops.conv(a2, pk["conv2"], pad=(1, 1), res=skip)
+            return ops.conv(a2, pk["conv2"], pad=(1, 1), res=skip, want_col_stats=out_stats)
         sc, sh = ops.gn_stats(x, *pk["gn1"], groups=32, eps=1e-5, x2=x2)
-        h = ops.conv(x, pk["conv1"], x2=x2, pad=(1, 1), pre=(sc, sh), pre_act=ACT_SILU, rowbias=e)
+        h = ops.conv(x, pk["conv1"], x2=x2, pad=(1, 1), pre=(sc, sh), pre_act=ACT_SILU, rowbias=e, want_col_stats=hst)
         sc2, sh2 = ops.gn_stats(h, *pk["gn2"], groups=32, eps=1e-5)
         if pk["skip"] is None:
             assert x2 is None
             skip = x
         else:
             skip = ops.conv(x, pk["skip"], x2=x2)
-        return ops.conv(h, pk["conv2"], pad=(1, 1), pre=(sc2, sh2), pre_act=ACT_SILU, res=skip)
+        return ops.conv(h, pk["conv2"], pad=(1, 1), pre=(sc2, sh2), pre_act=ACT_SILU, res=skip, want_col_stats=out_stats)
 
 
 class Downsample(nn.Module):
@@ -79,12 +80,12 @@
         self.op = nn.Conv2d(channels, self.out_channels, 3, stride=2, padding=padding)
         self._pk = None
 
-    def run(self, x):
+    def run(self, x, out_stats=False):
         if self._pk is None:
             self._pk = ops.pack_conv(self.op.weight, self.op.bias)
         if ops.use_dma() and self.channels % 32 == 0:
             x = ops.split_rows(x)
-        return ops.conv(x, self._pk, stride=(2, 2), pad=(1, 1))
+        return ops.conv(x, self._pk, stride=(2, 2), pad=(1, 1), want_col_stats=out_stats)
 
 
 class Upsample(nn.Module):
@@ -97,12 +98,12 @@
         self.conv = nn.Conv2d(channels, self.out_channels, 3, padding=padding)
         self._pk = None
 
-    def run(self, x):
+    def run(self, x, out_stats=False):
         if self._pk is None:
             self._pk = ops.pack_conv(self.conv.weight, self.conv.bias)
         if ops.use_dma() and self.channels % 32 == 0:
             x = ops.split_rows(x)
-        return ops.conv(x, self._pk, pad=(1, 1), up=(2, 2))
+        return ops.conv(x, self._pk, pad=(1, 1), up=(2, 2), want_col_stats=out_stats)
 
 
 class GEGLU(nn.Module):
@@ -225,7 +226,7 @@
         self.proj_out = nn.Conv2d(inner, in_channels, 1)
         self._pk = None
 
-    def run(self, x, context=None, mask=None):
+    def run(self, x, context=None, mask=None, out_stats=False):
         if self._pk is None:
             self._pk = dict(gn=(self.norm.weight.detach().float().cuda().contiguous(),
                                 self.norm.bias.detach().float().cuda().contiguous()),
@@ -239,36 +240,49 @@
             for i, blk in enumerate(self.transformer_blocks):
                 r = blk.run(h, context, mask, want_split=i == len(self.transformer_blocks) - 1)
                 h, hs = r if isinstance(r, tuple) else (r, None)
-            return ops.conv((hs if hs is not None else h).view(B, H, W, -1), pk["pout"], res=x)
+            return ops.conv((hs if hs is not None else h).view(B, H, W, -1), pk["pout"], res=x, want_col_stats=out_stats)
         sc, sh = ops.gn_stats(x, *pk["gn"], groups=32, eps=1e-6)
         h = ops.conv(x, pk["pin"], pre=(sc, sh)).view(B, H * W, -1)
         for blk in self.transformer_blocks:
             h = blk.run(h, context, mask)
-        return ops.conv(h.view(B, H, W, -1), pk["pout"], res=x)
+        return ops.conv(h.view(B, H, W, -1), pk["pout"], res=x, want_col_stats=out_stats)
+
+
+def _out_width(layer) -> int:
+    if isinstance(layer, SpatialTransformer):
+        return layer.in_channels
+    return layer.out_channels
 
 
 class TimestepEmbedSequential(nn.Sequential):
 
-    def run(self, x, emb, context_list, mask_list, x2=None, lo=0, hi=None):
+    def run(self, x, emb, context_list, mask_list, x2=None, lo=0, hi=None, next_c=None):
         ctxs = [None] + list(context_list)
         masks = [None] + list(mask_list)
         layers = list(self)
         st_id = sum(isinstance(l, SpatialTransformer) for l in layers[:lo])
         for layer in layers[lo:hi]:
+            P = x.shape[1] * x.shape[2]
+            if isinstance(layer, Downsample):
+                P = ((x.shape[1] + 1) // 2) * ((x.shape[2] + 1) // 2)
+            elif isinstance(layer, Upsample):
+                P *= 4
+            st = ops.gn_wants_records(P, _out_width(layer)) or \
+                (next_c is not None and hi is None and layer is layers[-1] and ops.gn_wants_records(P, next_c))
             if isinstance(layer, ResBlock):
-                x = layer.run(x, emb[layer._emb_slice], x2)
+                x = layer.run(x, emb[layer._emb_slice], x2, out_stats=st)
                 x2 = None
             elif isinstance(layer, SpatialTransformer):
                 if st_id >= len(ctxs):
                     c, m = None, None
                 else:
                     c, m = ctxs[st_id], masks[st_id]
-                x = layer.run(x, c, m)
+                x = layer.run(x, c, m, out_stats=st)
                 st_id += 1
             elif isinstance(layer, (Downsample, Upsample)):
-                x = layer.run(x)
+                x = layer.run(x, out_stats=st)
             elif isinstance(layer, _ConvIn):
-                x = layer.run(x)
+                x = layer.run(x, out_stats=st)
             else:
                 raise RuntimeError(f"unexpected layer {type(layer)}")
         assert x2 is None, "skip tensor was not consumed by a ResBlock"
@@ -288,10 +302,10 @@
 
     _pk = None
 
-    def run(self, x):
+    def run(self, x, out_stats=False):
         if self._pk is None:
             self._pk = ops.pack_conv(self.weight, self.bias)
-        return ops.conv(x, self._pk, pad=(1, 1))
+        return ops.conv(x, self._pk, pad=(1, 1), want_col_stats=out_stats)
 
 
 class UNetModel(nn.Module):
@@ -434,6 +448,15 @@
             )
         return self._pk
 
+    def _norm_widths(self):
+        if getattr(self, "_nw", None) is None:
+            w_in = [_out_width(list(m)[-1]) for m in self.input_blocks]
+            w_out = [_out_width(list(m)[-1]) for m in self.output_blocks]
+            n = len(w_in)
+            cat = [(w_in[-1] if j == 0 else w_out[j - 1]) + w_in[n - 1 - j] for j in range(len(w_out))]
+            self._nw = ([cat[n - 1 - i] for i in range(n)], cat[0], cat[1:] + [w_out[-1]])
+        return self._nw
+
     def _shared_prefix_end(self, context_list):
         if self.use_extra_film_by_concat:
             return None
@@ -472,28 +495,29 @@
         emb = _EmbSlices(emb_rows)
         h = ops.nchw_to_nhwc(x.float().contiguous())
         hs = []
+        in_c, mid_c, out_c = self._norm_widths()
         if div is None:
-            for module in self.input_blocks:
-                h = module.run(h, emb, context_list, mask_list)
+            for bi, module in enumerate(self.input_blocks):
+                h = module.run(h, emb, context_list, mask_list, next_c=in_c[bi])
                 hs.append(h)
         else:
-            dup = lambda t: t.repeat(2, *([1] * (t.dim() - 1)))
+            dup = ops.dup_samples
             emb_half, emb = emb, _EmbSlices(dup(emb_rows))
             for bi, module in enumerate(self.input_blocks):
                 if bi < div[0]:
-                    h = module.run(h, emb_half, context_list, mask_list)
+                    h = module.run(h, emb_half, context_list, mask_list, next_c=in_c[bi])
                 elif bi == div[0]:
                     h = module.run(h, emb_half, context_list, mask_list, hi=div[1])
-                    h = module.run(dup(h), emb, context_list, mask_list, lo=div[1])
+                    h = module.run(dup(h), emb, context_list, mask_list, lo=div[1], next_c=in_c[bi])
                 else:
-                    h = module.run(h, emb, context_list, mask_list)
+                    h = module.run(h, emb, context_list, mask_list, next_c=in_c[bi])
                 hs.append(h)
-        h = self.middle_block.run(h, emb, context_list, mask_list)
-        for module in self.output_blocks:
+        h = self.middle_block.run(h, emb, context_list, mask_list, next_c=mid_c)
+        for bi, module in enumerate(self.output_blocks):
             skip = hs.pop()
             if skip.shape[0] != h.shape[0]:
-                skip = dup(skip)
-            h = module.run(h, emb, context_list, mask_list, x2=skip)
+                skip = ops.dup_samples(skip)
+            h = module.run(h, emb, context_list, mask_list, x2=skip, next_c=out_c[bi])
         sc, sh = ops.gn_stats(h, *pk["gn"], groups=32, eps=1e-5)
         out = ops.conv(h, pk["out"], pad=(1, 1), pre=(sc, sh), pre_act=ACT_SILU)
         return ops.nhwc_to_nchw(out)
diff --git a/include/aldm_hip.h b/include/aldm_hip.h
--- a/include/aldm_hip.h
+++ b/include/aldm_hip.h
@@ -83,10 +83,12 @@
     int32_t out_split_fmt;
     float out_split_scale;
     float vt_scale;
+    float* col_stats;
 } aldm_igemm_desc;
 
 int aldm_igemm(const aldm_igemm_desc* d, void* stream);
 int64_t aldm_igemm_ws_floats(const aldm_igemm_desc* d);
+int aldm_igemm_col_stats(const aldm_igemm_desc* d);
 enum { ALDM_FMT_BF16 = 0, ALDM_FMT_F16 = 1 };
 int aldm_igemm_plan(const aldm_igemm_desc* d, int* bm, int* bn, int64_t* flops, int* splits, int* kgroups,
                     int* mma);
@@ -128,6 +130,17 @@
 int aldm_groupnorm_split_f16(const float* x1, const float* x2, int B, int P, int C1, int C2, int G, float eps,
                              const float* gamma, const float* beta, int act, float* scale, float* shift, float* ws,
                              void* dst, void* dst_raw, int raw_parts, float f16_scale, void* stream);
+int aldm_groupnorm_stats_rec(const float* x1, const float* x2, int B, int P, int C1, int C2, int G, float eps,
+                             const float* gamma, const float* beta, float* scale, float* shift, float* ws,
+                             const float* rec1, const float* rec2, int rb1, int rb2, void* stream);
+int aldm_groupnorm_split_rec(const float* x1, const float* x2, int B, int P, int C1, int C2, int G, float eps,
+                             const float* gamma, const float* beta, int act, float* scale, float* shift, float* ws,
+                             void* dst, void* dst_raw, int parts, const float* rec1, const float* rec2, int rb1, int rb2,
+                             void* stream);
+int aldm_groupnorm_split_f16_rec(const float* x1, const float* x2, int B, int P, int C1, int C2, int G, float eps,
+                                 const float* gamma, const float* beta, int act, float* scale, float* shift, float* ws,
+                                 void* dst, void* dst_raw, int raw_parts, float f16_scale, const float* rec1, const float* rec2,
+                                 int rb1, int rb2, void* stream);
 int aldm_layernorm(const float* x, float* y, int M, int C, const float* gamma,
                    const float* beta, float eps, void* stream);
 int aldm_layernorm_split(const float* x, float* y, void* y_split, int M, int C, const float* gamma,
```

Measured after the change: 19.02 audio-s/s (median of 6 runs). No clear change (+0.4%).
